# vklyukin/nf_distillation

Hardware: NVIDIA B200
Metric: kd_train_samples_per_sec (higher is better)
Workload: dtype bf16

## Files before the change

include/nfk.h:

```cpp
#ifndef NFK_H_
#define NFK_H_

#ifdef __cplusplus
extern "C" {
#endif

#define NFK_OK 0
#define NFK_ERR_SHAPE (-1)
#define NFK_ERR_ALIGN (-2)
#define NFK_ERR_ARG (-3)
#define NFK_ERR_LAUNCH (-4)
#define NFK_ERR_DRIVER (-5)

#define NFK_EPI_F32 0
#define NFK_EPI_BIAS_RELU_BF16 1
#define NFK_EPI_MASK_BF16 2

int nfk_version(void);

int nfk_gemm_nt_bf16(const void* A, long long lda, const void* B, long long ldb, int M, int N, int K, int epi,
                     void* out, long long ldo, const float* bias, const void* aux, long long ldaux, float* colsum,
                     void* stream);

int nfk_gemm_set_prof(void* buf);

int nfk_gemm_tn_bf16(const void* A, long long lda, const void* B, long long ldb, int Mo, int No, int Kpix,
                     float* out, long long ldo, int sm_count, void* stream);

typedef struct nfk_invconv_item {
  const float *an_bias, *an_logs, *lower, *upper, *log_s, *p, *sign_s, *weight;
  int C, reverse, transpose;
  float *outW, *outb, *out_sl;
} nfk_invconv_item;
typedef struct nfk_invconv_bwd_item {
  nfk_invconv_item fwd;
  const float* dWf;
  int dWf_ld;
  const float* dbf;
  const float* g_ld;
  int B;
  float pixels;
  float *d_bias, *d_logs, *d_lower, *d_upper, *d_log_s, *d_weight;
} nfk_invconv_bwd_item;
int nfk_invconv_prep_batch(int n, const nfk_invconv_item* items, void* stream);
int nfk_invconv_prep_bwd_batch(int n, const nfk_invconv_bwd_item* items, void* stream);

int nfk_invconv_prep(const float* an_bias, const float* an_logs, const float* lower, const float* upper,
                     const float* log_s, const float* p, const float* sign_s, const float* weight, int C, int reverse,
                     int transpose, float* outW, float* outb, float* out_sl, void* stream);

int nfk_invconv_prep_bwd(const float* an_bias, const float* an_logs, const float* lower, const float* upper,
                         const float* log_s, const float* p, const float* sign_s, const float* weight, int C,
                         int reverse, int transpose, const float* Wf, const float* dWf, const float* dbf,
                         const float* g_ld, int B,
                         float pixels, float* d_bias, float* d_logs, float* d_lower, float* d_upper, float* d_log_s,
                         float* d_weight, void* stream);

typedef struct nfk_coupling_item {
  const float *w1, *b1, *l1, *w2, *b2, *l2, *w3, *b3, *l3;
  int cin, hid, cout, K1p, K3p, with_transposed;
  void *B1, *B1T, *B2, *B2T, *B3, *B3T;
  float *bias1, *bias2, *bias3;
} nfk_coupling_item;
typedef struct nfk_coupling_bwd_item {
  nfk_coupling_item fwd;
  const float *dB1, *dbias1, *dB2, *dbias2, *dB3, *dbias3;
  float *dw1, *db1, *dl1, *dw2, *db2, *dl2, *dw3, *db3, *dl3;
} nfk_coupling_bwd_item;
int nfk_coupling_prep_batch(int n, const nfk_coupling_item* items, void* stream);
int nfk_coupling_prep_bwd_batch(int n, const nfk_coupling_bwd_item* items, void* stream);

int nfk_coupling_prep(const float* w1, const float* b1, const float* l1, const float* w2, const float* b2,
                      const float* l2, const float* w3, const float* b3, const float* l3, int cin, int hid, int cout,
                      int K1p, int K3p, void* B1, void* B1T, void* B2, void* B2T, void* B3, void* B3T, float* bias1,
                      float* bias2, float* bias3, int with_transposed, void* stream);

int nfk_coupling_prep_bwd(const float* w1, const float* b1, const float* l1, const float* w2, const float* b2,
                          const float* l2, const float* w3, const float* b3, const float* l3, int cin, int hid,
                          int cout, int K1p, int K3p, const float* dB1, const float* dbias1, const float* dB2,
                          const float* dbias2, const float* dB3, const float* dbias3, float* dw1, float* db1,
                          float* dl1, float* dw2, float* db2, float* dl2, float* dw3, float* db3, float* dl3,
                          void* stream);

int nfk_affine1x1_fwd(const float* x, const float* Wf, const float* bf, const float* sl, float* y, void* col,
                      int K1p, const float* ld_in, float* ld_out, int B, int C, int H, int W, void* stream);

int nfk_coupling_fwd(const float* P, int K3p, const float* bias3, float* y, float* hsave, float* ld, int B, int C,
                     int H, int W, int reverse, void* stream);

int nfk_coupling_bwd(const float* g_out, const float* g_ld, const float* z_out, const float* hsave, float* dy,
                     void* dhcol, int K3p, float* dbias3, int B, int C, int H, int W, void* stream);

int nfk_affine1x1_bwd(const float* dy, const float* dcol, int K1p, const float* x, const float* Wf, float* dx,
                      float* dWf, float* dbf, int B, int C, int H, int W, void* stream);

int nfk_coupling_inv_bwd(const float* g_zc, const float* g_ld, const float* zc, const float* hsave, float* dz,
                         void* dhcol, int K3p, float* dbias3, int B, int C, int H, int W, void* stream);

int nfk_col2im_add(const float* dcol, int K1p, float* dz, int B, int C, int H, int W, void* stream);

int nfk_split2d_fwd(const float* x, const float* w, const float* bias, const float* logs, float* z1_out, float* ld,
                    int B, int C, int H, int W, void* stream);
int nfk_split2d_rev(const float* z1, const float* w, const float* bias, const float* logs, const float* eps,
                    float temperature, float* out, int B, int C, int H, int W, void* stream);
int nfk_split2d_bwd(const float* x, const float* w, const float* bias, const float* logs, const float* g_z1,
                    const float* g_ld, float* dx, float* dw, float* dbias, float* dlogs, int B, int C, int H, int W,
                    void* stream);
int nfk_split2d_squeeze_fwd(const float* x, const float* w, const float* bias, const float* logs, float* z1_out,
                            float* z1_sq_out, float* ld, int B, int C, int H, int W, void* stream);
int nfk_split2d_squeeze_bwd(const float* x, const float* w, const float* bias, const float* logs, const float* g_z1,
                            const float* g_z1_sq, const float* g_ld, float* dx, float* dw, float* dbias, float* dlogs,
                            int B, int C, int H, int W, void* stream);
int nfk_dequant_squeeze(const void* src, int src_is_u8, int n_bits, const float* noise, float* x_out, float* sq_out,
                        int B, int C, int H, int W, void* stream);
int nfk_prior_bpd_fwd(const float* z, const float* mean, const float* logs, const float* logdet, int B, int n,
                      float scale, float* out, void* stream);
int nfk_prior_bpd_bwd(const float* z, const float* mean, const float* logs, const float* g_bpd, int B, int n,
                      float scale, float* dz, float* dlogdet, void* stream);
int nfk_kd_mse_fwd(const float* s, const float* t, int B, int n, float scale, float* acc, void* stream);
int nfk_kd_mse_bwd(const float* s, const float* t, const float* g, int B, int n, float scale, float* ds,
                   int accumulate, void* stream);

int nfk_pconv_coupling_supported(int C, int H, int W, int hid);
int nfk_pconv_coupling_fwd(const void* h2, const void* B3, int K3p, const float* bias3, float* y, float* hsave,
                           float* ld, int B, int C, int H, int W, int hid, int reverse, void* stream);

int nfk_conv1_dgrad_affine_bwd_supported(int C, int H, int W, int hid);
int nfk_conv1_dgrad_affine_bwd(const void* dpre1, const void* B1T, int K1p, const float* dy, const float* x,
                               const float* Wf, float* dx, float* dWf, float* dbf, int B, int C, int H, int W, int hid,
                               void* stream);

int nfk_flow1d_supported(int D, int Cc, int hid, int training);
int nfk_flow1d_sizes(int D, int Cc, int hid, int* total_fwd, int* total_bwd, int* total_grad, int* n_act,
                     int* offsets);
int nfk_flow1d_pack(const float* Wf, const float* bf, const float* const* w, const float* const* b, int D, int Cc,
                    int hid, float* PF, float* PB, void* stream);
int nfk_flow1d_fwd(const float* x, const float* cond, const float* PF, const float* sl, float* y, const float* ld_in,
                   float* ld_out, float* acts, int B, int D, int Cc, int hid, int reverse, void* stream);
int nfk_flow1d_bwd(const float* x_in, const float* cond, const float* acts, const float* PB, const float* y_out,
                   const float* g_out, const float* g_ld, float* dx, float* G, int B, int D, int Cc, int hid,
                   int reverse, void* stream);
int nfk_affine_rows(const float* x, const float* Wf, const float* bf, const float* sl, float* y, const float* ld_in,
                    float* ld_out, int B, int D, float pixels, void* stream);

int nfk_gemm_nt_bf16_ranged(const void* A, long long lda, const void* B, long long ldb, int M, int N, int K, int epi,
                            void* out, long long ldo, const float* bias, const void* aux, long long ldaux,
                            float* colsum, int bn, const int* kb_begin, const int* kb_end, void* stream);

int nfk_made_prep(const float* w1, const float* w2, const float* w3, const int* deg1, const int* deg2, int D, int H,
                  int Dp, int N3p, void* B1, void* B1T, void* B2, void* B2T, void* B3, void* B3T, int with_t,
                  void* stream);
int nfk_made_prep_bwd(const float* dB1, const float* dB2, const float* dB3, const int* deg1, const int* deg2, int D,
                      int H, int Dp, float* dw1, float* dw2, float* dw3, void* stream);
int nfk_rows_to_bf16(const float* x, int B, int D, int Dp, void* xb, void* stream);
int nfk_made_affine_fwd(const float* x, const float* out, int N3p, float* u, void* ub, int Dp, const float* ld_in,
                        float* ld_out, int B, int D, int flip, void* stream);
int nfk_made_affine_bwd(const float* x, const float* out, int N3p, const float* g_u, const float* g_ld, float* dx,
                        void* dout, float* db3, int B, int D, int flip, void* stream);
int nfk_made_inv_update(float* x, void* xb, int Dp, const float* u_in, const float* out, int N3p, const float* ld_in,
                        float* ld_out, int B, int D, int i, int flip, int last, void* stream);
int nfk_made_inverse_resident_supported(int D, int H, int Dp);
int nfk_made_inverse_push_supported(int D, int H, int Dp, int N3p);
int nfk_made_inverse_jobs(const int* cnt1, const int* cnt2, int D, int H, int Dp, int N3p, int push, int* jobs,
                          int cap);
int nfk_made_inverse_pack(const int* jobs, int njobs, const void* B1, const void* B2, const void* B3, int N3p, int D,
                          int H, int Dp, int push, void* wstream, void* stream);
int nfk_made_inverse_resident(const float* u_in, const void* wstream, const float* b1, const float* b2,
                              const float* b3, const int* jobs, int njobs, int push, int N3p, float* x,
                              const float* ld_in, float* ld_out, int B, int D, int H, int Dp, int flip, int mtiles,
                              void* stream);
int nfk_made_inv_bwd_update(const float* c, int ldc, const float* g_x, const float* g_ld, const float* out, int N3p,
                            const float* u_in, float* g_u, void* dout, float* db3, int B, int D, int d, int flip,
                            void* stream);
int nfk_made_inverse_bwd_supported(int D, int H, int N3p);
int nfk_made_inverse_bwd_jobs(const int* cnt1, const int* cnt2, int D, int H, int N3p, int* jobs, int cap);
int nfk_made_inverse_bwd_pack(const int* jobs, int njobs, const void* B1T, const void* B2T, const void* B3T, int D,
                              int H, int N3p, void* wstream, void* stream);
int nfk_made_inverse_bwd_resident(const float* g_x, const float* g_ld, const float* out, const void* m1,
                                  const void* m2, const float* u_in, const void* wstream, const int* jobs, int njobs,
                                  float* g_u, void* dout, float* db3, int B, int D, int H, int N3p, int flip,
                                  int mtiles, void* stream);

int nfk_cnet_set_prof(void* buf);
int nfk_cnet_fwd_fused(const void* col, int K1p, const void* B1, const void* B2, const float* bias1,
                       const float* bias2, void* h1, void* h2, void* mask1, void* mask2, long long ldmask, int M,
                       int hid, void* stream);
int nfk_cnet_bwd_fused(const void* dhcol, int K3p, const void* B3T, const void* B2T, const void* mask_h2,
                       const void* mask_h1, long long ldmask, void* dpre2, void* dpre1, float* dbias2, float* dbias1,
                       int M, int hid, void* stream);
int nfk_cnet_fwd_fused_ranged(const void* col, int K1p, const void* B1, const void* B2, const float* bias1,
                              const float* bias2, void* h1, void* h2, void* mask1, void* mask2, long long ldmask,
                              int M, int hid, int kb2_end_half0, void* stream);

#define NFK_LOSS_MAX_LEVELS 8
typedef struct {
  const float* s[NFK_LOSS_MAX_LEVELS];
  const float* t[NFK_LOSS_MAX_LEVELS];
  float* ds[NFK_LOSS_MAX_LEVELS];
  int n[NFK_LOSS_MAX_LEVELS];
  int L;
} nfk_loss_levels;
int nfk_kd_nll_loss_scratch_floats(int B);
int nfk_kd_nll_loss_fwd(const nfk_loss_levels* levels, const float* z_last, int nz, const float* prior_mean,
                        const float* prior_logs, const float* logdet, float nll_scale, const float* nll_in,
                        const float* perc, const float* sample_w, float w_nll, float w_kd, float w_perc, int B,
                        float* nll_out, float* kd_out, float* means, float* scratch, void* stream);
int nfk_kd_nll_loss_bwd(const nfk_loss_levels* levels, const float* z_last, int nz, const float* prior_mean,
                        const float* prior_logs, float nll_scale, const float* sample_w, float w_nll, float w_kd,
                        float w_perc, int B, const float* g_means, const float* g_nll, const float* g_kd,
                        float* dz_last, float* dlogdet, float* dnll_in, float* dperc, void* stream);

int nfk_optim_partials(void);
int nfk_grad_sqnorm(const float* g, long long n, float* partials, int* step, void* stream);
int nfk_adam_step(float* p, const float* g, float* m, float* v, long long n, const float* partials, const int* step,
                  float max_norm, float lr, float beta1, float beta2, float eps, float weight_decay, int adamax,
                  float* norm_out, void* stream);

int nfk_split3_rows(const float* src, long long lds, long long rows, int K, int Ksrc, int pattern, void* out,
                    void* stream);
int nfk_im2col3x3_split3(const float* src, int layout, int Ctot, int c0, int Cc, int B, int H, int W, int flip,
                         int Kp, int pattern, void* out, void* stream);
int nfk_act_split3(const float* pre, long long M, int N, int mode, const void* gate, long long ldg, int pattern,
                   void* out, float* colsum, void* stream);
int nfk_coupling_bwd_f32(const float* g_out, const float* g_ld, const float* z_out, const float* hsave, float* dy,
                         float* dh, float* dbias3, int B, int C, int H, int W, void* stream);

#ifdef __cplusplus
}
#endif
#endif
```

nf_distillation_b200/_lib.py:

```python
from __future__ import annotations

import ctypes
import os

from . import build as _build

_c = ctypes
_vp, _i, _ll, _f = _c.c_void_p, _c.c_int, _c.c_longlong, _c.c_float

ERRORS = {
    -1: "NFK_ERR_SHAPE (unsupported / inconsistent sizes)",
    -2: "NFK_ERR_ALIGN (pointer or leading dimension not 16-byte aligned)",
    -3: "NFK_ERR_ARG (missing / invalid argument)",
    -4: "NFK_ERR_LAUNCH (CUDA launch failure)",
    -5: "NFK_ERR_DRIVER (tensor-map encode failure)",
}



class InvconvItem(_c.Structure):
    _fields_ = [(n, _vp) for n in ("an_bias", "an_logs", "lower", "upper", "log_s", "p", "sign_s", "weight")] + \
               [("C", _i), ("reverse", _i), ("transpose", _i)] + \
               [(n, _vp) for n in ("outW", "outb", "out_sl")]


class InvconvBwdItem(_c.Structure):
    _fields_ = [("fwd", InvconvItem), ("dWf", _vp), ("dWf_ld", _i), ("dbf", _vp), ("g_ld", _vp), ("B", _i),
                ("pixels", _f)] + \
               [(n, _vp) for n in ("d_bias", "d_logs", "d_lower", "d_upper", "d_log_s", "d_weight")]


class CouplingItem(_c.Structure):
    _fields_ = [(n, _vp) for n in ("w1", "b1", "l1", "w2", "b2", "l2", "w3", "b3", "l3")] + \
               [(n, _i) for n in ("cin", "hid", "cout", "K1p", "K3p", "with_transposed")] + \
               [(n, _vp) for n in ("B1", "B1T", "B2", "B2T", "B3", "B3T", "bias1", "bias2", "bias3")]


class CouplingBwdItem(_c.Structure):
    _fields_ = [("fwd", CouplingItem)] + \
               [(n, _vp) for n in ("dB1", "dbias1", "dB2", "dbias2", "dB3", "dbias3")] + \
               [(n, _vp) for n in ("dw1", "db1", "dl1", "dw2", "db2", "dl2", "dw3", "db3", "dl3")]


NFK_LOSS_MAX_LEVELS = 8


class LossLevels(_c.Structure):
    _fields_ = [("s", _vp * NFK_LOSS_MAX_LEVELS), ("t", _vp * NFK_LOSS_MAX_LEVELS), ("ds", _vp * NFK_LOSS_MAX_LEVELS),
                ("n", _i * NFK_LOSS_MAX_LEVELS), ("L", _i)]


SIGNATURES: dict[str, list] = {
    "nfk_version": [],
    "nfk_gemm_nt_bf16": [_vp, _ll, _vp, _ll, _i, _i, _i, _i, _vp, _ll, _vp, _vp, _ll, _vp, _vp],
    "nfk_gemm_set_prof": [_vp],
    "nfk_gemm_tn_bf16": [_vp, _ll, _vp, _ll, _i, _i, _i, _vp, _ll, _i, _vp],
    "nfk_invconv_prep_batch": [_i, _vp, _vp],
    "nfk_invconv_prep_bwd_batch": [_i, _vp, _vp],
    "nfk_invconv_prep": [_vp] * 8 + [_i, _i, _i, _vp, _vp, _vp, _vp],
    "nfk_invconv_prep_bwd": [_vp] * 8 + [_i, _i, _i, _vp, _vp, _vp, _vp, _i, _f] + [_vp] * 6 + [_vp],
    "nfk_coupling_prep_batch": [_i, _vp, _vp],
    "nfk_coupling_prep_bwd_batch": [_i, _vp, _vp],
    "nfk_coupling_prep": [_vp] * 9 + [_i] * 5 + [_vp] * 9 + [_i, _vp],
    "nfk_coupling_prep_bwd": [_vp] * 9 + [_i] * 5 + [_vp] * 6 + [_vp] * 9 + [_vp],
    "nfk_affine1x1_fwd": [_vp, _vp, _vp, _vp, _vp, _vp, _i, _vp, _vp, _i, _i, _i, _i, _vp],
    "nfk_coupling_fwd": [_vp, _i, _vp, _vp, _vp, _vp, _i, _i, _i, _i, _i, _vp],
    "nfk_coupling_bwd": [_vp, _vp, _vp, _vp, _vp, _vp, _i, _vp, _i, _i, _i, _i, _vp],
    "nfk_affine1x1_bwd": [_vp, _vp, _i, _vp, _vp, _vp, _vp, _vp, _i, _i, _i, _i, _vp],
    "nfk_coupling_inv_bwd": [_vp, _vp, _vp, _vp, _vp, _vp, _i, _vp, _i, _i, _i, _i, _vp],
    "nfk_col2im_add": [_vp, _i, _vp, _i, _i, _i, _i, _vp],
    "nfk_split2d_fwd": [_vp] * 6 + [_i] * 4 + [_vp],
    "nfk_split2d_rev": [_vp] * 5 + [_f, _vp] + [_i] * 4 + [_vp],
    "nfk_split2d_bwd": [_vp] * 10 + [_i] * 4 + [_vp],
    "nfk_split2d_squeeze_fwd": [_vp] * 7 + [_i] * 4 + [_vp],
    "nfk_split2d_squeeze_bwd": [_vp] * 11 + [_i] * 4 + [_vp],
    "nfk_dequant_squeeze": [_vp, _i, _i, _vp, _vp, _vp, _i, _i, _i, _i, _vp],
    "nfk_prior_bpd_fwd": [_vp] * 4 + [_i, _i, _f, _vp, _vp],
    "nfk_prior_bpd_bwd": [_vp] * 4 + [_i, _i, _f, _vp, _vp, _vp],
    "nfk_kd_mse_fwd": [_vp, _vp, _i, _i, _f, _vp, _vp],
    "nfk_kd_mse_bwd": [_vp, _vp, _vp, _i, _i, _f, _vp, _i, _vp],
    "nfk_flow1d_supported": [_i, _i, _i, _i],
    "nfk_flow1d_sizes": [_i, _i, _i, _vp, _vp, _vp, _vp, _vp],
    "nfk_flow1d_pack": [_vp, _vp, _vp, _vp, _i, _i, _i, _vp, _vp, _vp],
    "nfk_flow1d_fwd": [_vp] * 8 + [_i] * 5 + [_vp],
    "nfk_flow1d_bwd": [_vp] * 9 + [_i] * 5 + [_vp],
    "nfk_affine_rows": [_vp] * 7 + [_i, _i, _f, _vp],
    "nfk_gemm_nt_bf16_ranged": [_vp, _ll, _vp, _ll, _i, _i, _i, _i, _vp, _ll, _vp, _vp, _ll, _vp, _i, _vp, _vp, _vp],
    "nfk_cnet_set_prof": [_vp],
    "nfk_cnet_fwd_fused": [_vp, _i, _vp, _vp, _vp, _vp, _vp, _vp, _vp, _vp, _ll, _i, _i, _vp],
    "nfk_cnet_bwd_fused": [_vp, _i, _vp, _vp, _vp, _vp, _ll, _vp, _vp, _vp, _vp, _i, _i, _vp],
    "nfk_cnet_fwd_fused_ranged": [_vp, _i, _vp, _vp, _vp, _vp, _vp, _vp, _vp, _vp, _ll, _i, _i, _i, _vp],
    "nfk_pconv_coupling_supported": [_i, _i, _i, _i],
    "nfk_pconv_coupling_fwd": [_vp, _vp, _i, _vp, _vp, _vp, _vp, _i, _i, _i, _i, _i, _i, _vp],
    "nfk_conv1_dgrad_affine_bwd_supported": [_i, _i, _i, _i],
    "nfk_conv1_dgrad_affine_bwd": [_vp] * 9 + [_i] * 5 + [_vp],
    "nfk_made_prep": [_vp] * 5 + [_i] * 4 + [_vp] * 6 + [_i, _vp],
    "nfk_made_prep_bwd": [_vp] * 5 + [_i] * 3 + [_vp] * 3 + [_vp],
    "nfk_rows_to_bf16": [_vp, _i, _i, _i, _vp, _vp],
    "nfk_made_affine_fwd": [_vp, _vp, _i, _vp, _vp, _i, _vp, _vp, _i, _i, _i, _vp],
    "nfk_made_affine_bwd": [_vp, _vp, _i, _vp, _vp, _vp, _vp, _vp, _i, _i, _i, _vp],
    "nfk_made_inv_update": [_vp, _vp, _i, _vp, _vp, _i, _vp, _vp, _i, _i, _i, _i, _i, _vp],
    "nfk_made_inverse_resident_supported": [_i, _i, _i],
    "nfk_made_inverse_push_supported": [_i, _i, _i, _i],
    "nfk_made_inverse_jobs": [_vp, _vp, _i, _i, _i, _i, _i, _vp, _i],
    "nfk_made_inverse_pack": [_vp, _i, _vp, _vp, _vp, _i, _i, _i, _i, _i, _vp, _vp],
    "nfk_made_inverse_resident": [_vp] * 6 + [_i] * 3 + [_vp] * 3 + [_i] * 6 + [_vp],
    "nfk_made_inv_bwd_update": [_vp, _i, _vp, _vp, _vp, _i, _vp, _vp, _vp, _vp, _i, _i, _i, _i, _vp],
    "nfk_made_inverse_bwd_supported": [_i, _i, _i],
    "nfk_made_inverse_bwd_jobs": [_vp, _vp, _i, _i, _i, _vp, _i],
    "nfk_made_inverse_bwd_pack": [_vp, _i, _vp, _vp, _vp, _i, _i, _i, _vp, _vp],
    "nfk_made_inverse_bwd_resident": [_vp] * 8 + [_i] + [_vp] * 3 + [_i] * 6 + [_vp],
    "nfk_kd_nll_loss_scratch_floats": [_i],
    "nfk_kd_nll_loss_fwd": [_vp, _vp, _i, _vp, _vp, _vp, _f, _vp, _vp, _vp, _f, _f, _f, _i, _vp, _vp, _vp, _vp, _vp],
    "nfk_kd_nll_loss_bwd": [_vp, _vp, _i, _vp, _vp, _f, _vp, _f, _f, _f, _i, _vp, _vp, _vp, _vp, _vp, _vp, _vp, _vp],
    "nfk_optim_partials": [],
    "nfk_grad_sqnorm": [_vp, _ll, _vp, _vp, _vp],
    "nfk_adam_step": [_vp, _vp, _vp, _vp, _ll, _vp, _vp, _f, _f, _f, _f, _f, _f, _i, _vp, _vp],
    "nfk_split3_rows": [_vp, _ll, _ll, _i, _i, _i, _vp, _vp],
    "nfk_im2col3x3_split3": [_vp, _i, _i, _i, _i, _i, _i, _i, _i, _i, _i, _vp, _vp],
    "nfk_act_split3": [_vp, _ll, _i, _i, _vp, _ll, _i, _vp, _vp, _vp],
    "nfk_coupling_bwd_f32": [_vp, _vp, _vp, _vp, _vp, _vp, _vp, _i, _i, _i, _i, _vp],
}


class NfkError(RuntimeError):
    pass


def _load() -> ctypes.CDLL:
    path = _build.LIB_PATH
    if _build.needs_build():
        try:
            _build.build()
        except Exception as e:
            if not os.path.exists(path):
                raise ImportError(
                    f"libnfk.so is not built and cannot be built here ({e}); there is no CPU fallback") from e
    lib = ctypes.CDLL(path)
    for name, argtypes in SIGNATURES.items():
        fn = getattr(lib, name)
        fn.argtypes = argtypes
        fn.restype = _c.c_int
    return lib


LIB = _load()


def check(rc: int, what: str) -> None:
    if rc != 0:
        raise NfkError(f"{what} failed: {ERRORS.get(rc, rc)}")


def ptr(t) -> int | None:
    return None if t is None else t.data_ptr()


def stream_ptr() -> int:
    import torch

    return torch.cuda.current_stream().cuda_stream
```

nf_distillation_b200/csrc/cnet_fused.cu:

```cuda
#include <cuda.h>
#include <cuda_bf16.h>
#include <cuda_runtime.h>
#include <cstdint>
#include <cstdlib>

#include "../../include/nfk.h"
#include "launch_util.h"
#include "ptx.cuh"

namespace nfk {

constexpr int CF_THREADS = 320;
constexpr int CF_HID = 512;
constexpr int CF_SLOT = 16384;
constexpr int CF_SLOTS = 4;
constexpr int CF_PANEL = 16384;

struct CnetArgs {
  int M;
  int kb1;
  const float* bias1;
  const float* bias2;
  uint32_t* mask1;
  uint32_t* mask2;
  long long ldmask;
  int store_h1;
  long long* prof;
  int kb2_end[2];
  float* colsum1;
  float* colsum2;
};

struct CnetSmem {
  static constexpr int h1 = 0;
  static constexpr int ring = h1 + 8 * CF_PANEL;
  static constexpr int stage = ring + CF_SLOTS * CF_SLOT;
  static constexpr int bars = stage + 8 * 4096;
  static constexpr int total = bars + 256;
};

__device__ __forceinline__ uint32_t pack2(float lo, float hi) {
  __nv_bfloat162 v = __floats2bfloat162_rn(lo, hi);
  return *reinterpret_cast<uint32_t*>(&v);
}

template <int MODE>
__device__ __forceinline__ void cnet_fused_body(const CUtensorMap& tmCol, const CUtensorMap& tmB1,
                                                const CUtensorMap& tmB2, const CUtensorMap& tmH1,
                                                const CUtensorMap& tmH2, const CnetArgs& g) {
  extern __shared__ __align__(1024) uint8_t smem[];
  pdl_launch_dependents();
  if (smem_u32(smem) & 1023u) __trap();
  const int warp = static_cast<int>(uniform_u32(threadIdx.x >> 5)), lane = threadIdx.x & 31;
  const uint32_t rank = blockIdx.x & 1;
  const int pair = blockIdx.x >> 1, num_pairs = gridDim.x >> 1;
  const int num_tiles = (g.M + 255) / 256;

  uint64_t* full = reinterpret_cast<uint64_t*>(smem + CnetSmem::bars);
  uint64_t* empty = full + CF_SLOTS;
  uint64_t* acc_full = empty + CF_SLOTS;
  uint64_t* acc_empty = acc_full + 2;
  uint64_t* h1_full = acc_empty + 2;
  uint64_t* h1_empty = h1_full + 8;
  uint32_t* tmem_slot = reinterpret_cast<uint32_t*>(h1_empty + 1);

  if (warp == 0 && lane == 0) {
    tma_prefetch_desc(&tmCol); tma_prefetch_desc(&tmB1); tma_prefetch_desc(&tmB2); tma_prefetch_desc(&tmH2);
    for (int s = 0; s < CF_SLOTS; ++s) { mbar_init(&full[s], 1); mbar_init(&empty[s], 1); }
    for (int a = 0; a < 2; ++a) { mbar_init(&acc_full[a], 1); mbar_init(&acc_empty[a], 16); }
    for (int p = 0; p < 8; ++p) mbar_init(&h1_full[p], 8);
    mbar_init(h1_empty, 1);
    fence_mbar_init();
  }
  if (warp == 1) { tmem_alloc_pair(tmem_slot, 512); tmem_relinquish_pair(); }
  tc_fence_before();
  cluster_sync_all();
  tc_fence_after();
  const uint32_t tmem_base = uniform_u32(*tmem_slot);
  pdl_wait();

  if (warp == 0) {
    {
      int s = 0; uint32_t ph = 0;
      auto load = [&](const CUtensorMap* tm, int c0, int c1) {
        mbar_wait_warp(&empty[s], ph ^ 1);
        if (rank == 0) mbar_expect_tx_elect(&full[s], 2 * CF_SLOT);
        tma_load_2d_pair_elect(smem + CnetSmem::ring + s * CF_SLOT, tm, &full[s], c0, c1);
        if (++s == CF_SLOTS) { s = 0; ph ^= 1; }
      };
      for (int t = pair; t < num_tiles; t += num_pairs) {
        const int row0 = t * 256 + static_cast<int>(rank) * 128;
        for (int h = 0; h < 2; ++h)
          for (int kb = 0; kb < g.kb1; ++kb) {
            load(&tmCol, kb * 64, row0);
            load(&tmB1, kb * 64, h * 256 + static_cast<int>(rank) * 128);
          }
        for (int h = 0; h < 2; ++h)
          for (int kb = 0; kb < g.kb2_end[h]; ++kb) load(&tmB2, kb * 64, h * 256 + static_cast<int>(rank) * 128);
      }
    }
  } else if (warp == 1) {
    if (rank == 0) {
      const uint32_t idesc = umma_idesc_bf16(256, 256, false, false);
      const uint32_t ring_addr = smem_u32(smem + CnetSmem::ring);
      const uint32_t h1_addr = smem_u32(smem + CnetSmem::h1);
      int s = 0; uint32_t ph = 0;
      uint32_t nacc = 0;
      uint32_t tile_ph = 0;
      long long w_op = 0, w_acc = 0, w_h1 = 0;
      const long long t_begin = g.prof ? clock64() : 0;
      auto take = [&]() {
        const long long c0 = g.prof ? clock64() : 0;
        mbar_wait_warp(&full[s], ph);
        if (g.prof) w_op += clock64() - c0;
        tc_fence_after();
        return ring_addr + s * CF_SLOT;
      };
      auto advance = [&]() { if (++s == CF_SLOTS) { s = 0; ph ^= 1; } };
      auto release = [&]() { umma_commit_pair_elect(&empty[s], 3); advance(); };
      auto acc_begin = [&]() {
        const uint32_t st = nacc & 1;
        const long long c0 = g.prof ? clock64() : 0;
        mbar_wait_warp(&acc_empty[st], ((nacc >> 1) & 1) ^ 1);
        if (g.prof) w_acc += clock64() - c0;
        tc_fence_after();
        return tmem_base + st * 256;
      };
      auto acc_end = [&]() { umma_commit_pair_elect(&acc_full[nacc & 1], 3); ++nacc; };
      for (int t = pair; t < num_tiles; t += num_pairs) {
        for (int h = 0; h < 2; ++h) {
          const uint32_t d = acc_begin();
          for (int kb = 0; kb < g.kb1; ++kb) {
            const uint32_t a = take();
            const int sa = s;
            advance();
            const uint32_t b = take();
#pragma unroll
            for (int k = 0; k < 4; ++k)
              umma_f16_pair_elect(d, umma_desc_sw128(a + k * 32, 16, 1024), umma_desc_sw128(b + k * 32, 16, 1024), idesc,
                            (kb > 0 || k > 0) ? 1u : 0u);
            umma_commit_pair_elect(&empty[sa], 3);
            release();
          }
          acc_end();
        }
        int panels_seen = 0;
        for (int h = 0; h < 2; ++h) {
          const uint32_t d = acc_begin();
          for (int kb = 0; kb < g.kb2_end[h]; ++kb) {
            if (kb >= panels_seen) {
              const long long c0 = g.prof ? clock64() : 0;
              mbar_wait_warp(&h1_full[kb], tile_ph);
              if (g.prof) w_h1 += clock64() - c0;
              tc_fence_after();
              panels_seen = kb + 1;
            }
            const uint32_t b = take();
#pragma unroll
            for (int k = 0; k < 4; ++k)
              umma_f16_pair_elect(d, umma_desc_sw128(h1_addr + kb * CF_PANEL + k * 32, 16, 1024),
                            umma_desc_sw128(b + k * 32, 16, 1024), idesc, (kb > 0 || k > 0) ? 1u : 0u);
            release();
          }
          acc_end();
        }
        umma_commit_pair_elect(h1_empty, 3);
        tile_ph ^= 1;
      }
      if (g.prof && lane == 0) {
        long long* o = g.prof + blockIdx.x * 8;
        o[0] = clock64() - t_begin; o[1] = w_op; o[2] = w_acc; o[3] = w_h1;
      }
    }
  } else {
    const int qd = warp & 3;
    const int hf = (warp - 2) >> 2;
    const uint32_t lane_off = static_cast<uint32_t>(qd * 32) << 16;
    const uint32_t sw = static_cast<uint32_t>(lane & 7);
    uint8_t* stage = smem + CnetSmem::stage + (warp - 2) * 4096;
    uint32_t nacc = 0, tile_ph = 0;
    auto epi16 = [&](const uint32_t (&r)[16], const float* bias16, uint8_t* dst, int cc0, bool want_bits) -> uint32_t {
      uint32_t p[8];
      const __nv_bfloat162 zero2 = __floats2bfloat162_rn(0.f, 0.f);
#pragma unroll
      for (int j = 0; j < 16; j += 4) {
        const float4 b = __ldg(reinterpret_cast<const float4*>(bias16 + j));
        const float2 s0 = __fadd2_rn(make_float2(__uint_as_float(r[j]), __uint_as_float(r[j + 1])),
                                     make_float2(b.x, b.y));
        const float2 s1 = __fadd2_rn(make_float2(__uint_as_float(r[j + 2]), __uint_as_float(r[j + 3])),
                                     make_float2(b.z, b.w));
        const __nv_bfloat162 h0 = __hmax2(__float22bfloat162_rn(s0), zero2);
        const __nv_bfloat162 h1 = __hmax2(__float22bfloat162_rn(s1), zero2);
        p[j / 2] = *reinterpret_cast<const uint32_t*>(&h0);
        p[j / 2 + 1] = *reinterpret_cast<const uint32_t*>(&h1);
      }
      uint32_t bits = 0;
      if (want_bits) {
#pragma unroll
        for (int k = 0; k < 8; ++k) {
          bits |= ((p[k] & 0xFFFFu) ? 1u : 0u) << (2 * k);
          bits |= ((p[k] >> 16) ? 1u : 0u) << (2 * k + 1);
        }
      }
      *reinterpret_cast<uint4*>(dst + ((static_cast<uint32_t>(cc0) ^ sw) << 4)) = make_uint4(p[0], p[1], p[2], p[3]);
      *reinterpret_cast<uint4*>(dst + ((static_cast<uint32_t>(cc0 + 1) ^ sw) << 4)) =
          make_uint4(p[4], p[5], p[6], p[7]);
      return bits;
    };
    auto panel64 = [&](const uint32_t (&r0)[16], const uint32_t (&r1)[16], const uint32_t (&r2)[16],
                       const uint32_t (&r3)[16], const float* bias, uint8_t* dst_rows, uint32_t* mask, long long row,
                       int col0) {
      uint8_t* dst = dst_rows + lane * 128;
      const bool wb = mask != nullptr;
      const uint32_t b0 = epi16(r0, bias, dst, 0, wb), b1 = epi16(r1, bias + 16, dst, 2, wb);
      const uint32_t b2 = epi16(r2, bias + 32, dst, 4, wb), b3 = epi16(r3, bias + 48, dst, 6, wb);
      if (wb && row < g.M) {
        mask[static_cast<long long>(col0 >> 5) * g.ldmask + row] = b0 | (b1 << 16);
        mask[static_cast<long long>((col0 + 32) >> 5) * g.ldmask + row] = b2 | (b3 << 16);
      }
    };
    auto epi16m = [&](const uint32_t (&r)[16], uint32_t bits16, uint8_t* dst, int cc0) {
      uint32_t p[8];
#pragma unroll
      for (int k = 0; k < 8; ++k) {
        const float lo = ((bits16 >> (2 * k)) & 1u) ? __uint_as_float(r[2 * k]) : 0.f;
        const float hi = ((bits16 >> (2 * k + 1)) & 1u) ? __uint_as_float(r[2 * k + 1]) : 0.f;
        p[k] = pack2(lo, hi);
      }
      *reinterpret_cast<uint4*>(dst + ((static_cast<uint32_t>(cc0) ^ sw) << 4)) = make_uint4(p[0], p[1], p[2], p[3]);
      *reinterpret_cast<uint4*>(dst + ((static_cast<uint32_t>(cc0 + 1) ^ sw) << 4)) =
          make_uint4(p[4], p[5], p[6], p[7]);
    };
    auto panel64m = [&](const uint32_t (&r0)[16], const uint32_t (&r1)[16], const uint32_t (&r2)[16],
                        const uint32_t (&r3)[16], uint32_t w0, uint32_t w1, uint8_t* dst_rows) {
      uint8_t* dst = dst_rows + lane * 128;
      epi16m(r0, w0 & 0xFFFFu, dst, 0); epi16m(r1, w0 >> 16, dst, 2);
      epi16m(r2, w1 & 0xFFFFu, dst, 4); epi16m(r3, w1 >> 16, dst, 6);
    };
    auto panel_colsum = [&](const uint8_t* rows, float& s0, float& s1) {
      const uint8_t* pb = rows + (lane & 3) * 4;
      const uint32_t chunk = static_cast<uint32_t>(lane >> 2);
      float a0 = 0.f, a1 = 0.f, b0 = 0.f, b1 = 0.f;
#pragma unroll 8
      for (int r = 0; r < 32; r += 2) {
        const uint32_t w0 = *reinterpret_cast<const uint32_t*>(pb + r * 128 + ((chunk ^ (r & 7)) << 4));
        const uint32_t w1 = *reinterpret_cast<const uint32_t*>(pb + (r + 1) * 128 + ((chunk ^ ((r + 1) & 7)) << 4));
        a0 += __uint_as_float(w0 << 16); a1 += __uint_as_float(w0 & 0xFFFF0000u);
        b0 += __uint_as_float(w1 << 16); b1 += __uint_as_float(w1 & 0xFFFF0000u);
      }
      s0 += a0 + b0; s1 += a1 + b1;
    };
    float cs1[4][2] = {}, cs2[4][2] = {};
    auto load128 = [&](uint32_t tm, uint32_t (&R)[8][16]) {
#pragma unroll
      for (int i = 0; i < 8; ++i) tmem_ld16(tm + 16 * i, R[i]);
      tmem_ld_wait();
    };
    for (int t = pair; t < num_tiles; t += num_pairs) {
      const int row0 = t * 256 + static_cast<int>(rank) * 128 + qd * 32;
      const long long row = row0 + lane;
      uint32_t mw1[8], mw2[8];
      if constexpr (MODE == 1) {
#pragma unroll
        for (int i = 0; i < 4; ++i) {
          const int c1 = (4 * (i >> 1) + 2 * (i & 1) + hf) * 64;
          const int c2 = (i >> 1) * 256 + hf * 128 + (i & 1) * 64;
          const bool ok = row < g.M;
          mw1[2 * i] = ok ? __ldg(g.mask1 + static_cast<long long>(c1 >> 5) * g.ldmask + row) : 0u;
          mw1[2 * i + 1] = ok ? __ldg(g.mask1 + static_cast<long long>((c1 + 32) >> 5) * g.ldmask + row) : 0u;
          mw2[2 * i] = ok ? __ldg(g.mask2 + static_cast<long long>(c2 >> 5) * g.ldmask + row) : 0u;
          mw2[2 * i + 1] = ok ? __ldg(g.mask2 + static_cast<long long>((c2 + 32) >> 5) * g.ldmask + row) : 0u;
        }
      }
      mbar_wait(h1_empty, tile_ph ^ 1);
      if (g.store_h1) {
        if (lane == 0) asm volatile("cp.async.bulk.wait_group.read 0;" ::: "memory");
        __syncwarp();
      }
      for (int h = 0; h < 2; ++h) {
        const uint32_t st = nacc & 1;
        mbar_wait(&acc_full[st], (nacc >> 1) & 1);
        tc_fence_after();
        const uint32_t tm = tmem_base + st * 256 + lane_off;
        uint32_t R[8][16];
#pragma unroll
        for (int i = 0; i < 4; ++i) tmem_ld16(tm + hf * 64 + 16 * i, R[i]);
#pragma unroll
        for (int i = 0; i < 4; ++i) tmem_ld16(tm + (hf + 2) * 64 + 16 * i, R[4 + i]);
        tmem_ld_wait();
        tc_fence_before();
        __syncwarp();
        if (lane == 0) mbar_arrive_cluster(&acc_empty[st], 0);
#pragma unroll
        for (int pz = 0; pz < 2; ++pz) {
          const int panel = 4 * h + 2 * pz + hf;
          uint8_t* dst = smem + CnetSmem::h1 + panel * CF_PANEL + qd * 32 * 128;
          if constexpr (MODE == 0) {
            if (pz == 0) panel64(R[0], R[1], R[2], R[3], g.bias1 + panel * 64, dst, g.mask1, row, panel * 64);
            else panel64(R[4], R[5], R[6], R[7], g.bias1 + panel * 64, dst, g.mask1, row, panel * 64);
          } else {
            if (pz == 0) panel64m(R[0], R[1], R[2], R[3], h ? mw1[4] : mw1[0], h ? mw1[5] : mw1[1], dst);
            else panel64m(R[4], R[5], R[6], R[7], h ? mw1[6] : mw1[2], h ? mw1[7] : mw1[3], dst);
          }
          fence_proxy_async();
          __syncwarp();
          if constexpr (MODE == 1) {
            float s0 = 0.f, s1 = 0.f;
            panel_colsum(dst, s0, s1);
            if (h == 0) { cs1[pz][0] += s0; cs1[pz][1] += s1; } else { cs1[2 + pz][0] += s0; cs1[2 + pz][1] += s1; }
          }
          if (lane == 0) {
            mbar_arrive_cluster(&h1_full[panel], 0);
            if (g.store_h1 && row0 < g.M) tma_store_2d(dst, &tmH1, panel * 64, row0);
          }
        }
        if (g.store_h1 && lane == 0) asm volatile("cp.async.bulk.commit_group;" ::: "memory");
        ++nacc;
      }
      for (int h = 0; h < 2; ++h) {
        const uint32_t st = nacc & 1;
        mbar_wait(&acc_full[st], (nacc >> 1) & 1);
        tc_fence_after();
        const uint32_t tm = tmem_base + st * 256 + hf * 128 + lane_off;
        uint32_t R[8][16];
        load128(tm, R);
        tc_fence_before();
        __syncwarp();
        if (lane == 0) mbar_arrive_cluster(&acc_empty[st], 0);
#pragma unroll
        for (int pz = 0; pz < 2; ++pz) {
          const int col0 = h * 256 + hf * 128 + pz * 64;
          if (lane == 0) asm volatile("cp.async.bulk.wait_group.read 0;" ::: "memory");
          __syncwarp();
          if constexpr (MODE == 0) {
            if (pz == 0) panel64(R[0], R[1], R[2], R[3], g.bias2 + col0, stage, g.mask2, row, col0);
            else panel64(R[4], R[5], R[6], R[7], g.bias2 + col0, stage, g.mask2, row, col0);
          } else {
            if (pz == 0) panel64m(R[0], R[1], R[2], R[3], h ? mw2[4] : mw2[0], h ? mw2[5] : mw2[1], stage);
            else panel64m(R[4], R[5], R[6], R[7], h ? mw2[6] : mw2[2], h ? mw2[7] : mw2[3], stage);
          }
          fence_proxy_async();
          __syncwarp();
          if constexpr (MODE == 1) {
            float s0 = 0.f, s1 = 0.f;
            panel_colsum(stage, s0, s1);
            if (h == 0) { cs2[pz][0] += s0; cs2[pz][1] += s1; } else { cs2[2 + pz][0] += s0; cs2[2 + pz][1] += s1; }
          }
          if (lane == 0 && row0 < g.M) {
            tma_store_2d(stage, &tmH2, col0, row0);
            asm volatile("cp.async.bulk.commit_group;" ::: "memory");
          }
        }
        ++nacc;
      }
      tile_ph ^= 1;
    }
    if constexpr (MODE == 1) {
      const int cpair = (lane >> 2) * 8 + (lane & 3) * 2;
#pragma unroll
      for (int i = 0; i < 4; ++i) {
        const int c1 = (4 * (i >> 1) + 2 * (i & 1) + hf) * 64 + cpair;
        const int c2 = (i >> 1) * 256 + hf * 128 + (i & 1) * 64 + cpair;
        if (g.colsum1) { atomicAdd(g.colsum1 + c1, cs1[i][0]); atomicAdd(g.colsum1 + c1 + 1, cs1[i][1]); }
        if (g.colsum2) { atomicAdd(g.colsum2 + c2, cs2[i][0]); atomicAdd(g.colsum2 + c2 + 1, cs2[i][1]); }
      }
    }
    if (lane == 0) asm volatile("cp.async.bulk.wait_group 0;" ::: "memory");
  }
  tc_fence_before();
  cluster_sync_all();
  if (warp == 1) tmem_dealloc_pair(tmem_base, 512);
}

__global__ void __cluster_dims__(2, 1, 1) __launch_bounds__(CF_THREADS, 1)
cnet_fwd_fused_kernel(const __grid_constant__ CUtensorMap tmCol, const __grid_constant__ CUtensorMap tmB1,
                      const __grid_constant__ CUtensorMap tmB2, const __grid_constant__ CUtensorMap tmH1,
                      const __grid_constant__ CUtensorMap tmH2, const CnetArgs g) {
  cnet_fused_body<0>(tmCol, tmB1, tmB2, tmH1, tmH2, g);
}

__global__ void __cluster_dims__(2, 1, 1) __launch_bounds__(CF_THREADS, 1)
cnet_bwd_fused_kernel(const __grid_constant__ CUtensorMap tmCol, const __grid_constant__ CUtensorMap tmB1,
                      const __grid_constant__ CUtensorMap tmB2, const __grid_constant__ CUtensorMap tmH1,
                      const __grid_constant__ CUtensorMap tmH2, const CnetArgs g) {
  cnet_fused_body<1>(tmCol, tmB1, tmB2, tmH1, tmH2, g);
}

typedef CUresult (*EncodeTiledFn2)(CUtensorMap*, CUtensorMapDataType, cuuint32_t, void*, const cuuint64_t*,
                                   const cuuint64_t*, const cuuint32_t*, const cuuint32_t*, CUtensorMapInterleave,
                                   CUtensorMapSwizzle, CUtensorMapL2promotion, CUtensorMapFloatOOBfill);

static int cf_tmap(CUtensorMap* m, const void* ptr, uint64_t cols, uint64_t rows, uint64_t ld, uint32_t box_rows,
                   bool f32) {
  static EncodeTiledFn2 enc = nullptr;
  if (!enc) {
    void* p = nullptr;
    cudaDriverEntryPointQueryResult q;
    if (cudaGetDriverEntryPoint("cuTensorMapEncodeTiled", &p, cudaEnableDefault, &q) != cudaSuccess ||
        q != cudaDriverEntryPointSuccess)
      return NFK_ERR_DRIVER;
    enc = reinterpret_cast<EncodeTiledFn2>(p);
  }
  const uint64_t es = f32 ? 4 : 2;
  if ((reinterpret_cast<uintptr_t>(ptr) & 15) || (ld * es) % 16) return NFK_ERR_ALIGN;
  cuuint64_t dims[2] = {cols, rows};
  cuuint64_t strides[1] = {ld * es};
  cuuint32_t box[2] = {static_cast<cuuint32_t>(128 / es), box_rows};
  cuuint32_t estr[2] = {1, 1};
  return enc(m, f32 ? CU_TENSOR_MAP_DATA_TYPE_FLOAT32 : CU_TENSOR_MAP_DATA_TYPE_BFLOAT16, 2, const_cast<void*>(ptr),
             dims, strides, box, estr, CU_TENSOR_MAP_INTERLEAVE_NONE, CU_TENSOR_MAP_SWIZZLE_128B,
             CU_TENSOR_MAP_L2_PROMOTION_L2_256B, CU_TENSOR_MAP_FLOAT_OOB_FILL_NONE) == CUDA_SUCCESS
             ? NFK_OK
             : NFK_ERR_DRIVER;
}

int cnet_ts_fwd(const void* col, int K1p, const void* B1, const void* B2, const float* bias1, const float* bias2,
                void* h1, void* h2, void* mask1, void* mask2, long long ldmask, int M, int kb2_end_half0,
                long long* prof, void* stream);
int cnet_ts_bwd(const void* dhcol, int K3p, const void* B3T, const void* B2T, const void* mask_h2,
                const void* mask_h1, long long ldmask, void* dpre2, void* dpre1, float* dbias2, float* dbias1, int M,
                void* stream);
static bool cnet_use_ts() {
  static const bool v = [] { const char* e = getenv("NFK_CNET_TS"); return !(e && e[0] == '0'); }();
  return v;
}

}

using namespace nfk;

static long long* g_cnet_prof = nullptr;
extern "C" int nfk_cnet_set_prof(void* buf) {
  g_cnet_prof = static_cast<long long*>(buf);
  return NFK_OK;
}

extern "C" int nfk_cnet_fwd_fused(const void* col, int K1p, const void* B1, const void* B2, const float* bias1,
                                  const float* bias2, void* h1, void* h2, void* mask1, void* mask2,
                                  long long ldmask, int M, int hid, void* stream) {
  return nfk_cnet_fwd_fused_ranged(col, K1p, B1, B2, bias1, bias2, h1, h2, mask1, mask2, ldmask, M, hid, 8, stream);
}

extern "C" int nfk_cnet_fwd_fused_ranged(const void* col, int K1p, const void* B1, const void* B2, const float* bias1,
                                         const float* bias2, void* h1, void* h2, void* mask1, void* mask2,
                                         long long ldmask, int M, int hid, int kb2_end_half0, void* stream) {
  if (M <= 0 || hid != CF_HID || K1p % 64 || K1p < 64 || K1p > 512) return NFK_ERR_SHAPE;
  if (kb2_end_half0 < 1 || kb2_end_half0 > 8) return NFK_ERR_ARG;
  if (!col || !B1 || !B2 || !bias1 || !bias2 || !h2) return NFK_ERR_ARG;
  if ((mask1 || mask2) && ldmask < M) return NFK_ERR_ARG;
  if (cnet_use_ts())
    return cnet_ts_fwd(col, K1p, B1, B2, bias1, bias2, h1, h2, mask1, mask2, ldmask, M, kb2_end_half0, g_cnet_prof,
                       stream);
  CnetArgs g{M, K1p / 64, bias1, bias2, static_cast<uint32_t*>(mask1), static_cast<uint32_t*>(mask2), ldmask,
             h1 ? 1 : 0, g_cnet_prof, {kb2_end_half0, 8}, nullptr, nullptr};
  CUtensorMap tmCol, tmB1, tmB2, tmH1, tmH2;
  int rc;
  if ((rc = cf_tmap(&tmCol, col, K1p, M, K1p, 128, false))) return rc;
  if ((rc = cf_tmap(&tmB1, B1, K1p, hid, K1p, 128, false))) return rc;
  if ((rc = cf_tmap(&tmB2, B2, hid, hid, hid, 128, false))) return rc;
  if ((rc = cf_tmap(&tmH2, h2, hid, M, hid, 32, false))) return rc;
  if (h1) { if ((rc = cf_tmap(&tmH1, h1, hid, M, hid, 32, false))) return rc; }
  else tmH1 = tmH2;
  if ((rc = ensure_dyn_smem(reinterpret_cast<const void*>(cnet_fwd_fused_kernel), CnetSmem::total))) return rc;
  int dev = 0, sms = 148;
  cudaGetDevice(&dev);
  cudaDeviceGetAttribute(&sms, cudaDevAttrMultiProcessorCount, dev);
  const int tiles = (M + 255) / 256;
  const int pairs = tiles < sms / 2 ? tiles : sms / 2;
  const cudaError_t le = launch_pdl(cnet_fwd_fused_kernel, dim3(2 * pairs), dim3(CF_THREADS), CnetSmem::total,
                                    static_cast<cudaStream_t>(stream), tmCol, tmB1, tmB2, tmH1, tmH2, g);
  return (le == cudaSuccess && cudaGetLastError() == cudaSuccess) ? NFK_OK : NFK_ERR_LAUNCH;
}

extern "C" int nfk_cnet_bwd_fused(const void* dhcol, int K3p, const void* B3T, const void* B2T, const void* mask_h2,
                                  const void* mask_h1, long long ldmask, void* dpre2, void* dpre1, float* dbias2,
                                  float* dbias1, int M, int hid, void* stream) {
  if (M <= 0 || hid != CF_HID || K3p % 64 || K3p < 64 || K3p > 512) return NFK_ERR_SHAPE;
  if (!dhcol || !B3T || !B2T || !mask_h2 || !mask_h1 || !dpre2 || !dpre1) return NFK_ERR_ARG;
  if (ldmask < M) return NFK_ERR_ARG;
  if (cnet_use_ts())
    return cnet_ts_bwd(dhcol, K3p, B3T, B2T, mask_h2, mask_h1, ldmask, dpre2, dpre1, dbias2, dbias1, M, stream);
  CnetArgs g{M, K3p / 64, nullptr, nullptr, static_cast<uint32_t*>(const_cast<void*>(mask_h2)),
             static_cast<uint32_t*>(const_cast<void*>(mask_h1)), ldmask, 1, nullptr, {8, 8}, dbias2, dbias1};
  CUtensorMap tmA, tmB1, tmB2, tmD2, tmD1;
  int rc;
  if ((rc = cf_tmap(&tmA, dhcol, K3p, M, K3p, 128, false))) return rc;
  if ((rc = cf_tmap(&tmB1, B3T, K3p, hid, K3p, 128, false))) return rc;
  if ((rc = cf_tmap(&tmB2, B2T, hid, hid, hid, 128, false))) return rc;
  if ((rc = cf_tmap(&tmD2, dpre2, hid, M, hid, 32, false))) return rc;
  if ((rc = cf_tmap(&tmD1, dpre1, hid, M, hid, 32, false))) return rc;
  if ((rc = ensure_dyn_smem(reinterpret_cast<const void*>(cnet_bwd_fused_kernel), CnetSmem::total))) return rc;
  int dev = 0, sms = 148;
  cudaGetDevice(&dev);
  cudaDeviceGetAttribute(&sms, cudaDevAttrMultiProcessorCount, dev);
  const int tiles = (M + 255) / 256;
  const int pairs = tiles < sms / 2 ? tiles : sms / 2;
  const cudaError_t le = launch_pdl(cnet_bwd_fused_kernel, dim3(2 * pairs), dim3(CF_THREADS), CnetSmem::total,
                                    static_cast<cudaStream_t>(stream), tmA, tmB1, tmB2, tmD2, tmD1, g);
  return (le == cudaSuccess && cudaGetLastError() == cudaSuccess) ? NFK_OK : NFK_ERR_LAUNCH;
}
```

nf_distillation_b200/csrc/cnet_ts.cu:

```cuda
#include <cuda.h>
#include <cuda_bf16.h>
#include <cuda_runtime.h>
#include <cstdint>
#include <cstdlib>

#include "../../include/nfk.h"
#include "launch_util.h"
#include "ptx.cuh"

namespace nfk {

constexpr int TS_THREADS = 576;
constexpr int TS_HID = 512;
constexpr int TS_BOX = 8192;
constexpr int TS_SLOT = 2 * TS_BOX;
constexpr int TS_MAX_SLOTS = 8;
constexpr int TS_COLBLK = 16384;
constexpr int TS_STAGE = 4096;
constexpr int TS_STAGE_BYTES = 16 * TS_STAGE;
constexpr int TS_BAR_BYTES = 512;
constexpr int TS_BIAS_BYTES = 2 * TS_HID * 4;
constexpr uint32_t TS_ACC0 = 256;

struct TsArgs {
  int M;
  int kb1;
  int nslots;
  const float* bias1;
  const float* bias2;
  uint32_t* mask1;
  uint32_t* mask2;
  long long ldmask;
  int store_h1;
  long long* prof;
  int kb2_end[2];
  float* colsum1;
  float* colsum2;
};

__device__ __forceinline__ void umma_f16_pair_ts(uint32_t tmem_d, uint32_t tmem_a, uint64_t bdesc, uint32_t idesc,
                                                 uint32_t accumulate) {
  asm volatile(
      "{\n\t.reg .pred p;\n\t"
      "setp.ne.b32 p, %4, 0;\n\t"
      "tcgen05.mma.cta_group::2.kind::f16 [%0], [%1], %2, %3, p;\n\t}\n"
      ::"r"(tmem_d), "r"(tmem_a), "l"(bdesc), "r"(idesc), "r"(accumulate)
      : "memory");
}
__device__ __forceinline__ void tmem_st16(uint32_t taddr, const uint32_t (&a)[8], const uint32_t (&b)[8]) {
  asm volatile(
      "tcgen05.st.sync.aligned.32x32b.x16.b32 [%0], "
      "{%1,%2,%3,%4,%5,%6,%7,%8,%9,%10,%11,%12,%13,%14,%15,%16};"
      ::"r"(taddr), "r"(a[0]), "r"(a[1]), "r"(a[2]), "r"(a[3]), "r"(a[4]), "r"(a[5]), "r"(a[6]), "r"(a[7]), "r"(b[0]),
        "r"(b[1]), "r"(b[2]), "r"(b[3]), "r"(b[4]), "r"(b[5]), "r"(b[6]), "r"(b[7])
      : "memory");
}
__device__ __forceinline__ uint32_t relu_bf16x2(float lo, float hi) {
  uint32_t d;
  asm("cvt.rn.relu.bf16x2.f32 %0, %1, %2;" : "=r"(d) : "f"(hi), "f"(lo));
  return d;
}
__device__ __forceinline__ void tmem_st_wait() { asm volatile("tcgen05.wait::st.sync.aligned;" ::: "memory"); }

template <int MODE>
__device__ __forceinline__ void cnet_ts_body(const CUtensorMap& tmCol, const CUtensorMap& tmB1, const CUtensorMap& tmB2,
                                             const CUtensorMap& tmH1, const CUtensorMap& tmH2, const TsArgs& g) {
  extern __shared__ __align__(1024) uint8_t smem[];
  pdl_launch_dependents();
  if (smem_u32(smem) & 1023u) __trap();
  const int warp = static_cast<int>(uniform_u32(threadIdx.x >> 5)), lane = threadIdx.x & 31;
  const uint32_t rank = blockIdx.x & 1;
  const int pair = blockIdx.x >> 1, num_pairs = gridDim.x >> 1;
  const int num_tiles = (g.M + 255) / 256;
  const int nslots = g.nslots;

  uint8_t* colbuf = smem;
  uint8_t* stage_base = colbuf + g.kb1 * TS_COLBLK;
  uint8_t* ring = stage_base + TS_STAGE_BYTES;
  uint64_t* full = reinterpret_cast<uint64_t*>(ring + nslots * TS_SLOT);
  uint64_t* empty = full + TS_MAX_SLOTS;
  uint64_t* acc_full = empty + TS_MAX_SLOTS;
  uint64_t* acc_empty = acc_full + 2;
  uint64_t* h1_full = acc_empty + 2;
  uint64_t* h1_empty = h1_full + 8;
  uint64_t* col_full = h1_empty + 1;
  uint64_t* col_empty = col_full + 1;
  uint32_t* tmem_slot = reinterpret_cast<uint32_t*>(col_empty + 1);
  float* bias_s = reinterpret_cast<float*>(reinterpret_cast<uint8_t*>(full) + TS_BAR_BYTES);

  if (warp == 0 && lane == 0) {
    tma_prefetch_desc(&tmCol); tma_prefetch_desc(&tmB1); tma_prefetch_desc(&tmB2); tma_prefetch_desc(&tmH2);
    for (int s = 0; s < nslots; ++s) { mbar_init(&full[s], 1); mbar_init(&empty[s], 1); }
    for (int a = 0; a < 2; ++a) { mbar_init(&acc_full[a], 1); mbar_init(&acc_empty[a], 16); }
    for (int p = 0; p < 8; ++p) mbar_init(&h1_full[p], 8);
    mbar_init(h1_empty, 1);
    mbar_init(col_full, 1);
    mbar_init(col_empty, 1);
    fence_mbar_init();
  }
  if (warp == 1) { tmem_alloc_pair(tmem_slot, 512); tmem_relinquish_pair(); }
  tc_fence_before();
  cluster_sync_all();
  tc_fence_after();
  const uint32_t tmem_base = uniform_u32(*tmem_slot);
  pdl_wait();

  if (warp == 0) {
    {
      int s = 0; uint32_t ph = 0, col_ph = 0;
      auto load = [&](const CUtensorMap* tm, int kb, int kend, int row) {
        const int nkb = kend - kb < 2 ? kend - kb : 2;
        mbar_wait_warp(&empty[s], ph ^ 1);
        if (rank == 0) mbar_expect_tx_elect(&full[s], static_cast<uint32_t>(2 * nkb * TS_BOX));
        for (int j = 0; j < nkb; ++j)
          tma_load_2d_pair_elect(ring + s * TS_SLOT + j * TS_BOX, tm, &full[s], (kb + j) * 64, row);
        if (++s == nslots) { s = 0; ph ^= 1; }
      };
      auto load_col = [&](int t) {
        mbar_wait_warp(col_empty, col_ph ^ 1);
        if (rank == 0) mbar_expect_tx_elect(col_full, static_cast<uint32_t>(2 * g.kb1 * TS_COLBLK));
        const int row0 = t * 256 + static_cast<int>(rank) * 128;
        for (int kb = 0; kb < g.kb1; ++kb)
          tma_load_2d_pair_elect(colbuf + kb * TS_COLBLK, &tmCol, col_full, kb * 64, row0);
        col_ph ^= 1;
      };
      if (pair < num_tiles) load_col(pair);
      for (int t = pair; t < num_tiles; t += num_pairs) {
        const int wrow = static_cast<int>(rank) * 64;
        for (int q = 0; q < 4; ++q)
          for (int kb = 0; kb < g.kb1; kb += 2) load(&tmB1, kb, g.kb1, q * 128 + wrow);
        for (int q = 0; q < 4; ++q) {
          const int qe = q;
          const int kend = qe < 2 ? g.kb2_end[0] : g.kb2_end[1];
          for (int kb = 0; kb < kend; kb += 2) load(&tmB2, kb, kend, qe * 128 + wrow);
          if (q == 0 && t + num_pairs < num_tiles) load_col(t + num_pairs);
        }
      }
    }
  } else if (warp == 1) {
    if (rank == 0) {
      const uint32_t idesc = umma_idesc_bf16(256, 128, false, false);
      const uint32_t ring_addr = smem_u32(ring);
      const uint32_t col_addr = smem_u32(colbuf);
      int s = 0; uint32_t ph = 0;
      uint32_t nacc = 0;
      uint32_t tile_ph = 0;
      long long w_op = 0, w_acc = 0, w_h1 = 0, w_col = 0, w_b1 = 0, w_q0 = 0;
      const long long t_begin = g.prof ? clock64() : 0;
      auto take = [&]() {
        const long long c0 = g.prof ? clock64() : 0;
        mbar_wait_warp(&full[s], ph);
        if (g.prof) w_op += clock64() - c0;
        tc_fence_after();
        return ring_addr + s * TS_SLOT;
      };
      auto release = [&]() { umma_commit_pair_elect(&empty[s], 3); if (++s == nslots) { s = 0; ph ^= 1; } };
      auto acc_begin = [&]() {
        const uint32_t st = nacc & 1;
        const long long c0 = g.prof ? clock64() : 0;
        mbar_wait_warp(&acc_empty[st], ((nacc >> 1) & 1) ^ 1);
        if (g.prof) w_acc += clock64() - c0;
        tc_fence_after();
        return tmem_base + TS_ACC0 + st * 128;
      };
      auto acc_end = [&]() { umma_commit_pair_elect(&acc_full[nacc & 1], 3); ++nacc; };
#ifdef NFK_CNET_TIMELINE
      auto mstamp = [&](int t, int idx) {
        if (g.prof && blockIdx.x == 0 && t == 6 * num_pairs && lane == 0) g.prof[150 * 8 + idx] = clock64();
      };
#else
      auto mstamp = [](int, int) {};
#endif
      for (int t = pair; t < num_tiles; t += num_pairs) {
        mstamp(t, 0);
        {
          const long long c0 = g.prof ? clock64() : 0;
          mbar_wait_warp(col_full, tile_ph);
          if (g.prof) { w_op += clock64() - c0; w_col += clock64() - c0; }
          tc_fence_after();
        }
        const long long w_op_g1 = w_op;
        for (int q = 0; q < 4; ++q) {
          const uint32_t d = acc_begin();
          if (q == 0) mstamp(t, 1);
          for (int kb = 0; kb < g.kb1; kb += 2) {
            const uint32_t b = take();
            const int nkb = g.kb1 - kb < 2 ? g.kb1 - kb : 2;
            for (int j = 0; j < nkb; ++j) {
#pragma unroll
              for (int k = 0; k < 4; ++k)
                umma_f16_pair_elect(d, umma_desc_sw128(col_addr + (kb + j) * TS_COLBLK + k * 32, 16, 1024),
                                    umma_desc_sw128(b + j * TS_BOX + k * 32, 16, 1024), idesc,
                                    (kb + j > 0 || k > 0) ? 1u : 0u);
            }
            release();
          }
          acc_end();
        }
        umma_commit_pair_elect(col_empty, 3);
        mstamp(t, 2);
        w_b1 += w_op - w_op_g1;
        int blocks_seen = 0;
        for (int q = 0; q < 4; ++q) {
          const uint32_t d = acc_begin();
          mstamp(t, 3 + q);
          const long long w_op_q = w_op;
          const int kend = q < 2 ? g.kb2_end[0] : g.kb2_end[1];
          for (int kb = 0; kb < kend; kb += 2) {
            const uint32_t b = take();
            const int nkb = kend - kb < 2 ? kend - kb : 2;
            for (int j = 0; j < nkb; ++j) {
              if (kb + j >= blocks_seen) {
                const long long c0 = g.prof ? clock64() : 0;
                mbar_wait_warp(&h1_full[kb + j], tile_ph);
                if (g.prof) w_h1 += clock64() - c0;
                tc_fence_after();
                blocks_seen = kb + j + 1;
              }
#pragma unroll
              for (int k = 0; k < 4; ++k)
                umma_f16_pair_ts_elect(d, tmem_base + static_cast<uint32_t>((kb + j) * 32 + k * 8),
                                       umma_desc_sw128(b + j * TS_BOX + k * 32, 16, 1024), idesc,
                                       (kb + j > 0 || k > 0) ? 1u : 0u);
            }
            release();
          }
          acc_end();
          if (q == 0) w_q0 += w_op - w_op_q;
          if (q == 3) mstamp(t, 7);
        }
        umma_commit_pair_elect(h1_empty, 3);
        tile_ph ^= 1;
      }
      if (g.prof && lane == 0) {
        long long* o = g.prof + blockIdx.x * 8;
        o[0] = clock64() - t_begin; o[1] = w_op; o[2] = w_acc; o[3] = w_h1; o[4] = w_col; o[5] = w_b1; o[6] = w_q0;
      }
    }
  } else {
    const int ew = warp - 2;
    const int qd = warp & 3;
    const int hf = (ew >> 2) & 1;
    const int ws = ew >> 3;
    const uint32_t lane_off = static_cast<uint32_t>(qd * 32) << 16;
    const uint32_t sw = static_cast<uint32_t>(lane & 7);
    uint8_t* panel = stage_base + ew * TS_STAGE;
    uint32_t nuse = 0, tile_ph = 0;
    auto epi16 = [&](const uint32_t (&r)[16], const float* bias16, uint32_t (&p)[8], bool want_bits) -> uint32_t {
#pragma unroll
      for (int j = 0; j < 16; j += 4) {
        const float4 b = *reinterpret_cast<const float4*>(bias16 + j);
        const float2 s0 = __fadd2_rn(make_float2(__uint_as_float(r[j]), __uint_as_float(r[j + 1])),
                                     make_float2(b.x, b.y));
        const float2 s1 = __fadd2_rn(make_float2(__uint_as_float(r[j + 2]), __uint_as_float(r[j + 3])),
                                     make_float2(b.z, b.w));
        p[j / 2] = relu_bf16x2(s0.x, s0.y);
        p[j / 2 + 1] = relu_bf16x2(s1.x, s1.y);
      }
      uint32_t bits = 0;
      if (want_bits) {
#pragma unroll
        for (int k = 0; k < 8; ++k) {
          bits |= ((p[k] & 0xFFFFu) ? 1u : 0u) << (2 * k);
          bits |= ((p[k] >> 16) ? 1u : 0u) << (2 * k + 1);
        }
      }
      return bits;
    };
    auto epi16m = [&](const uint32_t (&r)[16], uint32_t bits16, uint32_t (&p)[8]) {
#pragma unroll
      for (int k = 0; k < 8; ++k) {
        const float lo = ((bits16 >> (2 * k)) & 1u) ? __uint_as_float(r[2 * k]) : 0.f;
        const float hi = ((bits16 >> (2 * k + 1)) & 1u) ? __uint_as_float(r[2 * k + 1]) : 0.f;
        __nv_bfloat162 v = __floats2bfloat162_rn(lo, hi);
        p[k] = *reinterpret_cast<uint32_t*>(&v);
      }
    };
    auto to_panel = [&](const uint32_t (&P)[4][8]) {
      if (lane == 0) asm volatile("cp.async.bulk.wait_group.read 0;" ::: "memory");
      __syncwarp();
      uint8_t* dst = panel + lane * 128;
#pragma unroll
      for (int i = 0; i < 4; ++i) {
        *reinterpret_cast<uint4*>(dst + ((static_cast<uint32_t>(2 * i) ^ sw) << 4)) =
            make_uint4(P[i][0], P[i][1], P[i][2], P[i][3]);
        *reinterpret_cast<uint4*>(dst + ((static_cast<uint32_t>(2 * i + 1) ^ sw) << 4)) =
            make_uint4(P[i][4], P[i][5], P[i][6], P[i][7]);
      }
      fence_proxy_async();
      __syncwarp();
    };
    auto panel_colsum = [&](float& s0, float& s1) {
      const uint8_t* pb = panel + (lane & 3) * 4;
      const uint32_t chunk = static_cast<uint32_t>(lane >> 2);
      float a0 = 0.f, a1 = 0.f, b0 = 0.f, b1 = 0.f;
#pragma unroll 8
      for (int r = 0; r < 32; r += 2) {
        const uint32_t w0 = *reinterpret_cast<const uint32_t*>(pb + r * 128 + ((chunk ^ (r & 7)) << 4));
        const uint32_t w1 = *reinterpret_cast<const uint32_t*>(pb + (r + 1) * 128 + ((chunk ^ ((r + 1) & 7)) << 4));
        a0 += __uint_as_float(w0 << 16); a1 += __uint_as_float(w0 & 0xFFFF0000u);
        b0 += __uint_as_float(w1 << 16); b1 += __uint_as_float(w1 & 0xFFFF0000u);
      }
      s0 += a0 + b0; s1 += a1 + b1;
    };
    float cs1[2][2] = {}, cs2[2][2] = {};
    if constexpr (MODE == 0) {
      for (int i = threadIdx.x - 64; i < TS_HID; i += TS_THREADS - 64) {
        bias_s[i] = __ldg(g.bias1 + i);
        bias_s[TS_HID + i] = __ldg(g.bias2 + i);
      }
      asm volatile("bar.sync 1, %0;" ::"n"(TS_THREADS - 64) : "memory");
    }

#ifdef NFK_CNET_TIMELINE
    auto stamp = [&](int t, int idx) {
      if (g.prof && blockIdx.x == 0 && t == 6 * num_pairs && lane == 0) {
        if (qd == 0 && hf == 0) g.prof[(148 + ws) * 8 + idx] = clock64();
        g.prof[(152 + ew) * 8 + idx] = clock64();
      }
    };
#else
    auto stamp = [](int, int) {};
#endif
    for (int t = pair; t < num_tiles; t += num_pairs) {
      const int row0 = t * 256 + static_cast<int>(rank) * 128 + qd * 32;
      const long long row = row0 + lane;
      const bool row_ok = row < g.M;
      uint32_t mw1[4], mw2[4];
      if constexpr (MODE == 1) {
#pragma unroll
        for (int qq = 0; qq < 2; ++qq) {
          const int c = (2 * qq + ws) * 128 + hf * 64;
          mw1[2 * qq] = row_ok ? __ldg(g.mask1 + static_cast<long long>(c >> 5) * g.ldmask + row) : 0u;
          mw1[2 * qq + 1] = row_ok ? __ldg(g.mask1 + static_cast<long long>((c + 32) >> 5) * g.ldmask + row) : 0u;
          mw2[2 * qq] = row_ok ? __ldg(g.mask2 + static_cast<long long>(c >> 5) * g.ldmask + row) : 0u;
          mw2[2 * qq + 1] = row_ok ? __ldg(g.mask2 + static_cast<long long>((c + 32) >> 5) * g.ldmask + row) : 0u;
        }
      }
      const uint32_t tm = tmem_base + TS_ACC0 + ws * 128 + hf * 64 + lane_off;
#pragma unroll
      for (int qq = 0; qq < 2; ++qq) {
        mbar_wait(&acc_full[ws], nuse & 1);
        stamp(t, qq == 0 ? 0 : 6);
        tc_fence_after();
        uint32_t R[4][16];
#pragma unroll
        for (int i = 0; i < 4; ++i) tmem_ld16(tm + 16 * i, R[i]);
        tmem_ld_wait();
        if (qq == 0) stamp(t, 1);
        tc_fence_before();
        __syncwarp();
        if (lane == 0) mbar_arrive_cluster(&acc_empty[ws], 0);
        const int col0 = (2 * qq + ws) * 128 + hf * 64;
        uint32_t P[4][8];
        if constexpr (MODE == 0) {
          const bool wb = g.mask1 != nullptr;
          uint32_t b[4];
#pragma unroll
          for (int i = 0; i < 4; ++i) b[i] = epi16(R[i], bias_s + col0 + 16 * i, P[i], wb);
          if (wb && row_ok) {
            g.mask1[static_cast<long long>(col0 >> 5) * g.ldmask + row] = b[0] | (b[1] << 16);
            g.mask1[static_cast<long long>((col0 + 32) >> 5) * g.ldmask + row] = b[2] | (b[3] << 16);
          }
        } else {
          epi16m(R[0], mw1[2 * qq] & 0xFFFFu, P[0]); epi16m(R[1], mw1[2 * qq] >> 16, P[1]);
          epi16m(R[2], mw1[2 * qq + 1] & 0xFFFFu, P[2]); epi16m(R[3], mw1[2 * qq + 1] >> 16, P[3]);
        }
        if (qq == 0) stamp(t, 2);
        if (qq == 0) {
          mbar_wait(h1_empty, tile_ph ^ 1);
          tc_fence_after();
        }
        if (qq == 0) stamp(t, 3);
        const uint32_t th = tmem_base + lane_off + static_cast<uint32_t>(col0 >> 1);
        tmem_st16(th, P[0], P[1]);
        tmem_st16(th + 16, P[2], P[3]);
        tmem_st_wait();
        if (qq == 0) stamp(t, 4);
        tc_fence_before();
        __syncwarp();
        if (lane == 0) mbar_arrive_cluster(&h1_full[2 * (2 * qq + ws) + hf], 0);
        stamp(t, qq == 0 ? 5 : 7);
        if (g.store_h1) {
          to_panel(P);
          if constexpr (MODE == 1) {
            float s0 = 0.f, s1 = 0.f;
            panel_colsum(s0, s1);
            cs1[qq][0] += s0; cs1[qq][1] += s1;
          }
          if (lane == 0) {
            if (row0 < g.M) tma_store_2d(panel, &tmH1, col0, row0);
            asm volatile("cp.async.bulk.commit_group;" ::: "memory");
          }
        }
        ++nuse;
      }
#pragma unroll
      for (int qq = 0; qq < 2; ++qq) {
        mbar_wait(&acc_full[ws], nuse & 1);
        tc_fence_after();
        uint32_t R[4][16];
#pragma unroll
        for (int i = 0; i < 4; ++i) tmem_ld16(tm + 16 * i, R[i]);
        tmem_ld_wait();
        tc_fence_before();
        __syncwarp();
        if (lane == 0) mbar_arrive_cluster(&acc_empty[ws], 0);
        const int col0 = (2 * qq + ws) * 128 + hf * 64;
        uint32_t P[4][8];
        if constexpr (MODE == 0) {
          const bool wb = g.mask2 != nullptr;
          uint32_t b[4];
#pragma unroll
          for (int i = 0; i < 4; ++i) b[i] = epi16(R[i], bias_s + TS_HID + col0 + 16 * i, P[i], wb);
          if (wb && row_ok) {
            g.mask2[static_cast<long long>(col0 >> 5) * g.ldmask + row] = b[0] | (b[1] << 16);
            g.mask2[static_cast<long long>((col0 + 32) >> 5) * g.ldmask + row] = b[2] | (b[3] << 16);
          }
        } else {
          epi16m(R[0], mw2[2 * qq] & 0xFFFFu, P[0]); epi16m(R[1], mw2[2 * qq] >> 16, P[1]);
          epi16m(R[2], mw2[2 * qq + 1] & 0xFFFFu, P[2]); epi16m(R[3], mw2[2 * qq + 1] >> 16, P[3]);
        }
        to_panel(P);
        if constexpr (MODE == 1) {
          float s0 = 0.f, s1 = 0.f;
          panel_colsum(s0, s1);
          cs2[qq][0] += s0; cs2[qq][1] += s1;
        }
        if (lane == 0) {
          if (row0 < g.M) tma_store_2d(panel, &tmH2, col0, row0);
          asm volatile("cp.async.bulk.commit_group;" ::: "memory");
        }
        ++nuse;
      }
      tile_ph ^= 1;
    }
    if constexpr (MODE == 1) {
      const int cpair = (lane >> 2) * 8 + (lane & 3) * 2;
#pragma unroll
      for (int qq = 0; qq < 2; ++qq) {
        const int c = (2 * qq + ws) * 128 + hf * 64 + cpair;
        if (g.colsum1) { atomicAdd(g.colsum1 + c, cs1[qq][0]); atomicAdd(g.colsum1 + c + 1, cs1[qq][1]); }
        if (g.colsum2) { atomicAdd(g.colsum2 + c, cs2[qq][0]); atomicAdd(g.colsum2 + c + 1, cs2[qq][1]); }
      }
    }
    if (lane == 0) asm volatile("cp.async.bulk.wait_group 0;" ::: "memory");
  }
  tc_fence_before();
  cluster_sync_all();
  if (warp == 1) tmem_dealloc_pair(tmem_base, 512);
}

__global__ void __cluster_dims__(2, 1, 1) __launch_bounds__(TS_THREADS, 1)
cnet_fwd_ts_kernel(const __grid_constant__ CUtensorMap tmCol, const __grid_constant__ CUtensorMap tmB1,
                   const __grid_constant__ CUtensorMap tmB2, const __grid_constant__ CUtensorMap tmH1,
                   const __grid_constant__ CUtensorMap tmH2, const TsArgs g) {
  cnet_ts_body<0>(tmCol, tmB1, tmB2, tmH1, tmH2, g);
}

__global__ void __cluster_dims__(2, 1, 1) __launch_bounds__(TS_THREADS, 1)
cnet_bwd_ts_kernel(const __grid_constant__ CUtensorMap tmCol, const __grid_constant__ CUtensorMap tmB1,
                   const __grid_constant__ CUtensorMap tmB2, const __grid_constant__ CUtensorMap tmH1,
                   const __grid_constant__ CUtensorMap tmH2, const TsArgs g) {
  cnet_ts_body<1>(tmCol, tmB1, tmB2, tmH1, tmH2, g);
}

typedef CUresult (*EncodeTiledFn3)(CUtensorMap*, CUtensorMapDataType, cuuint32_t, void*, const cuuint64_t*,
                                   const cuuint64_t*, const cuuint32_t*, const cuuint32_t*, CUtensorMapInterleave,
                                   CUtensorMapSwizzle, CUtensorMapL2promotion, CUtensorMapFloatOOBfill);

static int ts_tmap(CUtensorMap* m, const void* ptr, uint64_t cols, uint64_t rows, uint64_t ld, uint32_t box_rows) {
  static EncodeTiledFn3 enc = nullptr;
  if (!enc) {
    void* p = nullptr;
    cudaDriverEntryPointQueryResult q;
    if (cudaGetDriverEntryPoint("cuTensorMapEncodeTiled", &p, cudaEnableDefault, &q) != cudaSuccess ||
        q != cudaDriverEntryPointSuccess)
      return NFK_ERR_DRIVER;
    enc = reinterpret_cast<EncodeTiledFn3>(p);
  }
  if ((reinterpret_cast<uintptr_t>(ptr) & 15) || (ld * 2) % 16) return NFK_ERR_ALIGN;
  cuuint64_t dims[2] = {cols, rows};
  cuuint64_t strides[1] = {ld * 2};
  cuuint32_t box[2] = {64, box_rows};
  cuuint32_t estr[2] = {1, 1};
  return enc(m, CU_TENSOR_MAP_DATA_TYPE_BFLOAT16, 2, const_cast<void*>(ptr), dims, strides, box, estr,
             CU_TENSOR_MAP_INTERLEAVE_NONE, CU_TENSOR_MAP_SWIZZLE_128B, CU_TENSOR_MAP_L2_PROMOTION_L2_256B,
             CU_TENSOR_MAP_FLOAT_OOB_FILL_NONE) == CUDA_SUCCESS
             ? NFK_OK
             : NFK_ERR_DRIVER;
}

static int ts_smem_plan(int kb1, int* nslots) {
  const int fixed = kb1 * TS_COLBLK + TS_STAGE_BYTES + TS_BAR_BYTES + TS_BIAS_BYTES;
  int n = (227 * 1024 - fixed) / TS_SLOT;
  if (n > TS_MAX_SLOTS) n = TS_MAX_SLOTS;
  static const int cap = [] { const char* e = getenv("NFK_CNET_SLOTS"); return e ? atoi(e) : 0; }();
  if (cap >= 2 && n > cap) n = cap;
  *nslots = n;
  return fixed + n * TS_SLOT;
}

template <int MODE>
static int ts_launch(const void* A, int Ka, const void* W1, const void* W2, void* out1, void* out2, TsArgs g,
                     cudaStream_t stream) {
  int nslots = 0;
  const int smem_bytes = ts_smem_plan(Ka / 64, &nslots);
  if (nslots < 2) return NFK_ERR_SHAPE;
  g.nslots = nslots;
  CUtensorMap tmA, tmW1, tmW2, tmO1, tmO2;
  int rc;
  if ((rc = ts_tmap(&tmA, A, Ka, g.M, Ka, 128))) return rc;
  if ((rc = ts_tmap(&tmW1, W1, Ka, TS_HID, Ka, 64))) return rc;
  if ((rc = ts_tmap(&tmW2, W2, TS_HID, TS_HID, TS_HID, 64))) return rc;
  if ((rc = ts_tmap(&tmO2, out2, TS_HID, g.M, TS_HID, 32))) return rc;
  if (out1) { if ((rc = ts_tmap(&tmO1, out1, TS_HID, g.M, TS_HID, 32))) return rc; }
  else tmO1 = tmO2;
  auto kernel = MODE == 0 ? cnet_fwd_ts_kernel : cnet_bwd_ts_kernel;
  if ((rc = ensure_dyn_smem(reinterpret_cast<const void*>(kernel), smem_bytes))) return rc;
  int dev = 0, sms = 148;
  cudaGetDevice(&dev);
  cudaDeviceGetAttribute(&sms, cudaDevAttrMultiProcessorCount, dev);
  const int tiles = (g.M + 255) / 256;
  const int pairs = tiles < sms / 2 ? tiles : sms / 2;
  const cudaError_t le = launch_pdl(kernel, dim3(2 * pairs), dim3(TS_THREADS), smem_bytes, stream, tmA, tmW1, tmW2,
                                    tmO1, tmO2, g);
  return (le == cudaSuccess && cudaGetLastError() == cudaSuccess) ? NFK_OK : NFK_ERR_LAUNCH;
}

int cnet_ts_fwd(const void* col, int K1p, const void* B1, const void* B2, const float* bias1, const float* bias2,
                void* h1, void* h2, void* mask1, void* mask2, long long ldmask, int M, int kb2_end_half0,
                long long* prof, void* stream) {
  TsArgs g{M, K1p / 64, 0, bias1, bias2, static_cast<uint32_t*>(mask1), static_cast<uint32_t*>(mask2), ldmask,
           h1 ? 1 : 0, prof, {kb2_end_half0, 8}, nullptr, nullptr};
  return ts_launch<0>(col, K1p, B1, B2, h1, h2, g, static_cast<cudaStream_t>(stream));
}

int cnet_ts_bwd(const void* dhcol, int K3p, const void* B3T, const void* B2T, const void* mask_h2,
                const void* mask_h1, long long ldmask, void* dpre2, void* dpre1, float* dbias2, float* dbias1, int M,
                void* stream) {
  TsArgs g{M, K3p / 64, 0, nullptr, nullptr, static_cast<uint32_t*>(const_cast<void*>(mask_h2)),
           static_cast<uint32_t*>(const_cast<void*>(mask_h1)), ldmask, 1, nullptr, {8, 8}, dbias2, dbias1};
  return ts_launch<1>(dhcol, K3p, B3T, B2T, dpre2, dpre1, g, static_cast<cudaStream_t>(stream));
}

}
```

nf_distillation_b200/csrc/zpath.cu:

```cuda
#include <cuda_bf16.h>
#include <cuda_runtime.h>
#include <cstdint>

#include "../../include/nfk.h"
#include "launch_util.h"
#include "ptx.cuh"

namespace nfk {

constexpr int ZT = 256;

__device__ __forceinline__ uint32_t bf2(float lo, float hi) {
  __nv_bfloat162 v = __floats2bfloat162_rn(lo, hi);
  return *reinterpret_cast<uint32_t*>(&v);
}

__device__ __forceinline__ void sigmoid_logsigmoid(float t, float& s, float& ls) {
  const float e = expf(-fabsf(t));
  const float l1p = log1pf(e);
  if (t >= 0.f) {
    s = 1.f / (1.f + e);
    ls = -l1p;
  } else {
    s = e / (1.f + e);
    ls = t - l1p;
  }
}

struct Geo {
  int B, HW, W, H;
  int ipc;
  int pixt;
  int og;
  int lgHW, lgW;
};

__device__ __forceinline__ void copy_out_rows(uint4* __restrict__ out4, const uint4* __restrict__ cst, int npix,
                                              int r16, int rs16, int tid) {
  if ((r16 & (r16 - 1)) == 0 && r16 <= ZT) {
    const int lg = __ffs(r16) - 1;
    const int c4 = tid & (r16 - 1), step = ZT >> lg;
    for (int pl = tid >> lg; pl < npix; pl += step) out4[(pl << lg) + c4] = cst[pl * rs16 + c4];
  } else {
    for (int i = tid; i < npix * r16; i += ZT) {
      const int pl = i / r16, c4 = i - pl * r16;
      out4[i] = cst[pl * rs16 + c4];
    }
  }
}

template <int C>
__global__ void __launch_bounds__(ZT)
affine1x1_fwd_kernel(const float* __restrict__ x, const float* __restrict__ Wf, const float* __restrict__ bf,
                     const float* __restrict__ sl, float* __restrict__ y, __nv_bfloat16* __restrict__ col,
                     const float* __restrict__ ld_in, float* __restrict__ ld_out, Geo g, int K1p) {
  pdl_launch_dependents();
  pdl_wait();
  extern __shared__ float sm[];
  constexpr int CH = C / 2;
  float* Ws = sm;
  float* bs = Ws + C * C;
  float* y1s = bs + C;
  float* cst_raw = y1s + ((CH * (g.pixt + 1) + 3) & ~3);
  const int tid = threadIdx.x;
  const int b0 = blockIdx.x * g.ipc;
  const int nimg = min(g.ipc, g.B - b0);
  const int npix = nimg << g.lgHW;
  const int ldp = g.pixt + 1;
  const int HWm = g.HW - 1, Wm = g.W - 1;

  const int pixb = ZT / g.og;
  const int og = tid / pixb;
  const int opg = C / g.og;
  constexpr bool PREFETCH_X = C <= 24;
  float xv[C];
  if (PREFETCH_X) {
    const int pl = tid % pixb;
    if (pl < npix && og < g.og) {
      const float* xp = x + (static_cast<long long>(b0 + (pl >> g.lgHW)) * C << g.lgHW) + (pl & HWm);
#pragma unroll
      for (int i = 0; i < C; ++i) xv[i] = __ldg(xp + (static_cast<long long>(i) << g.lgHW));
    }
  }
  if (Wf) {
    constexpr int W4 = C * C / 4, WPT = (W4 + ZT - 1) / ZT;
    float4 wreg[WPT];
#pragma unroll
    for (int k = 0; k < WPT; ++k) {
      const int i = tid + k * ZT;
      if (i < W4) wreg[k] = __ldg(reinterpret_cast<const float4*>(Wf) + i);
    }
#pragma unroll
    for (int k = 0; k < WPT; ++k) {
      const int i = tid + k * ZT;
      if (i < W4) reinterpret_cast<float4*>(Ws)[i] = wreg[k];
    }
    for (int i = tid; i < C; i += ZT) bs[i] = bf[i];
  }
  if (ld_out && tid < nimg) ld_out[b0 + tid] = ld_in[b0 + tid] + sl[0] * static_cast<float>(g.HW);
  __syncthreads();

  for (int pl = tid % pixb; pl < npix && og < g.og; pl += pixb) {
    const int img = pl >> g.lgHW, p = pl & HWm;
    const float* xp = x + (static_cast<long long>(b0 + img) * C << g.lgHW) + p;
    if (!PREFETCH_X || pl >= pixb) {
#pragma unroll
      for (int i = 0; i < C; ++i) xv[i] = __ldg(xp + (static_cast<long long>(i) << g.lgHW));
    }
    if (Wf) {
      float* yp = y + (static_cast<long long>(b0 + img) * C << g.lgHW) + p;
      for (int o = og * opg; o < (og + 1) * opg; ++o) {
        float acc = bs[o];
        const float4* wr = reinterpret_cast<const float4*>(Ws + o * C);
#pragma unroll
        for (int i = 0; i < C / 4; ++i) {
          const float4 w = wr[i];
          acc = fmaf(w.x, xv[4 * i], acc);
          acc = fmaf(w.y, xv[4 * i + 1], acc);
          acc = fmaf(w.z, xv[4 * i + 2], acc);
          acc = fmaf(w.w, xv[4 * i + 3], acc);
        }
        yp[static_cast<long long>(o) << g.lgHW] = acc;
        if (col && o < CH) y1s[o * ldp + pl] = acc;
      }
    } else if (col) {
#pragma unroll
      for (int o = 0; o < CH; ++o)
        if (o >= og * opg && o < (og + 1) * opg) y1s[o * ldp + pl] = xv[o];
    }
  }
  if (!col) return;
  __syncthreads();
  constexpr int K1 = 9 * CH;
  constexpr int NCH = (K1 + 7) / 8;
  const int r16 = K1p / 8;
  const int rs16 = r16 + 1;
  uint4* cst = reinterpret_cast<uint4*>(cst_raw);
  int noff[9];
#pragma unroll
  for (int tap = 0; tap < 9; ++tap) noff[tap] = (tap / 3 - 1) * g.W + (tap % 3 - 1);
  const int GR = g.pixt >= ZT ? 1 : ZT / g.pixt;
  const int gid = tid / g.pixt;
  for (int pl = GR > 1 ? (tid & (g.pixt - 1)) : tid; pl < npix; pl += (GR > 1 ? g.pixt : ZT)) {
    const int rem = pl & HWm;
    const int yy = rem >> g.lgW, xx = rem & Wm;
    uint32_t vmask = 0;
#pragma unroll
    for (int tap = 0; tap < 9; ++tap) {
      const int ny = yy + tap / 3 - 1, nx = xx + tap % 3 - 1;
      vmask |= (ny >= 0 && ny < g.H && nx >= 0 && nx < g.W) ? (1u << tap) : 0u;
    }
    const float* yb = y1s + pl;
    uint4* drow = cst + pl * rs16;
#pragma unroll
    for (int c4 = 0; c4 < NCH; ++c4) {
      if (GR > 1 && (c4 & (GR - 1)) != gid) continue;
      float v[8];
#pragma unroll
      for (int e = 0; e < 8; ++e) {
        constexpr int dummy = 0; (void)dummy;
        const int k = c4 * 8 + e;
        if (k < K1) {
          const int tap = k / CH, ci = k % CH;
          v[e] = ((vmask >> tap) & 1u) ? yb[ci * ldp + noff[tap]] : 0.f;
        } else {
          v[e] = 0.f;
        }
      }
      drow[c4] = make_uint4(bf2(v[0], v[1]), bf2(v[2], v[3]), bf2(v[4], v[5]), bf2(v[6], v[7]));
    }
    for (int c4 = NCH; c4 < r16; ++c4)
      if (GR == 1 || (c4 & (GR - 1)) == gid) drow[c4] = make_uint4(0u, 0u, 0u, 0u);
  }
  __syncthreads();
  uint4* out4 = reinterpret_cast<uint4*>(col + (static_cast<long long>(b0) << g.lgHW) * K1p);
  copy_out_rows(out4, cst, npix, r16, rs16, tid);
}

template <int CH, int UN>
__device__ __forceinline__ void col2im_gather(const float* __restrict__ dcol, int K1p, const Geo& g, long long m0,
                                              int i0, int nitems, float (&out)[UN]) {
  const int HWm = g.HW - 1, Wm = g.W - 1;
  float v[UN][9];
#pragma unroll
  for (int u = 0; u < UN; ++u) {
    const int i = i0 + u * ZT;
    const bool live = i < nitems;
    const int pl = live ? i / CH : 0, ci = live ? i - pl * CH : 0;
    const long long m = m0 + pl;
    const int rem = static_cast<int>(m & HWm);
    const int yy = rem >> g.lgW, xx = rem & Wm;
#pragma unroll
    for (int tap = 0; tap < 9; ++tap) {
      const int ddy = tap / 3 - 1, ddx = tap % 3 - 1;
      const int ny = yy - ddy, nx = xx - ddx;
      v[u][tap] = (live && ny >= 0 && ny < g.H && nx >= 0 && nx < g.W)
                      ? __ldg(dcol + (m - ddy * g.W - ddx) * K1p + tap * CH + ci) : 0.f;
    }
  }
#pragma unroll
  for (int u = 0; u < UN; ++u) {
    float a = 0.f;
#pragma unroll
    for (int tap = 0; tap < 9; ++tap) a += v[u][tap];
    out[u] = a;
  }
}

template <int C>
__global__ void __launch_bounds__(ZT)
coupling_fwd_kernel(const float* __restrict__ P, int K3p, const float* __restrict__ bias3, float* __restrict__ y,
                    float* __restrict__ hsave, float* __restrict__ ld, Geo g, int reverse) {
  constexpr int J = C / 2;
  const long long M = static_cast<long long>(g.B) << g.lgHW;
  const long long item = static_cast<long long>(blockIdx.x) * ZT + threadIdx.x;
  const long long m = item / J;
  const int j = static_cast<int>(item - m * J);
  const bool live = m < M;
  const int lane = threadIdx.x & 31;
  float lsum = 0.f;
  int b = -1;
  if (live) {
    b = static_cast<int>(m >> g.lgHW);
    const int rem = static_cast<int>(m) & (g.HW - 1);
    const int yy = rem >> g.lgW, xx = rem & (g.W - 1);
    float sh = __ldg(bias3 + 2 * j), lg = __ldg(bias3 + 2 * j + 1);
    const float* prow = P + m * K3p + 2 * j;
#pragma unroll
    for (int tap = 0; tap < 9; ++tap) {
      const int dy = tap / 3 - 1, dx = tap % 3 - 1;
      const int ny = yy + dy, nx = xx + dx;
      if (ny >= 0 && ny < g.H && nx >= 0 && nx < g.W) {
        const float2 v = __ldg(reinterpret_cast<const float2*>(prow + static_cast<long long>(dy * g.W + dx) * K3p +
                                                               tap * C));
        sh += v.x;
        lg += v.y;
      }
    }
    if (hsave) *reinterpret_cast<float2*>(hsave + m * C + 2 * j) = make_float2(sh, lg);
    float s, lsv;
    sigmoid_logsigmoid(lg + 2.f, s, lsv);
    float* yp = y + ((static_cast<long long>(b) * C + J + j) << g.lgHW) + rem;
    const float z2 = *yp;
    *yp = reverse ? (z2 / s - sh) : (z2 + sh) * s;
    lsum = reverse ? -lsv : lsv;
  }
  if (ld) {
#pragma unroll
    for (int o = 1; o < 32; o <<= 1) {
      const float v = __shfl_down_sync(0xffffffffu, lsum, o);
      const int bb = __shfl_down_sync(0xffffffffu, b, o);
      if (lane + o < 32 && bb == b) lsum += v;
    }
    const int bp = __shfl_up_sync(0xffffffffu, b, 1);
    if (live && (lane == 0 || bp != b)) atomicAdd(ld + b, lsum);
  }
}

template <int C, bool INV>
__global__ void __launch_bounds__(ZT)
coupling_bwd_kernel(const float* __restrict__ g_out, const float* __restrict__ g_ld, const float* __restrict__ z_out,
                    const float* __restrict__ hsave, float* __restrict__ dy, __nv_bfloat16* __restrict__ dhcol,
                    int K3p, float* __restrict__ dbias3, Geo g, int brows) {
  pdl_launch_dependents();
  pdl_wait();
  extern __shared__ float sm[];
  constexpr int J = C / 2;
  const int bands = g.H / brows;
  const bool banded = bands > 1;
  const int halo = banded ? g.W : 0;
  const int tile = banded ? brows * g.W : g.pixt;
  const int ldp = tile + 2 * halo + 1;
  float* dhs = sm;
  float* dbs = dhs + C * ldp;
  uint4* cst = reinterpret_cast<uint4*>(dbs + ((C + 3) & ~3));
  const int tid = threadIdx.x;
  const int HWm = g.HW - 1, Wm = g.W - 1;
  const int ngroups = banded ? g.B * bands : (g.B + g.ipc - 1) / g.ipc;
  constexpr int K3 = 9 * C;
  constexpr int NCH = (K3 + 7) / 8;
  const int r16 = K3p / 8, rs16 = r16 + 1;
  int noff[9];
#pragma unroll
  for (int tap = 0; tap < 9; ++tap) noff[tap] = -((tap / 3 - 1) * g.W + (tap % 3 - 1));
  for (int i = tid; i < C; i += ZT) dbs[i] = 0.f;

  for (int grp = blockIdx.x; grp < ngroups; grp += gridDim.x) {
    const int b0 = banded ? grp / bands : grp * g.ipc;
    const int p0 = banded ? (grp - b0 * bands) * tile : 0;
    const int nimg = banded ? 1 : min(g.ipc, g.B - b0);
    const int npix = banded ? tile : nimg << g.lgHW;
    const int np2 = npix + 2 * halo;
    __syncthreads();
    constexpr int UN = 4;
    for (int i0 = tid; i0 < J * np2; i0 += UN * ZT) {
      float g1[UN], g2[UN], o2[UN], glv[UN];
      float2 hh[UN];
      long long lo[UN];
      int pqv[UN], jjv[UN];
      bool inr[UN], ownv[UN];
#pragma unroll
      for (int u = 0; u < UN; ++u) {
        const int i = i0 + u * ZT;
        const int jj = i / np2, pq = i - jj * np2;
        const int pl = pq - halo;
        const int img = banded ? 0 : pl >> g.lgHW;
        const int rem = banded ? p0 + pl : pl & HWm;
        jjv[u] = jj; pqv[u] = pq;
        ownv[u] = i < J * np2 && pl >= 0 && pl < npix;
        inr[u] = i < J * np2 && rem >= 0 && rem < g.HW;
        g1[u] = g2[u] = o2[u] = glv[u] = 0.f;
        hh[u] = make_float2(0.f, 0.f);
        lo[u] = 0;
        if (inr[u]) {
          lo[u] = ((static_cast<long long>(b0 + img) * C + jj) << g.lgHW) + rem;
          const long long hi = lo[u] + (static_cast<long long>(J) << g.lgHW);
          const long long m = (static_cast<long long>(b0 + img) << g.lgHW) + rem;
          g2[u] = g_out[hi];
          o2[u] = z_out[hi];
          hh[u] = *reinterpret_cast<const float2*>(hsave + m * C + 2 * jj);
          glv[u] = g_ld[b0 + img];
          if (ownv[u]) g1[u] = g_out[lo[u]];
        }
      }
#pragma unroll
      for (int u = 0; u < UN; ++u) {
        if (i0 + u * ZT >= J * np2) continue;
        float dsh = 0.f, dlg = 0.f;
        if (inr[u]) {
          float sg, lsv;
          sigmoid_logsigmoid(hh[u].y + 2.f, sg, lsv);
          dsh = INV ? -g2[u] : g2[u] * sg;
          dlg = INV ? -(g2[u] * (o2[u] + hh[u].x) + glv[u]) * (1.f - sg) : (g2[u] * o2[u] + glv[u]) * (1.f - sg);
          if (ownv[u]) {
            dy[lo[u]] = g1[u];
            dy[lo[u] + (static_cast<long long>(J) << g.lgHW)] = INV ? g2[u] / sg : dsh;
          }
        }
        const int jj = jjv[u];
        dhs[(2 * jj) * ldp + pqv[u]] = dsh;
        dhs[(2 * jj + 1) * ldp + pqv[u]] = dlg;
        float a = ownv[u] ? dsh : 0.f, bsum = ownv[u] ? dlg : 0.f;
        if ((np2 & 31) == 0) {
          for (int o = 16; o > 0; o >>= 1) {
            a += __shfl_xor_sync(0xffffffffu, a, o);
            bsum += __shfl_xor_sync(0xffffffffu, bsum, o);
          }
          if ((tid & 31) == 0) { atomicAdd(&dbs[2 * jj], a); atomicAdd(&dbs[2 * jj + 1], bsum); }
        } else {
          atomicAdd(&dbs[2 * jj], a);
          atomicAdd(&dbs[2 * jj + 1], bsum);
        }
      }
    }
    __syncthreads();
    const int GR = tile >= ZT ? 1 : ZT / tile;
    const int gid = tid / tile;
    for (int pl = GR > 1 ? (tid & (tile - 1)) : tid; pl < npix; pl += (GR > 1 ? tile : ZT)) {
      const int rem = banded ? p0 + pl : pl & HWm;
      const int yy = rem >> g.lgW, xx = rem & Wm;
      uint32_t vmask = 0;
#pragma unroll
      for (int tap = 0; tap < 9; ++tap) {
        const int ny = yy - (tap / 3 - 1), nx = xx - (tap % 3 - 1);
        vmask |= (ny >= 0 && ny < g.H && nx >= 0 && nx < g.W) ? (1u << tap) : 0u;
      }
      const float* db = dhs + halo + pl;
      uint4* drow = cst + pl * rs16;
#pragma unroll
      for (int c4 = 0; c4 < NCH; ++c4) {
        if (GR > 1 && (c4 & (GR - 1)) != gid) continue;
        float v[8];
#pragma unroll
        for (int e = 0; e < 8; ++e) {
          const int k = c4 * 8 + e;
          if (k < K3) {
            const int tap = k / C, co = k % C;
            v[e] = ((vmask >> tap) & 1u) ? db[co * ldp + noff[tap]] : 0.f;
          } else {
            v[e] = 0.f;
          }
        }
        drow[c4] = make_uint4(bf2(v[0], v[1]), bf2(v[2], v[3]), bf2(v[4], v[5]), bf2(v[6], v[7]));
      }
      for (int c4 = NCH; c4 < r16; ++c4)
        if (GR == 1 || (c4 & (GR - 1)) == gid) drow[c4] = make_uint4(0u, 0u, 0u, 0u);
    }
    __syncthreads();
    uint4* out4 = reinterpret_cast<uint4*>(dhcol + ((static_cast<long long>(b0) << g.lgHW) + p0) * K3p);
    copy_out_rows(out4, cst, npix, r16, rs16, tid);
  }
  __syncthreads();
  for (int i = tid; i < C; i += ZT) atomicAdd(dbias3 + i, dbs[i]);
}

template <int C>
__global__ void __launch_bounds__(ZT)
affine1x1_bwd_kernel(const float* __restrict__ dy, const float* __restrict__ dcol, int K1p,
                     const float* __restrict__ x, const float* __restrict__ Wf, float* __restrict__ dx,
                     float* __restrict__ dWf, float* __restrict__ dbf, Geo g, int tile_floats) {
  pdl_launch_dependents();
  pdl_wait();
  extern __shared__ float sm[];
  constexpr int CH = C / 2;
  const int ldp = g.pixt + 1;
  float* WT = sm;
  float* dys = WT + C * C;
  float* xs = dys + C * ldp;
  float* acc = dys + tile_floats;
  const int tid = threadIdx.x;
  const int HWm = g.HW - 1;
  const int ngroups = (g.B + g.ipc - 1) / g.ipc;

  for (int i = tid; i < C * C; i += ZT) {
    const int o = i / C, c = i % C;
    WT[c * C + o] = Wf[i];
  }
  for (int i = tid; i < C * C + C; i += ZT) acc[i] = 0.f;
  constexpr int NBK = (C / 4) * (C / 4);
  constexpr int SL = NBK >= ZT ? 1 : ZT / NBK;
  constexpr int RB = (NBK + ZT - 1) / ZT;
  float wacc[RB][4][4] = {};

  for (int grp = blockIdx.x; grp < ngroups; grp += gridDim.x) {
    const int b0 = grp * g.ipc;
    const int nimg = min(g.ipc, g.B - b0);
    const int npix = nimg << g.lgHW;
    __syncthreads();
    {
      constexpr int UL = 4;
      const int total = C * npix;
      for (int i0 = tid; i0 < total; i0 += UL * ZT) {
        float xv[UL], dv[UL];
        int so[UL];
#pragma unroll
        for (int u = 0; u < UL; ++u) {
          const int i = i0 + u * ZT;
          xv[u] = dv[u] = 0.f;
          so[u] = -1;
          if (i < total) {
            const int c = i / npix, pl = i - c * npix;
            const int img = pl >> g.lgHW, rem = pl & HWm;
            const long long gi = ((static_cast<long long>(b0 + img) * C + c) << g.lgHW) + rem;
            xv[u] = x[gi];
            dv[u] = dy[gi];
            so[u] = c * ldp + pl;
          }
        }
#pragma unroll
        for (int u = 0; u < UL; ++u)
          if (so[u] >= 0) { xs[so[u]] = xv[u]; dys[so[u]] = dv[u]; }
      }
    }
    __syncthreads();
    if (dcol) {
      constexpr int UN = 3;
      for (int i0 = tid; i0 < CH * npix; i0 += UN * ZT) {
        float a[UN];
        col2im_gather<CH, UN>(dcol, K1p, g, static_cast<long long>(b0) << g.lgHW, i0, CH * npix, a);
#pragma unroll
        for (int u = 0; u < UN; ++u) {
          const int i = i0 + u * ZT;
          if (i < CH * npix) {
            const int pl = i / CH, ci = i - pl * CH;
            dys[ci * ldp + pl] += a[u];
          }
        }
      }
      __syncthreads();
    }
    for (int pl = tid; pl < npix; pl += ZT) {
      const int img = pl >> g.lgHW, rem = pl & HWm;
      float dv[C];
#pragma unroll
      for (int o = 0; o < C; ++o) dv[o] = dys[o * ldp + pl];
      float* dxp = dx + ((static_cast<long long>(b0 + img) * C) << g.lgHW) + rem;
#pragma unroll 4
      for (int i = 0; i < C; ++i) {
        float a = 0.f;
        const float4* wr = reinterpret_cast<const float4*>(WT + i * C);
#pragma unroll
        for (int o = 0; o < C / 4; ++o) {
          const float4 w = wr[o];
          a = fmaf(w.x, dv[4 * o], a);
          a = fmaf(w.y, dv[4 * o + 1], a);
          a = fmaf(w.z, dv[4 * o + 2], a);
          a = fmaf(w.w, dv[4 * o + 3], a);
        }
        dxp[static_cast<long long>(i) << g.lgHW] = a;
      }
    }
#pragma unroll
    for (int rb = 0; rb < RB; ++rb) {
      const int blk = (NBK < ZT ? tid % NBK : tid) + rb * ZT;
      const int slice = NBK < ZT ? tid / NBK : 0;
      if (blk >= NBK || slice >= SL) continue;
      const int to = blk / (C / 4), ti = blk % (C / 4);
      for (int p = slice; p < npix; p += SL) {
        float dv[4], xv[4];
#pragma unroll
        for (int q = 0; q < 4; ++q) {
          dv[q] = dys[(4 * to + q) * ldp + p];
          xv[q] = xs[(4 * ti + q) * ldp + p];
        }
#pragma unroll
        for (int q = 0; q < 4; ++q)
#pragma unroll
          for (int r = 0; r < 4; ++r) wacc[rb][q][r] = fmaf(dv[q], xv[r], wacc[rb][q][r]);
      }
    }
    {
      const int warp = tid >> 5, lane = tid & 31;
      for (int o = warp; o < C; o += ZT / 32) {
        float a = 0.f;
        for (int p = lane; p < npix; p += 32) a += dys[o * ldp + p];
        for (int sft = 16; sft > 0; sft >>= 1) a += __shfl_xor_sync(0xffffffffu, a, sft);
        if (lane == 0) acc[C * C + o] += a;
      }
    }
  }
  __syncthreads();
  float* scratch = dys;
#pragma unroll
  for (int rb = 0; rb < RB; ++rb) {
    const int blk = (NBK < ZT ? tid % NBK : tid) + rb * ZT;
    const int slice = NBK < ZT ? tid / NBK : 0;
    if (blk >= NBK || slice >= SL) continue;
    const int to = blk / (C / 4), ti = blk % (C / 4);
#pragma unroll
    for (int q = 0; q < 4; ++q)
#pragma unroll
      for (int r = 0; r < 4; ++r) scratch[slice * C * C + (4 * to + q) * C + 4 * ti + r] = wacc[rb][q][r];
  }
  __syncthreads();
  for (int i = tid; i < C * C; i += ZT) {
    float a = 0.f;
    for (int sl2 = 0; sl2 < SL; ++sl2) a += scratch[sl2 * C * C + i];
    acc[i] += a;
  }
  __syncthreads();
  for (int i = tid; i < C * C; i += ZT) atomicAdd(dWf + i, acc[i]);
  for (int i = tid; i < C; i += ZT) atomicAdd(dbf + i, acc[C * C + i]);
}

constexpr int C2I_UN = 3;
template <int C>
__global__ void __launch_bounds__(ZT)
col2im_add_kernel(const float* __restrict__ dcol, int K1p, float* __restrict__ dz, Geo g) {
  pdl_launch_dependents();
  pdl_wait();
  constexpr int CH = C / 2;
  constexpr int PPC = C2I_UN * ZT / CH;
  const long long M = static_cast<long long>(g.B) << g.lgHW;
  const long long m0 = static_cast<long long>(blockIdx.x) * PPC;
  const int nitems = static_cast<int>(min(static_cast<long long>(PPC), M - m0)) * CH;
  float a[C2I_UN];
  col2im_gather<CH, C2I_UN>(dcol, K1p, g, m0, threadIdx.x, nitems, a);
#pragma unroll
  for (int u = 0; u < C2I_UN; ++u) {
    const int i = threadIdx.x + u * ZT;
    if (i < nitems) {
      const int pl = i / CH, ci = i - pl * CH;
      const long long m = m0 + pl;
      dz[((((m >> g.lgHW) * C) + ci) << g.lgHW) + (m & (g.HW - 1))] += a[u];
    }
  }
}

static Geo make_geo(int B, int C, int H, int W, bool heavy) {
  Geo g;
  g.B = B; g.H = H; g.W = W; g.HW = H * W;
  int target = heavy ? (C <= 24 ? 256 : (C <= 48 ? 128 : 64)) : 256;
  g.ipc = g.HW >= target ? 1 : target / g.HW;
  if (g.ipc > B) g.ipc = B;
  while (g.ipc > 1 && (B + g.ipc - 1) / g.ipc < 2 * 148) g.ipc >>= 1;
  g.pixt = g.ipc * g.HW;
  g.og = 1;
  g.lgW = 0; while ((1 << g.lgW) < W) ++g.lgW;
  g.lgHW = 0; while ((1 << g.lgHW) < g.HW) ++g.lgHW;
  return g;
}

static bool pow2(int v) { return v > 0 && (v & (v - 1)) == 0; }

template <typename K>
static int ensure_smem(K kernel, int bytes) {
  return ensure_dyn_smem(reinterpret_cast<const void*>(kernel), bytes);
}

#define NFK_DISPATCH_C(C_, ...)                             \
  switch (C_) {                                             \
    case 12: { constexpr int CC = 12; __VA_ARGS__; } break; \
    case 24: { constexpr int CC = 24; __VA_ARGS__; } break; \
    case 48: { constexpr int CC = 48; __VA_ARGS__; } break; \
    case 96: { constexpr int CC = 96; __VA_ARGS__; } break; \
    default: return NFK_ERR_SHAPE;                          \
  }

}

using namespace nfk;

extern "C" int nfk_affine1x1_fwd(const float* x, const float* Wf, const float* bf, const float* sl, float* y,
                                 void* col, int K1p, const float* ld_in, float* ld_out, int B, int C, int H, int W,
                                 void* stream) {
  if (B <= 0 || H <= 0 || W <= 0 || H * W > 4096 || !pow2(H) || !pow2(W)) return NFK_ERR_SHAPE;
  if (!x || (!Wf && !col) || (Wf && (!bf || !y)) || (ld_out && (!ld_in || !sl))) return NFK_ERR_ARG;
  if (col && (K1p % 64 || K1p < 9 * (C / 2))) return NFK_ERR_SHAPE;
  Geo g = make_geo(B, C, H, W, false);
  if (col) {
    while (g.ipc > 1 && static_cast<long long>(g.pixt) * (K1p * 2 + 16) > 64 * 1024) { g.ipc >>= 1; g.pixt = g.ipc * g.HW; }
  }
  {
    const long long M = static_cast<long long>(B) * H * W;
    g.og = M >= 131072 ? 1 : (M >= 32768 ? 2 : (M >= 8192 && C < 48 ? 4 : 8));
    while (g.og > 1 && (C % g.og || (C / g.og) % 2)) g.og >>= 1;
  }
  if (col && g.HW <= 16)
    while (g.pixt < 128 && 2 * g.ipc <= B && (B + 2 * g.ipc - 1) / (2 * g.ipc) >= 148) { g.ipc <<= 1; g.pixt = g.ipc * g.HW; }
  const int smem = (C * C + C + (col ? (C / 2) * (g.pixt + 1) + 4 + g.pixt * (K1p / 8 + 1) * 4 : 0)) * 4;
  const int grid = (B + g.ipc - 1) / g.ipc;
  cudaStream_t st = static_cast<cudaStream_t>(stream);
  NFK_DISPATCH_C(C, {
    int rc = ensure_smem(affine1x1_fwd_kernel<CC>, smem);
    if (rc) return rc;
    if (launch_pdl(affine1x1_fwd_kernel<CC>, dim3(grid), dim3(ZT), smem, st, x, Wf, bf, sl, y,
                   static_cast<__nv_bfloat16*>(col), ld_in, ld_out, g, K1p) != cudaSuccess)
      return NFK_ERR_LAUNCH;
  });
  return cudaGetLastError() == cudaSuccess ? NFK_OK : NFK_ERR_LAUNCH;
}

extern "C" int nfk_coupling_fwd(const float* P, int K3p, const float* bias3, float* y, float* hsave, float* ld,
                                int B, int C, int H, int W, int reverse, void* stream) {
  if (B <= 0 || H <= 0 || W <= 0 || H * W > 4096 || K3p < 9 * C || K3p % 2 || !pow2(H) || !pow2(W))
    return NFK_ERR_SHAPE;
  if (!P || !bias3 || !y) return NFK_ERR_ARG;
  Geo g = make_geo(B, C, H, W, false);
  const long long items = static_cast<long long>(B) * H * W * (C / 2);
  const unsigned grid = static_cast<unsigned>((items + ZT - 1) / ZT);
  cudaStream_t st = static_cast<cudaStream_t>(stream);
  NFK_DISPATCH_C(C, { coupling_fwd_kernel<CC><<<grid, ZT, 0, st>>>(P, K3p, bias3, y, hsave, ld, g, reverse); });
  return cudaGetLastError() == cudaSuccess ? NFK_OK : NFK_ERR_LAUNCH;
}

namespace nfk {
template <bool INV>
static int coupling_bwd_launch(const float* g_out, const float* g_ld, const float* z_out, const float* hsave,
                               float* dy, void* dhcol, int K3p, float* dbias3, int B, int C, int H, int W,
                               void* stream) {
  if (B <= 0 || H <= 0 || W <= 0 || H * W > 4096 || K3p % 64 || K3p < 9 * C || !pow2(H) || !pow2(W))
    return NFK_ERR_SHAPE;
  if (!g_out || !g_ld || !z_out || !hsave || !dy || !dhcol || !dbias3) return NFK_ERR_ARG;
  Geo g = make_geo(B, C, H, W, true);
  auto bytes = [&](int tile, int halo) {
    return static_cast<long long>(C * (tile + 2 * halo + 1) + ((C + 3) & ~3)) * 4 +
           static_cast<long long>(tile) * (K3p / 8 + 1) * 16 + 16;
  };
  while (g.ipc > 1 && bytes(g.pixt, 0) > 100 * 1024) { g.ipc >>= 1; g.pixt = g.ipc * g.HW; }
  int brows = H;
  if (g.ipc == 1)
    while (brows > 1 && bytes(brows * W, brows < H ? W : 0) > 100 * 1024) brows >>= 1;
  const bool banded = brows < H;
  const int smem = static_cast<int>(bytes(banded ? brows * W : g.pixt, banded ? W : 0));
  const int groups = banded ? B * (H / brows) : (B + g.ipc - 1) / g.ipc;
  const int grid = groups < 4 * 148 ? groups : 4 * 148;
  cudaStream_t st = static_cast<cudaStream_t>(stream);
  NFK_DISPATCH_C(C, {
    int rc = ensure_smem(coupling_bwd_kernel<CC, INV>, smem);
    if (rc) return rc;
    if (launch_pdl(coupling_bwd_kernel<CC, INV>, dim3(grid), dim3(ZT), smem, st, g_out, g_ld, z_out, hsave, dy,
                   static_cast<__nv_bfloat16*>(dhcol), K3p, dbias3, g, brows) != cudaSuccess)
      return NFK_ERR_LAUNCH;
  });
  return cudaGetLastError() == cudaSuccess ? NFK_OK : NFK_ERR_LAUNCH;
}
}

extern "C" int nfk_coupling_bwd(const float* g_out, const float* g_ld, const float* z_out, const float* hsave,
                                float* dy, void* dhcol, int K3p, float* dbias3, int B, int C, int H, int W,
                                void* stream) {
  return coupling_bwd_launch<false>(g_out, g_ld, z_out, hsave, dy, dhcol, K3p, dbias3, B, C, H, W, stream);
}

extern "C" int nfk_coupling_inv_bwd(const float* g_zc, const float* g_ld, const float* zc, const float* hsave,
                                    float* dz, void* dhcol, int K3p, float* dbias3, int B, int C, int H, int W,
                                    void* stream) {
  return coupling_bwd_launch<true>(g_zc, g_ld, zc, hsave, dz, dhcol, K3p, dbias3, B, C, H, W, stream);
}

extern "C" int nfk_affine1x1_bwd(const float* dy, const float* dcol, int K1p, const float* x, const float* Wf,
                                 float* dx, float* dWf, float* dbf, int B, int C, int H, int W, void* stream) {
  if (B <= 0 || H <= 0 || W <= 0 || H * W > 4096 || !pow2(H) || !pow2(W)) return NFK_ERR_SHAPE;
  if (!dy || !x || !Wf || !dx || !dWf || !dbf) return NFK_ERR_ARG;
  Geo g = make_geo(B, C, H, W, true);
  const int nbk = (C / 4) * (C / 4);
  const int slices = nbk >= ZT ? 1 : ZT / nbk;
  int tile_floats = 2 * C * (g.pixt + 1);
  if (tile_floats < slices * C * C) tile_floats = slices * C * C;
  const int smem = (C * C + tile_floats + C * C + C) * 4;
  const int groups = (B + g.ipc - 1) / g.ipc;
  const int grid = groups < 4 * 148 ? groups : 4 * 148;
  cudaStream_t st = static_cast<cudaStream_t>(stream);
  NFK_DISPATCH_C(C, {
    int rc = ensure_smem(affine1x1_bwd_kernel<CC>, smem);
    if (rc) return rc;
    if (launch_pdl(affine1x1_bwd_kernel<CC>, dim3(grid), dim3(ZT), smem, st, dy, dcol, K1p, x, Wf, dx, dWf, dbf, g,
                   tile_floats) != cudaSuccess)
      return NFK_ERR_LAUNCH;
  });
  return cudaGetLastError() == cudaSuccess ? NFK_OK : NFK_ERR_LAUNCH;
}

extern "C" int nfk_col2im_add(const float* dcol, int K1p, float* dz, int B, int C, int H, int W, void* stream) {
  if (B <= 0 || H <= 0 || W <= 0 || H * W > 4096 || !pow2(H) || !pow2(W) || K1p < 9 * (C / 2)) return NFK_ERR_SHAPE;
  if (!dcol || !dz) return NFK_ERR_ARG;
  Geo g = make_geo(B, C, H, W, false);
  const long long M = static_cast<long long>(B) * H * W;
  const long long ppc = C2I_UN * ZT / (C / 2);
  const unsigned grid = static_cast<unsigned>((M + ppc - 1) / ppc);
  cudaStream_t st = static_cast<cudaStream_t>(stream);
  NFK_DISPATCH_C(C, {
    if (launch_pdl(col2im_add_kernel<CC>, dim3(grid), dim3(ZT), 0, st, dcol, K1p, dz, g) != cudaSuccess)
      return NFK_ERR_LAUNCH;
  });
  return cudaGetLastError() == cudaSuccess ? NFK_OK : NFK_ERR_LAUNCH;
}
```

nf_distillation_b200/functional.py:

```python
from __future__ import annotations

import os
from dataclasses import dataclass
from typing import Optional

import torch

from . import ops

BF16 = torch.bfloat16
F32 = torch.float32
USE_FUSED_CNET = os.environ.get("NFK_FUSED_CNET", "1") != "0"
USE_FUSED_PCONV = os.environ.get("NFK_FUSED_PCONV", "1") != "0"
USE_FUSED_CNET_BWD = os.environ.get("NFK_FUSED_CNET_BWD", "1") != "0"
USE_FUSED_DGRAD1 = os.environ.get("NFK_FUSED_DGRAD1", "1") != "0"

WGRAD_STREAM_MAX_M = int(os.environ.get("NFK_WGRAD_STREAM_MAX_M", "65536"))
_wgrad_streams: dict = {}
_wgrad_keepalive: list = []


def _wgrad_stream(dev):
    key = (dev.type, dev.index if dev.index is not None else torch.cuda.current_device())
    st = _wgrad_streams.get(key)
    if st is None:
        st = _wgrad_streams[key] = torch.cuda.Stream(device=dev)
    return st


def _join_wgrads(dev):
    if _wgrad_keepalive:
        torch.cuda.current_stream(dev).wait_stream(_wgrad_stream(dev))
        _wgrad_keepalive.clear()

_PARAM_EPOCH = [0]


def bump_param_epoch() -> None:
    _PARAM_EPOCH[0] += 1


def param_key(params) -> tuple:
    params = list(params)
    epoch = _PARAM_EPOCH[0] if any(p.requires_grad for p in params) else -1
    return (epoch, tuple((p.data_ptr(), p._version) for p in params))


@dataclass
class StepConsts:
    Wf: torch.Tensor
    bf: torch.Tensor
    sl: torch.Tensor
    B1: torch.Tensor = None
    B1T: torch.Tensor = None
    B2: torch.Tensor = None
    B2T: torch.Tensor = None
    B3: torch.Tensor = None
    B3T: torch.Tensor = None
    bias1: torch.Tensor = None
    bias2: torch.Tensor = None
    bias3: torch.Tensor = None


def build_affine(an_bias, an_logs, inv, C, reverse, transpose):
    dev = an_bias.device
    Wf = torch.empty(C, C, device=dev, dtype=F32)
    bf = torch.empty(C, device=dev, dtype=F32)
    sl = torch.empty(1, device=dev, dtype=F32)
    lower, upper, log_s, p, sign_s, weight = inv
    ops.invconv_prep(an_bias, an_logs, lower, upper, log_s, p, sign_s, weight, C, reverse, transpose, Wf, bf, sl)
    return Wf, bf, sl


class PrepCtx:

    def __init__(self, steps, reverse: bool):
        self.steps = list(steps)
        self.reverse = bool(reverse)
        self.index = {id(s): i for i, s in enumerate(self.steps)}
        n = len(self.steps)
        self.consts = [None] * n
        self.items = [None] * n
        self.grads = [None] * n
        self.cops = [None] * n
        self.citems = [None] * n
        self.cgrads = [None] * n
        self.token = None

    def build(self):
        flat = []
        for st in self.steps:
            iv = st.invconv
            if iv.LU_decomposed:
                flat += [st.actnorm.bias, st.actnorm.logs, iv.lower, iv.upper, iv.log_s]
            else:
                flat += [st.actnorm.bias, st.actnorm.logs, iv.weight, iv.weight, iv.weight]
        for st in self.steps:
            if not st.is_1d:
                flat += list(st._coupling_params_2d())
        self.token = PrepAllFn.apply(self, *flat)
        return self

    def lookup(self, step, reverse):
        i = self.index.get(id(step))
        return None if i is None or self.reverse != bool(reverse) else i


_PREP_STACK: list = []


class use_prep:

    def __init__(self, pctx):
        self.pctx = pctx

    def __enter__(self):
        if self.pctx is not None:
            _PREP_STACK.append(self.pctx)
        return self.pctx

    def __exit__(self, *exc):
        if self.pctx is not None:
            _PREP_STACK.pop()
            self.pctx.token = None
        return False


def prep_for(step, reverse):
    for pctx in reversed(_PREP_STACK):
        i = pctx.lookup(step, reverse)
        if i is not None:
            return pctx, i, pctx.token
    pctx = PrepCtx([step], reverse).build()
    token, pctx.token = pctx.token, None
    return pctx, 0, token


def prepare_steps(layers, reverse):
    if not torch.is_grad_enabled():
        return None
    steps = [l for l in layers if getattr(l, "_batched_prep_ok", None) is not None and l._batched_prep_ok()
             and l.actnorm.logs.requires_grad]
    if len(steps) < 2:
        return None
    return PrepCtx(steps, reverse).build()


class PrepAllFn(torch.autograd.Function):
    @staticmethod
    def forward(ctx, pctx, *flat):
        dev = flat[0].device
        sizes = [(st.in_channels * st.in_channels, st.in_channels, 1) for st in pctx.steps]
        total = sum(ops.round_up(a, 4) + ops.round_up(b, 4) + 4 for a, b, _ in sizes)
        buf = torch.empty(total, device=dev, dtype=F32)
        off = 0
        items = []
        for i, st in enumerate(pctx.steps):
            C = st.in_channels
            Wf = buf[off:off + C * C].view(C, C); off += ops.round_up(C * C, 4)
            bf = buf[off:off + C]; off += ops.round_up(C, 4)
            sl = buf[off:off + 1]; off += 4
            an_bias, an_logs, lower, upper, log_s = flat[5 * i:5 * i + 5]
            if st.invconv.LU_decomposed:
                it = ops.invconv_item(an_bias, an_logs, lower, upper, log_s, st.invconv.p, st.invconv.sign_s, None, C,
                                      pctx.reverse, st.is_1d, Wf, bf, sl)
            else:
                it = ops.invconv_item(an_bias, an_logs, None, None, None, None, None, lower, C, pctx.reverse,
                                      st.is_1d, Wf, bf, sl)
            items.append(it)
            pctx.consts[i] = (Wf, bf, sl)
            pctx.items[i] = it
        ops.invconv_prep_batch(items)
        off = 5 * len(pctx.steps)
        citems = []
        for i, st in enumerate(pctx.steps):
            if st.is_1d:
                continue
            cw = flat[off:off + 9]; off += 9
            C, hid = st.in_channels, st.hidden_channels
            cin, cout = C // 2, C
            K1p, K3p = ops.round_up(9 * cin, 64), ops.round_up(9 * cout, 64)
            e = lambda *s_: torch.empty(*s_, device=dev, dtype=BF16)
            B1, B2, B3 = e(hid, K1p), e(hid, hid), e(K3p, hid)
            B1T, B2T, B3T = e(K1p, hid), e(hid, hid), e(hid, K3p)
            bias = torch.empty(2 * hid + ops.round_up(cout, 4), device=dev, dtype=F32)
            bias1, bias2, bias3 = bias[:hid], bias[hid:2 * hid], bias[2 * hid:2 * hid + cout]
            it = ops.coupling_item(cw, cin, hid, cout, K1p, K3p, True, B1, B1T, B2, B2T, B3, B3T, bias1, bias2, bias3)
            citems.append(it)
            pctx.citems[i] = it
            pctx.cops[i] = (B1, B1T, B2, B2T, B3, B3T, bias1, bias2, bias3)
        ops.coupling_prep_batch(citems)
        ctx.pctx = pctx
        ctx.set_materialize_grads(False)
        ctx.save_for_backward(*flat)
        return torch.empty(1, device=dev, dtype=F32)

    @staticmethod
    def backward(ctx, _g_token):
        pctx = ctx.pctx
        flat = ctx.saved_tensors
        dev = flat[0].device
        _join_wgrads(dev)
        n = len(pctx.steps)
        live = [i for i in range(n) if pctx.grads[i] is not None]
        sizes = []
        for i in live:
            C = pctx.steps[i].in_channels
            sizes += [C, C, C * C, C * C, C]
        offs = [0]
        for sz in sizes:
            offs.append(offs[-1] + ops.round_up(sz, 4))
        arena = torch.empty(offs[-1], device=dev, dtype=F32)
        out = [None] * (5 * n)
        items = []
        for j, i in enumerate(live):
            C = pctx.steps[i].in_channels
            d = [arena[offs[5 * j + k]:offs[5 * j + k] + sizes[5 * j + k]] for k in range(5)]
            d_bias, d_logs = d[0].view_as(flat[5 * i]), d[1].view_as(flat[5 * i + 1])
            d_lower, d_upper, d_log_s = d[2].view(C, C), d[3].view(C, C), d[4]
            dWf, dWf_ld, dbf, g_ld, B, pixels = pctx.grads[i]
            if pctx.steps[i].invconv.LU_decomposed:
                items.append(ops.invconv_bwd_item(pctx.items[i], dWf.data_ptr(), dWf_ld, dbf, g_ld, B, pixels, d_bias,
                                                  d_logs, d_lower, d_upper, d_log_s))
                out[5 * i:5 * i + 5] = [d_bias, d_logs, d_lower, d_upper, d_log_s]
            else:
                items.append(ops.invconv_bwd_item(pctx.items[i], dWf.data_ptr(), dWf_ld, dbf, g_ld, B, pixels, d_bias,
                                                  d_logs, None, None, None, d_weight=d_lower))
                out[5 * i:5 * i + 5] = [d_bias, d_logs, d_lower, None, None]
        ops.invconv_prep_bwd_batch(items)
        pctx.grads = [None] * n
        off = 5 * n
        cout_grads, citems = [], []
        for i, st in enumerate(pctx.steps):
            if st.is_1d:
                continue
            cw = flat[off:off + 9]; off += 9
            if pctx.cgrads[i] is None:
                cout_grads += [None] * 9
                continue
            total = sum(ops.round_up(t.numel(), 4) for t in cw)
            arena_c = torch.empty(total, device=dev, dtype=F32)
            o2, gout = 0, []
            for t in cw:
                gout.append(arena_c[o2:o2 + t.numel()].view_as(t)); o2 += ops.round_up(t.numel(), 4)
            citems.append(ops.coupling_bwd_item(pctx.citems[i], pctx.cgrads[i], gout))
            cout_grads += gout
        ops.coupling_prep_bwd_batch(citems)
        pctx.cgrads = [None] * n
        return (None, *out, *cout_grads)


def build_coupling_ops(cw, cin, hid, cout, with_t):
    dev = cw[0].device
    K1p, K3p = ops.round_up(9 * cin, 64), ops.round_up(9 * cout, 64)
    e = lambda *s: torch.empty(*s, device=dev, dtype=BF16)
    B1, B2, B3 = e(hid, K1p), e(hid, hid), e(K3p, hid)
    B1T, B2T, B3T = (e(K1p, hid), e(hid, hid), e(hid, K3p)) if with_t else (None, None, None)
    bias1 = torch.empty(hid, device=dev, dtype=F32)
    bias2 = torch.empty(hid, device=dev, dtype=F32)
    bias3 = torch.empty(cout, device=dev, dtype=F32)
    ops.coupling_prep(*cw, cin, hid, cout, K1p, K3p, B1, B1T, B2, B2T, B3, B3T, bias1, bias2, bias3, with_t)
    return B1, B1T, B2, B2T, B3, B3T, bias1, bias2, bias3


def _coupling_net(col, k: StepConsts, M, hid, K1p, K3p, keep):
    dev = col.device
    m1 = ops.relu_mask_like(M, hid, dev) if keep else None
    m2 = ops.relu_mask_like(M, hid, dev) if keep else None
    h1 = torch.empty(M, hid, device=dev, dtype=BF16) if keep else None
    h2 = torch.empty(M, hid, device=dev, dtype=BF16)
    if USE_FUSED_CNET and ops.cnet_fused_supported(hid, K1p) and M >= 8192:
        ops.cnet_fwd_fused(col, K1p, k.B1, k.B2, k.bias1, k.bias2, h2, M, hid, h1=h1, mask1=m1, mask2=m2)
    else:
        if h1 is None:
            h1 = torch.empty(M, hid, device=dev, dtype=BF16)
        ops.gemm_nt(col, k.B1, M, hid, K1p, ops.EPI_BIAS_RELU_BF16, h1, bias=k.bias1, aux=m1)
        ops.gemm_nt(h1, k.B2, M, hid, hid, ops.EPI_BIAS_RELU_BF16, h2, bias=k.bias2, aux=m2)
    return (h1, h2, m1, m2) if keep else (None, h2, None, None)


def _conv3_coupling(h2, k: StepConsts, y, hsave, ld, B, C, H, W, hid, K3p, reverse):
    M = B * H * W
    if USE_FUSED_PCONV and ops.pconv_coupling_supported(C, H, W, hid):
        ops.pconv_coupling_fwd(h2, k.B3, K3p, k.bias3, y, hsave, ld, B, C, H, W, hid, reverse)
        return
    P = torch.empty(M, K3p, device=h2.device, dtype=F32)
    ops.gemm_nt(h2, k.B3, M, K3p, hid, ops.EPI_F32, P)
    ops.coupling_fwd(P, K3p, k.bias3, y, hsave, ld, B, C, H, W, reverse=reverse)


def flowstep2d_forward(x, ld_in, k: StepConsts, hid, keep):
    B, C, H, W = x.shape
    M, cin = B * H * W, C // 2
    K1p, K3p = ops.round_up(9 * cin, 64), ops.round_up(9 * C, 64)
    dev = x.device
    y = torch.empty_like(x)
    col = torch.empty(M, K1p, device=dev, dtype=BF16)
    ld_out = torch.empty(B, device=dev, dtype=F32)
    ops.affine1x1_fwd(x, k.Wf, k.bf, k.sl, y, col, K1p, ld_in, ld_out, B, C, H, W)
    h1, h2, m1, m2 = _coupling_net(col, k, M, hid, K1p, K3p, keep)
    hsave = torch.empty(M, C, device=dev, dtype=F32) if keep else None
    _conv3_coupling(h2, k, y, hsave, ld_out, B, C, H, W, hid, K3p, False)
    return y, ld_out, (col, h1, h2 if keep else None, hsave, m1, m2)


def flowstep2d_reverse(z, ld_in, k: StepConsts, hid, keep=False):
    B, C, H, W = z.shape
    M, cin = B * H * W, C // 2
    K1p, K3p = ops.round_up(9 * cin, 64), ops.round_up(9 * C, 64)
    dev = z.device
    col = torch.empty(M, K1p, device=dev, dtype=BF16)
    ops.affine1x1_fwd(z, None, None, None, None, col, K1p, None, None, B, C, H, W)
    h1, h2, m1, m2 = _coupling_net(col, k, M, hid, K1p, K3p, keep)
    hsave = torch.empty(M, C, device=dev, dtype=F32) if keep else None
    zc = z.clone()
    ld_mid = ld_in.clone()
    _conv3_coupling(h2, k, zc, hsave, ld_mid, B, C, H, W, hid, K3p, True)
    x = torch.empty_like(z)
    ld_out = torch.empty_like(ld_mid)
    ops.affine1x1_fwd(zc, k.Wf, k.bf, k.sl, x, None, 0, ld_mid, ld_out, B, C, H, W)
    if keep:
        return x, ld_out, (zc, col, h1, h2, hsave, m1, m2)
    return x, ld_out


def _grad_arena(C, hid, K1p, K3p, dev):
    sizes = [C, hid, hid, K3p * hid, hid * hid, hid * K1p, C * C, C]
    offs = [0]
    for s in sizes:
        offs.append(offs[-1] + ops.round_up(s, 4))
    arena = torch.zeros(offs[-1], device=dev, dtype=F32)
    dbias3, dbias2, dbias1, dB3, dB2, dB1, dWf, dbf = (arena[offs[i]:offs[i] + sizes[i]] for i in range(8))
    return (arena, dbias3, dbias2, dbias1, dB3.view(K3p, hid), dB2.view(hid, hid), dB1.view(hid, K1p),
            dWf.view(C, C), dbf)


def _coupling_net_backward(dhcol, col, h1, h2, m1, m2, B1T, B2T, B3T, dbias2, dbias1, dB3, dB2, dB1, arena, M, hid,
                           K1p, K3p):
    dev = dhcol.device
    dpre2 = torch.empty(M, hid, device=dev, dtype=BF16)
    dpre1 = torch.empty(M, hid, device=dev, dtype=BF16)
    if USE_FUSED_CNET_BWD and ops.cnet_fused_supported(hid, K3p) and M >= 8192:
        ops.cnet_bwd_fused(dhcol, K3p, B3T, B2T, m2, m1, dpre2, dpre1, dbias2, dbias1, M, hid)
    else:
        ops.gemm_nt(dhcol, B3T, M, hid, K3p, ops.EPI_MASK_BF16, dpre2, aux=m2, colsum=dbias2)
        ops.gemm_nt(dpre2, B2T, M, hid, hid, ops.EPI_MASK_BF16, dpre1, aux=m1, colsum=dbias1)
    if 0 < M <= WGRAD_STREAM_MAX_M:
        cur, side = torch.cuda.current_stream(dev), _wgrad_stream(dev)
        side.wait_stream(cur)
        with torch.cuda.stream(side):
            ops.gemm_tn(dhcol, h2, K3p, hid, M, dB3)
            ops.gemm_tn(dpre2, h1, hid, hid, M, dB2)
            ops.gemm_tn(dpre1, col, hid, K1p, M, dB1)
        _wgrad_keepalive.append((dhcol, dpre2, dpre1, h1, h2, col, arena))
    else:
        ops.gemm_tn(dhcol, h2, K3p, hid, M, dB3)
        ops.gemm_tn(dpre2, h1, hid, hid, M, dB2)
        ops.gemm_tn(dpre1, col, hid, K1p, M, dB1)
    return dpre1


def _conv1_dgrad(dpre1, B1T, M, K1p, hid):
    dcol = torch.empty(M, K1p, device=dpre1.device, dtype=F32)
    ops.gemm_nt(dpre1, B1T, M, K1p, hid, ops.EPI_F32, dcol)
    return dcol


class FlowStep2dFn(torch.autograd.Function):

    @staticmethod
    def forward(ctx, x, ld_in, hid, token, pctx, idx):
        B, C, H, W = x.shape
        x = x.contiguous()
        Wf, bf, sl = pctx.consts[idx]
        k = StepConsts(Wf, bf, sl, *pctx.cops[idx])
        y, ld_out, (col, h1, h2, hsave, m1, m2) = flowstep2d_forward(x, ld_in.contiguous(), k, hid, keep=True)
        ctx.hid = hid
        ctx.pctx, ctx.idx = pctx, idx
        ctx.save_for_backward(x, y, col, h1, h2, hsave, m1, m2, Wf, k.B1T, k.B2T, k.B3T)
        return y, ld_out

    @staticmethod
    def backward(ctx, g_out, g_ld):
        (x, z_out, col, h1, h2, hsave, m1, m2, Wf, B1T, B2T, B3T) = ctx.saved_tensors
        hid = ctx.hid
        B, C, H, W = x.shape
        M, cin = B * H * W, C // 2
        K1p, K3p = ops.round_up(9 * cin, 64), ops.round_up(9 * C, 64)
        dev = x.device
        _join_wgrads(dev)
        g_out = torch.zeros_like(x) if g_out is None else g_out.contiguous()
        g_ld = torch.zeros(B, device=dev, dtype=F32) if g_ld is None else g_ld.contiguous()
        arena, dbias3, dbias2, dbias1, dB3, dB2, dB1, dWf, dbf = _grad_arena(C, hid, K1p, K3p, dev)

        dy = torch.empty_like(x)
        dhcol = torch.empty(M, K3p, device=dev, dtype=BF16)
        ops.coupling_bwd(g_out, g_ld, z_out, hsave, dy, dhcol, K3p, dbias3, B, C, H, W)
        dpre1 = _coupling_net_backward(dhcol, col, h1, h2, m1, m2, B1T, B2T, B3T, dbias2, dbias1, dB3, dB2, dB1, arena,
                                       M, hid, K1p, K3p)
        dx = torch.empty_like(x)
        if USE_FUSED_DGRAD1 and ops.conv1_dgrad_affine_bwd_supported(C, H, W, hid):
            ops.conv1_dgrad_affine_bwd(dpre1, B1T, K1p, dy, x, Wf, dx, dWf, dbf, B, C, H, W, hid)
        else:
            dcol = _conv1_dgrad(dpre1, B1T, M, K1p, hid)
            ops.affine1x1_bwd(dy, dcol, K1p, x, Wf, dx, dWf, dbf, B, C, H, W)

        ctx.pctx.grads[ctx.idx] = (dWf, C, dbf, g_ld, B, float(H * W))
        ctx.pctx.cgrads[ctx.idx] = (dB1, dbias1, dB2, dbias2, dB3, dbias3)
        return (dx, g_ld, None, None, None, None)


class FlowStep2dReverseFn(torch.autograd.Function):

    @staticmethod
    def forward(ctx, z, ld_in, hid, token, pctx, idx):
        z = z.contiguous()
        Wf, bf, sl = pctx.consts[idx]
        k = StepConsts(Wf, bf, sl, *pctx.cops[idx])
        x, ld_out, (zc, col, h1, h2, hsave, m1, m2) = flowstep2d_reverse(z, ld_in.contiguous(), k, hid, keep=True)
        ctx.hid = hid
        ctx.pctx, ctx.idx = pctx, idx
        ctx.save_for_backward(zc, col, h1, h2, hsave, m1, m2, Wf, k.B1T, k.B2T, k.B3T)
        return x, ld_out

    @staticmethod
    def backward(ctx, g_x, g_ld):
        (zc, col, h1, h2, hsave, m1, m2, Wf, B1T, B2T, B3T) = ctx.saved_tensors
        hid = ctx.hid
        B, C, H, W = zc.shape
        M, cin = B * H * W, C // 2
        K1p, K3p = ops.round_up(9 * cin, 64), ops.round_up(9 * C, 64)
        dev = zc.device
        _join_wgrads(dev)
        g_x = torch.zeros_like(zc) if g_x is None else g_x.contiguous()
        g_ld = torch.zeros(B, device=dev, dtype=F32) if g_ld is None else g_ld.contiguous()
        arena, dbias3, dbias2, dbias1, dB3, dB2, dB1, dWf, dbf = _grad_arena(C, hid, K1p, K3p, dev)

        dzc = torch.empty_like(zc)
        ops.affine1x1_bwd(g_x, None, K1p, zc, Wf, dzc, dWf, dbf, B, C, H, W)
        dz = torch.empty_like(zc)
        dhcol = torch.empty(M, K3p, device=dev, dtype=BF16)
        ops.coupling_inv_bwd(dzc, g_ld, zc, hsave, dz, dhcol, K3p, dbias3, B, C, H, W)
        dpre1 = _coupling_net_backward(dhcol, col, h1, h2, m1, m2, B1T, B2T, B3T, dbias2, dbias1, dB3, dB2, dB1, arena,
                                       M, hid, K1p, K3p)
        ops.col2im_add(_conv1_dgrad(dpre1, B1T, M, K1p, hid), K1p, dz, B, C, H, W)

        ctx.pctx.grads[ctx.idx] = (dWf, C, dbf, g_ld, B, float(H * W))
        ctx.pctx.cgrads[ctx.idx] = (dB1, dbias1, dB2, dbias2, dB3, dbias3)
        return (dz, g_ld, None, None, None, None)


class Split2dFn(torch.autograd.Function):
    @staticmethod
    def forward(ctx, x, ld_in, w, bias, logs):
        B, C, H, W = x.shape
        x = x.contiguous()
        z1 = torch.empty(B, C // 2, H, W, device=x.device, dtype=F32)
        ld = ld_in.clone()
        ops.split2d_fwd(x, w, bias, logs, z1, ld, B, C, H, W)
        ctx.save_for_backward(x, w, bias, logs)
        return z1, ld

    @staticmethod
    def backward(ctx, g_z1, g_ld):
        x, w, bias, logs = ctx.saved_tensors
        B, C, H, W = x.shape
        dev = x.device
        g_ld = torch.zeros(B, device=dev, dtype=F32) if g_ld is None else g_ld.contiguous()
        g_z1 = None if g_z1 is None else g_z1.contiguous()
        dx = torch.empty_like(x)
        nw = w.numel()
        arena = torch.zeros(nw + 2 * C, device=dev, dtype=F32)
        dw, dbias, dlogs = arena[:nw].view_as(w), arena[nw:nw + C].view_as(bias), arena[nw + C:].view_as(logs)
        ops.split2d_bwd(x, w, bias, logs, g_z1, g_ld, dx, dw, dbias, dlogs, B, C, H, W)
        return dx, g_ld, dw, dbias, dlogs


class Split2dSqueezeFn(torch.autograd.Function):

    @staticmethod
    def forward(ctx, x, ld_in, w, bias, logs):
        B, C, H, W = x.shape
        x = x.contiguous()
        z1 = torch.empty(B, C // 2, H, W, device=x.device, dtype=F32)
        z1_sq = torch.empty(B, 2 * C, H // 2, W // 2, device=x.device, dtype=F32)
        ld = ld_in.clone()
        ops.split2d_fwd(x, w, bias, logs, z1, ld, B, C, H, W, z1_sq=z1_sq)
        ctx.save_for_backward(x, w, bias, logs)
        return z1, z1_sq, ld

    @staticmethod
    def backward(ctx, g_z1, g_sq, g_ld):
        x, w, bias, logs = ctx.saved_tensors
        B, C, H, W = x.shape
        dev = x.device
        g_ld = torch.zeros(B, device=dev, dtype=F32) if g_ld is None else g_ld.contiguous()
        g_z1 = None if g_z1 is None else g_z1.contiguous()
        g_sq = None if g_sq is None else g_sq.contiguous()
        dx = torch.empty_like(x)
        nw = w.numel()
        arena = torch.zeros(nw + 2 * C, device=dev, dtype=F32)
        dw, dbias, dlogs = arena[:nw].view_as(w), arena[nw:nw + C].view_as(bias), arena[nw + C:].view_as(logs)
        ops.split2d_bwd(x, w, bias, logs, g_z1, g_ld, dx, dw, dbias, dlogs, B, C, H, W, g_z1_sq=g_sq)
        return dx, g_ld, dw, dbias, dlogs


def split2d_reverse(z1, w, bias, logs, eps, temperature):
    B, CH, H, W = z1.shape
    out = torch.empty(B, 2 * CH, H, W, device=z1.device, dtype=F32)
    ops.split2d_rev(z1.contiguous(), w, bias, logs, eps, temperature, out, B, 2 * CH, H, W)
    return out


class Split2dReverseFn(torch.autograd.Function):

    @staticmethod
    def forward(ctx, z1, w, bias, logs, eps, temperature):
        ctx.ch = z1.shape[1]
        return split2d_reverse(z1, w.detach(), bias.detach(), logs.detach(), eps, temperature)

    @staticmethod
    def backward(ctx, g):
        return g[:, :ctx.ch], None, None, None, None, None


class PriorBpdFn(torch.autograd.Function):

    @staticmethod
    def forward(ctx, z, logdet, mean, logs, scale):
        B = z.shape[0]
        n = z[0].numel()
        z = z.contiguous()
        out = torch.empty(B, device=z.device, dtype=F32)
        ops.prior_bpd_fwd(z, mean, logs, logdet.contiguous(), B, n, scale, out)
        ctx.save_for_backward(z, mean, logs)
        ctx.scale = scale
        return out

    @staticmethod
    def backward(ctx, g):
        z, mean, logs = ctx.saved_tensors
        B = z.shape[0]
        n = z[0].numel()
        dz = torch.empty_like(z)
        dld = torch.empty(B, device=z.device, dtype=F32)
        ops.prior_bpd_bwd(z, mean, logs, g.contiguous(), B, n, ctx.scale, dz, dld)
        return dz, dld, None, None, None


class KdMseFn(torch.autograd.Function):

    @staticmethod
    def forward(ctx, *tensors):
        L = len(tensors) // 2
        s = [t.contiguous() for t in tensors[:L]]
        t = [t.contiguous() for t in tensors[L:]]
        B = s[0].shape[0]
        acc = torch.zeros(B, device=s[0].device, dtype=F32)
        for a, b in zip(s, t):
            n = a[0].numel()
            ops.kd_mse_fwd(a, b, B, n, 1.0 / (n * L), acc)
        ctx.save_for_backward(*s, *t)
        ctx.L = L
        return acc

    @staticmethod
    def backward(ctx, g):
        L = ctx.L
        saved = ctx.saved_tensors
        g = g.contiguous()
        grads = []
        for a, b in zip(saved[:L], saved[L:]):
            B, n = a.shape[0], a[0].numel()
            ds = torch.empty_like(a)
            ops.kd_mse_bwd(a, b, g, B, n, 1.0 / (n * L), ds)
            grads.append(ds)
        return (*grads, *([None] * L))


class KdNllLossFn(torch.autograd.Function):

    @staticmethod
    def forward(ctx, spec, ld_or_nll, z_last, perc, *s_levels):
        s = [t.contiguous() for t in s_levels]
        t = [x.detach().contiguous() for x in spec["teacher"]]
        assert len(s) == len(t)
        B = ld_or_nll.shape[0]
        dev = ld_or_nll.device
        ld_or_nll = ld_or_nll.contiguous()
        z_last = None if z_last is None else z_last.contiguous()
        perc = None if perc is None else perc.contiguous()
        mean, logs = spec["prior"] if spec.get("prior") is not None else (None, None)
        sw = spec.get("sample_w")
        sw = None if sw is None else sw.detach().to(F32).contiguous()
        w_nll, w_kd, w_perc = spec["w"]
        out = torch.empty(4 + 2 * B, device=dev, dtype=F32)
        means, nll, kd = out[:4], out[4:4 + B], out[4 + B:]
        ops.kd_nll_loss_fwd(s, t, z_last, mean, logs, ld_or_nll if z_last is not None else None,
                            spec.get("nll_scale", 1.0), None if z_last is not None else ld_or_nll, perc, sw,
                            w_nll, w_kd, w_perc, B, nll, kd, means)
        ctx.spec, ctx.sw, ctx.L, ctx.B = spec, sw, len(s), B
        ctx.has_z, ctx.has_perc = z_last is not None, perc is not None
        ctx.save_for_backward(z_last, mean, logs, *s, *t)
        ctx.mark_non_differentiable(nll, kd)
        return means, nll, kd

    @staticmethod
    def backward(ctx, g_means, _g_nll, _g_kd):
        z_last, mean, logs, *st = ctx.saved_tensors
        L, B = ctx.L, ctx.B
        s, t = st[:L], st[L:]
        spec = ctx.spec
        w_nll, w_kd, w_perc = spec["w"]
        dev = g_means.device
        needs = ctx.needs_input_grad
        ds = [torch.empty_like(a) if needs[4 + i] else None for i, a in enumerate(s)]
        dz = torch.empty_like(z_last) if ctx.has_z and needs[2] else None
        d_first = torch.empty(B, device=dev, dtype=F32) if needs[1] else None
        dperc = torch.empty(B, device=dev, dtype=F32) if ctx.has_perc and needs[3] else None
        ops.kd_nll_loss_bwd(s, t, ds, z_last if ctx.has_z else None, mean, logs, spec.get("nll_scale", 1.0), ctx.sw,
                            w_nll, w_kd, w_perc, B, g_means.contiguous(), None, None, dz,
                            d_first if ctx.has_z else None, None if ctx.has_z else d_first, dperc)
        return (None, d_first, dz, dperc, *ds)


def kd_mse(student_levels, teacher_levels) -> Optional[torch.Tensor]:
    if not student_levels:
        return None
    return KdMseFn.apply(*student_levels, *[t.detach() for t in teacher_levels])
```

nf_distillation_b200/ops.py:

```python
from __future__ import annotations

import ctypes

import torch

from ._lib import LIB, check

EPI_F32, EPI_BIAS_RELU_BF16, EPI_MASK_BF16 = 0, 1, 2

_LAUNCHES = 0


def launch_count() -> int:
    return _LAUNCHES


def _p(t):
    if t is None:
        return None
    assert t.is_cuda and t.is_contiguous(), "libnfk needs contiguous CUDA tensors"
    return t.data_ptr()


def _st():
    return torch.cuda.current_stream().cuda_stream


def _count(n=1):
    global _LAUNCHES
    _LAUNCHES += n


def round_up(x: int, m: int) -> int:
    return (x + m - 1) // m * m


def relu_mask_like(M, N, device):
    return torch.empty((N + 31) // 32, M, device=device, dtype=torch.int32)


def gemm_nt(A, B, M, N, K, epi, out, bias=None, aux=None, colsum=None):
    assert A.dtype == torch.bfloat16 and B.dtype == torch.bfloat16
    assert aux is None or aux.dtype == torch.int32
    _count()
    check(LIB.nfk_gemm_nt_bf16(_p(A), A.stride(0), _p(B), B.stride(0), M, N, K, epi, _p(out), out.stride(0),
                               _p(bias), _p(aux), 0 if aux is None else aux.stride(0), _p(colsum), _st()),
          "nfk_gemm_nt_bf16")


def gemm_tn(A, B, Mo, No, Kpix, out):
    assert A.dtype == torch.bfloat16 and B.dtype == torch.bfloat16 and out.dtype == torch.float32
    _count()
    check(LIB.nfk_gemm_tn_bf16(_p(A), A.stride(0), _p(B), B.stride(0), Mo, No, Kpix, _p(out), out.stride(0),
                               sm_count(), _st()), "nfk_gemm_tn_bf16")


_SM = {}


def sm_count() -> int:
    d = torch.cuda.current_device()
    if d not in _SM:
        _SM[d] = torch.cuda.get_device_properties(d).multi_processor_count
    return _SM[d]


def invconv_prep(an_bias, an_logs, lower, upper, log_s, p, sign_s, weight, C, reverse, transpose, outW, outb, out_sl):
    _count()
    check(LIB.nfk_invconv_prep(_p(an_bias), _p(an_logs), _p(lower), _p(upper), _p(log_s), _p(p), _p(sign_s),
                               _p(weight), C, int(reverse), int(transpose), _p(outW), _p(outb), _p(out_sl), _st()),
          "nfk_invconv_prep")


def invconv_prep_bwd(an_bias, an_logs, lower, upper, log_s, p, sign_s, weight, C, reverse, transpose, Wf, dWf, dbf,
                     g_ld, B, pixels, d_bias, d_logs, d_lower, d_upper, d_log_s, d_weight):
    _count()
    check(LIB.nfk_invconv_prep_bwd(_p(an_bias), _p(an_logs), _p(lower), _p(upper), _p(log_s), _p(p), _p(sign_s),
                                   _p(weight), C, int(reverse), int(transpose), _p(Wf), _p(dWf), _p(dbf), _p(g_ld),
                                   B,
                                   float(pixels), _p(d_bias), _p(d_logs), _p(d_lower), _p(d_upper), _p(d_log_s),
                                   _p(d_weight), _st()), "nfk_invconv_prep_bwd")


def invconv_item(an_bias, an_logs, lower, upper, log_s, p, sign_s, weight, C, reverse, transpose, outW, outb, out_sl):
    from ._lib import InvconvItem
    return InvconvItem(_p(an_bias), _p(an_logs), _p(lower), _p(upper), _p(log_s), _p(p), _p(sign_s), _p(weight), C,
                       int(reverse), int(transpose), _p(outW), _p(outb), _p(out_sl))


def invconv_prep_batch(items):
    from ._lib import InvconvItem
    n = len(items)
    if not n:
        return
    arr = (InvconvItem * n)(*items)
    _count((n + 23) // 24)
    check(LIB.nfk_invconv_prep_batch(n, ctypes.addressof(arr), _st()), "nfk_invconv_prep_batch")


def invconv_bwd_item(fwd_item, dWf_ptr, dWf_ld, dbf, g_ld, B, pixels, d_bias, d_logs, d_lower, d_upper, d_log_s,
                     d_weight=None):
    from ._lib import InvconvBwdItem
    return InvconvBwdItem(fwd_item, dWf_ptr, dWf_ld, _p(dbf), _p(g_ld), B, float(pixels), _p(d_bias), _p(d_logs),
                          _p(d_lower), _p(d_upper), _p(d_log_s), _p(d_weight))


def invconv_prep_bwd_batch(items):
    from ._lib import InvconvBwdItem
    n = len(items)
    if not n:
        return
    arr = (InvconvBwdItem * n)(*items)
    _count((n + 23) // 24)
    check(LIB.nfk_invconv_prep_bwd_batch(n, ctypes.addressof(arr), _st()), "nfk_invconv_prep_bwd_batch")


def coupling_item(cw, cin, hid, cout, K1p, K3p, with_t, B1, B1T, B2, B2T, B3, B3T, bias1, bias2, bias3):
    from ._lib import CouplingItem
    return CouplingItem(*[_p(t) for t in cw], cin, hid, cout, K1p, K3p, int(with_t), _p(B1), _p(B1T), _p(B2), _p(B2T),
                        _p(B3), _p(B3T), _p(bias1), _p(bias2), _p(bias3))


def coupling_prep_batch(items):
    from ._lib import CouplingItem
    n = len(items)
    if not n:
        return
    arr = (CouplingItem * n)(*items)
    _count((n + 15) // 16)
    check(LIB.nfk_coupling_prep_batch(n, ctypes.addressof(arr), _st()), "nfk_coupling_prep_batch")


def coupling_bwd_item(fwd_item, gin, gout):
    from ._lib import CouplingBwdItem
    return CouplingBwdItem(fwd_item, *[_p(t) for t in gin], *[_p(t) for t in gout])


def coupling_prep_bwd_batch(items):
    from ._lib import CouplingBwdItem
    n = len(items)
    if not n:
        return
    arr = (CouplingBwdItem * n)(*items)
    _count((n + 11) // 12)
    check(LIB.nfk_coupling_prep_bwd_batch(n, ctypes.addressof(arr), _st()), "nfk_coupling_prep_bwd_batch")


def coupling_prep(w1, b1, l1, w2, b2, l2, w3, b3, l3, cin, hid, cout, K1p, K3p, B1, B1T, B2, B2T, B3, B3T, bias1,
                  bias2, bias3, with_t):
    _count()
    check(LIB.nfk_coupling_prep(_p(w1), _p(b1), _p(l1), _p(w2), _p(b2), _p(l2), _p(w3), _p(b3), _p(l3), cin, hid,
                                cout, K1p, K3p, _p(B1), _p(B1T), _p(B2), _p(B2T), _p(B3), _p(B3T), _p(bias1),
                                _p(bias2), _p(bias3), int(with_t), _st()), "nfk_coupling_prep")


def coupling_prep_bwd(w1, b1, l1, w2, b2, l2, w3, b3, l3, cin, hid, cout, K1p, K3p, dB1, dbias1, dB2, dbias2, dB3,
                      dbias3, dw1, db1, dl1, dw2, db2, dl2, dw3, db3, dl3):
    _count()
    check(LIB.nfk_coupling_prep_bwd(_p(w1), _p(b1), _p(l1), _p(w2), _p(b2), _p(l2), _p(w3), _p(b3), _p(l3), cin, hid,
                                    cout, K1p, K3p, _p(dB1), _p(dbias1), _p(dB2), _p(dbias2), _p(dB3), _p(dbias3),
                                    _p(dw1), _p(db1), _p(dl1), _p(dw2), _p(db2), _p(dl2), _p(dw3), _p(db3), _p(dl3),
                                    _st()), "nfk_coupling_prep_bwd")


def affine1x1_fwd(x, Wf, bf, sl, y, col, K1p, ld_in, ld_out, B, C, H, W):
    _count()
    check(LIB.nfk_affine1x1_fwd(_p(x), _p(Wf), _p(bf), _p(sl), _p(y), _p(col), K1p, _p(ld_in), _p(ld_out), B, C, H,
                                W, _st()), "nfk_affine1x1_fwd")


def coupling_fwd(P, K3p, bias3, y, hsave, ld, B, C, H, W, reverse):
    _count()
    check(LIB.nfk_coupling_fwd(_p(P), K3p, _p(bias3), _p(y), _p(hsave), _p(ld), B, C, H, W, int(reverse), _st()),
          "nfk_coupling_fwd")


def coupling_bwd(g_out, g_ld, z_out, hsave, dy, dhcol, K3p, dbias3, B, C, H, W):
    _count()
    check(LIB.nfk_coupling_bwd(_p(g_out), _p(g_ld), _p(z_out), _p(hsave), _p(dy), _p(dhcol), K3p, _p(dbias3), B, C,
                               H, W, _st()), "nfk_coupling_bwd")


def affine1x1_bwd(dy, dcol, K1p, x, Wf, dx, dWf, dbf, B, C, H, W):
    _count()
    check(LIB.nfk_affine1x1_bwd(_p(dy), _p(dcol), K1p, _p(x), _p(Wf), _p(dx), _p(dWf), _p(dbf), B, C, H, W, _st()),
          "nfk_affine1x1_bwd")


def coupling_inv_bwd(g_zc, g_ld, zc, hsave, dz, dhcol, K3p, dbias3, B, C, H, W):
    _count()
    check(LIB.nfk_coupling_inv_bwd(_p(g_zc), _p(g_ld), _p(zc), _p(hsave), _p(dz), _p(dhcol), K3p, _p(dbias3), B, C,
                                   H, W, _st()), "nfk_coupling_inv_bwd")


def col2im_add(dcol, K1p, dz, B, C, H, W):
    _count()
    check(LIB.nfk_col2im_add(_p(dcol), K1p, _p(dz), B, C, H, W, _st()), "nfk_col2im_add")


def split2d_fwd(x, w, bias, logs, z1_out, ld, B, C, H, W, z1_sq=None):
    _count()
    check(LIB.nfk_split2d_squeeze_fwd(_p(x), _p(w), _p(bias), _p(logs), _p(z1_out), _p(z1_sq), _p(ld), B, C, H, W,
                                      _st()), "nfk_split2d_squeeze_fwd")


def dequant_squeeze(src, noise, x_out, sq_out, n_bits=8):
    _count()
    B, C, H, W = src.shape
    check(LIB.nfk_dequant_squeeze(_p(src), int(src.dtype == torch.uint8), n_bits, _p(noise), _p(x_out), _p(sq_out),
                                  B, C, H, W, _st()), "nfk_dequant_squeeze")


def split2d_rev(z1, w, bias, logs, eps, temperature, out, B, C, H, W):
    _count()
    check(LIB.nfk_split2d_rev(_p(z1), _p(w), _p(bias), _p(logs), _p(eps), float(temperature), _p(out), B, C, H, W,
                              _st()), "nfk_split2d_rev")


def split2d_bwd(x, w, bias, logs, g_z1, g_ld, dx, dw, dbias, dlogs, B, C, H, W, g_z1_sq=None):
    _count()
    check(LIB.nfk_split2d_squeeze_bwd(_p(x), _p(w), _p(bias), _p(logs), _p(g_z1), _p(g_z1_sq), _p(g_ld), _p(dx),
                                      _p(dw), _p(dbias), _p(dlogs), B, C, H, W, _st()), "nfk_split2d_squeeze_bwd")


def prior_bpd_fwd(z, mean, logs, logdet, B, n, scale, out):
    _count()
    check(LIB.nfk_prior_bpd_fwd(_p(z), _p(mean), _p(logs), _p(logdet), B, n, float(scale), _p(out), _st()),
          "nfk_prior_bpd_fwd")


def prior_bpd_bwd(z, mean, logs, g_bpd, B, n, scale, dz, dlogdet):
    _count()
    check(LIB.nfk_prior_bpd_bwd(_p(z), _p(mean), _p(logs), _p(g_bpd), B, n, float(scale), _p(dz), _p(dlogdet),
                                _st()), "nfk_prior_bpd_bwd")


def kd_mse_fwd(s, t, B, n, scale, acc):
    _count()
    check(LIB.nfk_kd_mse_fwd(_p(s), _p(t), B, n, float(scale), _p(acc), _st()), "nfk_kd_mse_fwd")


def kd_mse_bwd(s, t, g, B, n, scale, ds, accumulate=False):
    _count()
    check(LIB.nfk_kd_mse_bwd(_p(s), _p(t), _p(g), B, n, float(scale), _p(ds), int(accumulate), _st()),
          "nfk_kd_mse_bwd")


def pconv_coupling_supported(C, H, W, hid):
    return bool(LIB.nfk_pconv_coupling_supported(C, H, W, hid))


def pconv_coupling_fwd(h2, B3, K3p, bias3, y, hsave, ld, B, C, H, W, hid, reverse):
    _count()
    check(LIB.nfk_pconv_coupling_fwd(_p(h2), _p(B3), K3p, _p(bias3), _p(y), _p(hsave), _p(ld), B, C, H, W, hid,
                                     int(reverse), _st()), "nfk_pconv_coupling_fwd")


def conv1_dgrad_affine_bwd_supported(C, H, W, hid):
    return bool(LIB.nfk_conv1_dgrad_affine_bwd_supported(C, H, W, hid))


def conv1_dgrad_affine_bwd(dpre1, B1T, K1p, dy, x, Wf, dx, dWf, dbf, B, C, H, W, hid):
    assert dpre1.dtype == torch.bfloat16 and B1T.dtype == torch.bfloat16
    _count()
    check(LIB.nfk_conv1_dgrad_affine_bwd(_p(dpre1), _p(B1T), K1p, _p(dy), _p(x), _p(Wf), _p(dx), _p(dWf), _p(dbf), B,
                                         C, H, W, hid, _st()), "nfk_conv1_dgrad_affine_bwd")


def flow1d_supported(D, Cc, hid, training=False):
    return bool(LIB.nfk_flow1d_supported(D, Cc, hid, int(training)))


def flow1d_sizes(D, Cc, hid):
    import ctypes
    vals = [ctypes.c_int() for _ in range(4)]
    offs = (ctypes.c_int * 28)()
    check(LIB.nfk_flow1d_sizes(D, Cc, hid, *[ctypes.addressof(v) for v in vals], ctypes.addressof(offs)),
          "nfk_flow1d_sizes")
    return (*[v.value for v in vals], [tuple(offs[4 * l:4 * l + 4]) for l in range(7)])


def flow1d_pack(Wf, bf, ws, bs, D, Cc, hid, PF, PB):
    import ctypes
    _count()
    wa = (ctypes.c_void_p * 6)(*[_p(t) for t in ws])
    ba = (ctypes.c_void_p * 6)(*[_p(t) for t in bs])
    check(LIB.nfk_flow1d_pack(_p(Wf), _p(bf), ctypes.addressof(wa), ctypes.addressof(ba), D, Cc, hid, _p(PF), _p(PB),
                              _st()), "nfk_flow1d_pack")


def flow1d_fwd(x, cond, PF, sl, y, ld_in, ld_out, acts, B, D, Cc, hid, reverse):
    _count()
    check(LIB.nfk_flow1d_fwd(_p(x), _p(cond), _p(PF), _p(sl), _p(y), _p(ld_in), _p(ld_out), _p(acts), B, D, Cc, hid,
                             int(reverse), _st()), "nfk_flow1d_fwd")


def flow1d_bwd(x_in, cond, acts, PB, y_out, g_out, g_ld, dx, G, B, D, Cc, hid, reverse):
    _count()
    check(LIB.nfk_flow1d_bwd(_p(x_in), _p(cond), _p(acts), _p(PB), _p(y_out), _p(g_out), _p(g_ld), _p(dx), _p(G), B, D,
                             Cc, hid, int(reverse), _st()), "nfk_flow1d_bwd")


def affine_rows(x, Wf, bf, sl, y, ld_in, ld_out, B, D, pixels):
    _count()
    check(LIB.nfk_affine_rows(_p(x), _p(Wf), _p(bf), _p(sl), _p(y), _p(ld_in), _p(ld_out), B, D, float(pixels),
                              _st()), "nfk_affine_rows")


def gemm_nt_ranged(A, B, M, N, K, epi, out, bn, kb_begin, kb_end, bias=None, aux=None, colsum=None):
    import ctypes
    _count()
    n = len(kb_begin)
    kb0 = (ctypes.c_int * n)(*kb_begin)
    kb1 = (ctypes.c_int * n)(*kb_end)
    check(LIB.nfk_gemm_nt_bf16_ranged(_p(A), A.stride(0), _p(B), B.stride(0), M, N, K, epi, _p(out), out.stride(0),
                                      _p(bias), _p(aux), 0 if aux is None else aux.stride(0), _p(colsum), bn,
                                      ctypes.addressof(kb0), ctypes.addressof(kb1), _st()), "nfk_gemm_nt_bf16_ranged")


def made_prep(w1, w2, w3, deg1, deg2, D, H, Dp, N3p, B1, B1T, B2, B2T, B3, B3T, with_t):
    _count()
    check(LIB.nfk_made_prep(_p(w1), _p(w2), _p(w3), _p(deg1), _p(deg2), D, H, Dp, N3p, _p(B1), _p(B1T), _p(B2),
                            _p(B2T), _p(B3), _p(B3T), int(with_t), _st()), "nfk_made_prep")


def made_prep_bwd(dB1, dB2, dB3, deg1, deg2, D, H, Dp, dw1, dw2, dw3):
    _count()
    check(LIB.nfk_made_prep_bwd(_p(dB1), _p(dB2), _p(dB3), _p(deg1), _p(deg2), D, H, Dp, _p(dw1), _p(dw2), _p(dw3),
                                _st()), "nfk_made_prep_bwd")


def rows_to_bf16(x, B, D, Dp, xb):
    _count()
    check(LIB.nfk_rows_to_bf16(_p(x), B, D, Dp, _p(xb), _st()), "nfk_rows_to_bf16")


def made_affine_fwd(x, out, N3p, u, ub, Dp, ld_in, ld_out, B, D, flip):
    _count()
    check(LIB.nfk_made_affine_fwd(_p(x), _p(out), N3p, _p(u), _p(ub), Dp, _p(ld_in), _p(ld_out), B, D, int(flip),
                                  _st()), "nfk_made_affine_fwd")


def made_affine_bwd(x, out, N3p, g_u, g_ld, dx, dout, db3, B, D, flip):
    _count()
    check(LIB.nfk_made_affine_bwd(_p(x), _p(out), N3p, _p(g_u), _p(g_ld), _p(dx), _p(dout), _p(db3), B, D, int(flip),
                                  _st()), "nfk_made_affine_bwd")


def made_inv_update(x, xb, Dp, u_in, out, N3p, ld_in, ld_out, B, D, i, flip, last):
    _count()
    check(LIB.nfk_made_inv_update(_p(x), _p(xb), Dp, _p(u_in), _p(out), N3p, _p(ld_in), _p(ld_out), B, D, i,
                                  int(flip), int(last), _st()), "nfk_made_inv_update")


def made_inverse_resident_supported(D, H, Dp) -> bool:
    return bool(LIB.nfk_made_inverse_resident_supported(D, H, Dp))


def made_inverse_push_supported(D, H, Dp, N3p) -> bool:
    return bool(LIB.nfk_made_inverse_push_supported(D, H, Dp, N3p))


def made_inverse_jobs(cnt1, cnt2, D, H, Dp, N3p=0, push=False):
    import torch
    cnt1 = cnt1.to(torch.int32).contiguous().cpu()
    cnt2 = cnt2.to(torch.int32).contiguous().cpu()
    n = LIB.nfk_made_inverse_jobs(cnt1.data_ptr(), cnt2.data_ptr(), D, H, Dp, N3p, int(push), None, 0)
    if push and n == -1:
        return None
    if n <= 0:
        check(n if n < 0 else -1, "nfk_made_inverse_jobs")
    jobs = torch.empty(n, 8, dtype=torch.int32)
    check(0 if LIB.nfk_made_inverse_jobs(cnt1.data_ptr(), cnt2.data_ptr(), D, H, Dp, N3p, int(push), jobs.data_ptr(),
                                         n) == n else -1, "nfk_made_inverse_jobs")
    return jobs


def made_inverse_pack(jobs_dev, B1, B2, B3, N3p, D, H, Dp, push, wstream):
    _count()
    check(LIB.nfk_made_inverse_pack(_p(jobs_dev), jobs_dev.shape[0], _p(B1), _p(B2), _p(B3), N3p, D, H, Dp, int(push),
                                    _p(wstream), _st()), "nfk_made_inverse_pack")


def made_inverse_resident(u_in, wstream, b1, b2, b3, jobs, push, N3p, x, ld_in, ld_out, B, D, H, Dp, flip, mtiles=0):
    _count()
    check(LIB.nfk_made_inverse_resident(_p(u_in), _p(wstream), _p(b1), _p(b2), _p(b3), _p(jobs), jobs.shape[0],
                                        int(push), N3p, _p(x), _p(ld_in), _p(ld_out), B, D, H, Dp, int(flip),
                                        int(mtiles), _st()), "nfk_made_inverse_resident")


def made_inv_bwd_update(c, ldc, g_x, g_ld, out, N3p, u_in, g_u, dout, db3, B, D, d, flip):
    _count()
    check(LIB.nfk_made_inv_bwd_update(_p(c), ldc, _p(g_x), _p(g_ld), _p(out), N3p, _p(u_in), _p(g_u), _p(dout),
                                      _p(db3), B, D, d, int(flip), _st()), "nfk_made_inv_bwd_update")


def made_inverse_bwd_supported(D, H, N3p) -> bool:
    return bool(LIB.nfk_made_inverse_bwd_supported(D, H, N3p))


def made_inverse_bwd_jobs(cnt1, cnt2, D, H, N3p):
    import torch
    cnt1 = cnt1.to(torch.int32).contiguous().cpu()
    cnt2 = cnt2.to(torch.int32).contiguous().cpu()
    n = LIB.nfk_made_inverse_bwd_jobs(cnt1.data_ptr(), cnt2.data_ptr(), D, H, N3p, None, 0)
    if n <= 0:
        check(n if n < 0 else -1, "nfk_made_inverse_bwd_jobs")
    jobs = torch.empty(n, 8, dtype=torch.int32)
    check(0 if LIB.nfk_made_inverse_bwd_jobs(cnt1.data_ptr(), cnt2.data_ptr(), D, H, N3p, jobs.data_ptr(), n) == n
          else -1, "nfk_made_inverse_bwd_jobs")
    return jobs


def made_inverse_bwd_pack(jobs_dev, B1T, B2T, B3T, D, H, N3p, wstream):
    _count()
    check(LIB.nfk_made_inverse_bwd_pack(_p(jobs_dev), jobs_dev.shape[0], _p(B1T), _p(B2T), _p(B3T), D, H, N3p,
                                        _p(wstream), _st()), "nfk_made_inverse_bwd_pack")


def made_inverse_bwd_resident(g_x, g_ld, out, m1, m2, u_in, wstream, jobs, g_u, dout, db3, B, D, H, N3p, flip,
                              mtiles=0):
    _count()
    check(LIB.nfk_made_inverse_bwd_resident(_p(g_x), _p(g_ld), _p(out), _p(m1), _p(m2), _p(u_in), _p(wstream),
                                            _p(jobs), jobs.shape[0], _p(g_u), _p(dout), _p(db3), B, D, H, N3p,
                                            int(flip), int(mtiles), _st()), "nfk_made_inverse_bwd_resident")


def cnet_fused_supported(hid, K1p) -> bool:
    return hid == 512 and K1p % 64 == 0 and 64 <= K1p <= 512


def cnet_fwd_fused(col, K1p, B1, B2, bias1, bias2, h2, M, hid, h1=None, mask1=None, mask2=None, kb2_end_half0=8):
    _count()
    ldm = 0 if mask1 is None else mask1.stride(0)
    check(LIB.nfk_cnet_fwd_fused_ranged(_p(col), K1p, _p(B1), _p(B2), _p(bias1), _p(bias2), _p(h1), _p(h2), _p(mask1),
                                        _p(mask2), ldm, M, hid, int(kb2_end_half0), _st()), "nfk_cnet_fwd_fused_ranged")


def _loss_levels(s_list, t_list, ds_list=None):
    from ._lib import NFK_LOSS_MAX_LEVELS, LossLevels
    L = len(s_list)
    if L > NFK_LOSS_MAX_LEVELS:
        raise ValueError(f"at most {NFK_LOSS_MAX_LEVELS} KD levels per launch")
    lv = LossLevels()
    lv.L = L
    for k in range(L):
        lv.s[k], lv.t[k] = _p(s_list[k]), _p(t_list[k])
        lv.ds[k] = None if ds_list is None or ds_list[k] is None else _p(ds_list[k])
        lv.n[k] = s_list[k][0].numel()
    return lv


def kd_nll_loss_fwd(s_list, t_list, z_last, prior_mean, prior_logs, logdet, nll_scale, nll_in, perc, sample_w, w_nll,
                    w_kd, w_perc, B, nll_out, kd_out, means):
    _count()
    lv = _loss_levels(s_list, t_list)
    scratch = torch.empty(LIB.nfk_kd_nll_loss_scratch_floats(B), device=means.device, dtype=torch.float32)
    nz = 0 if z_last is None else z_last[0].numel()
    check(LIB.nfk_kd_nll_loss_fwd(ctypes.addressof(lv), _p(z_last), nz, _p(prior_mean), _p(prior_logs), _p(logdet),
                                  float(nll_scale), _p(nll_in), _p(perc), _p(sample_w), float(w_nll), float(w_kd),
                                  float(w_perc), B, _p(nll_out), _p(kd_out), _p(means), _p(scratch), _st()),
          "nfk_kd_nll_loss_fwd")


def kd_nll_loss_bwd(s_list, t_list, ds_list, z_last, prior_mean, prior_logs, nll_scale, sample_w, w_nll, w_kd, w_perc,
                    B, g_means, g_nll, g_kd, dz_last, dlogdet, dnll_in, dperc):
    _count()
    lv = _loss_levels(s_list, t_list, ds_list)
    nz = 0 if z_last is None else z_last[0].numel()
    check(LIB.nfk_kd_nll_loss_bwd(ctypes.addressof(lv), _p(z_last), nz, _p(prior_mean), _p(prior_logs),
                                  float(nll_scale), _p(sample_w), float(w_nll), float(w_kd), float(w_perc), B,
                                  _p(g_means), _p(g_nll), _p(g_kd), _p(dz_last), _p(dlogdet), _p(dnll_in), _p(dperc),
                                  _st()), "nfk_kd_nll_loss_bwd")


def optim_partials() -> int:
    return int(LIB.nfk_optim_partials())


def grad_sqnorm(g, partials, step=None):
    _count()
    check(LIB.nfk_grad_sqnorm(_p(g), g.numel(), _p(partials), _p(step), _st()), "nfk_grad_sqnorm")


def adam_step(p, g, m, v, partials, step, max_norm, lr, beta1, beta2, eps, weight_decay, adamax, norm_out=None):
    _count()
    check(LIB.nfk_adam_step(_p(p), _p(g), _p(m), _p(v), p.numel(), _p(partials), _p(step), float(max_norm), float(lr),
                            float(beta1), float(beta2), float(eps), float(weight_decay), int(adamax), _p(norm_out),
                            _st()), "nfk_adam_step")


def cnet_bwd_fused(dhcol, K3p, B3T, B2T, mask_h2, mask_h1, dpre2, dpre1, dbias2, dbias1, M, hid):
    _count()
    check(LIB.nfk_cnet_bwd_fused(_p(dhcol), K3p, _p(B3T), _p(B2T), _p(mask_h2), _p(mask_h1), mask_h2.stride(0),
                                 _p(dpre2), _p(dpre1), _p(dbias2), _p(dbias1), M, hid, _st()), "nfk_cnet_bwd_fused")
```

Measured before the change: 55200.

## Fuse affine 1x1 and im2col building into the tensor-core coupling-net kernel

Adds a MODE 2 variant of the TS cnet forward kernel whose two extra builder warps compute the affine 1x1 transform, the logdet and the swizzled im2col tile in shared memory. The tensor-core pipeline then consumes that tile directly instead of loading col through TMA. This removes the separate affine1x1 launch and the col round trip through global memory, and col is written back only when it is kept for backward. It is enabled for C==12 steps with M>=8192. In exchange it adds halo recomputation, extra shared-memory scratch that can reduce pipeline slots, and the risk that the builder warps stall the MMA.

```diff
diff --git a/include/nfk.h b/include/nfk.h
--- a/include/nfk.h
+++ b/include/nfk.h
@@ -191,6 +191,11 @@
 int nfk_cnet_fwd_fused_ranged(const void* col, int K1p, const void* B1, const void* B2, const float* bias1,
                               const float* bias2, void* h1, void* h2, void* mask1, void* mask2, long long ldmask,
                               int M, int hid, int kb2_end_half0, void* stream);
+int nfk_cnet_fwd_affine_supported(int B, int C, int H, int W, int hid, int K1p);
+int nfk_cnet_fwd_affine(const float* x, const float* Wf, const float* bf, const float* sl, float* y,
+                        const float* ld_in, float* ld_out, void* col, int K1p, const void* B1, const void* B2,
+                        const float* bias1, const float* bias2, void* h1, void* h2, void* mask1, void* mask2,
+                        long long ldmask, int B, int C, int H, int W, int hid, void* stream);
 
 #define NFK_LOSS_MAX_LEVELS 8
 typedef struct {
diff --git a/nf_distillation_b200/_lib.py b/nf_distillation_b200/_lib.py
--- a/nf_distillation_b200/_lib.py
+++ b/nf_distillation_b200/_lib.py
@@ -90,6 +90,8 @@
     "nfk_cnet_fwd_fused": [_vp, _i, _vp, _vp, _vp, _vp, _vp, _vp, _vp, _vp, _ll, _i, _i, _vp],
     "nfk_cnet_bwd_fused": [_vp, _i, _vp, _vp, _vp, _vp, _ll, _vp, _vp, _vp, _vp, _i, _i, _vp],
     "nfk_cnet_fwd_fused_ranged": [_vp, _i, _vp, _vp, _vp, _vp, _vp, _vp, _vp, _vp, _ll, _i, _i, _i, _vp],
+    "nfk_cnet_fwd_affine_supported": [_i] * 6,
+    "nfk_cnet_fwd_affine": [_vp] * 8 + [_i] + [_vp] * 8 + [_ll] + [_i] * 5 + [_vp],
     "nfk_pconv_coupling_supported": [_i, _i, _i, _i],
     "nfk_pconv_coupling_fwd": [_vp, _vp, _i, _vp, _vp, _vp, _vp, _i, _i, _i, _i, _i, _i, _vp],
     "nfk_conv1_dgrad_affine_bwd_supported": [_i, _i, _i, _i],
diff --git a/nf_distillation_b200/csrc/affine_row.cuh b/nf_distillation_b200/csrc/affine_row.cuh
--- /dev/null
+++ b/nf_distillation_b200/csrc/affine_row.cuh
@@ -0,0 +1,24 @@
+#pragma once
+
+namespace nfk {
+
+template <int C>
+__device__ __forceinline__ float affine_row(const float* w, float b, const float (&xv)[C]) {
+  float acc = b;
+  const float4* wr = reinterpret_cast<const float4*>(w);
+#pragma unroll
+  for (int i = 0; i < C / 4; ++i) {
+    const float4 q = wr[i];
+    acc = fmaf(q.x, xv[4 * i], acc);
+    acc = fmaf(q.y, xv[4 * i + 1], acc);
+    acc = fmaf(q.z, xv[4 * i + 2], acc);
+    acc = fmaf(q.w, xv[4 * i + 3], acc);
+  }
+  return acc;
+}
+
+__device__ __forceinline__ float affine_logdet(float ld_in, float sl, int pixels) {
+  return fmaf(sl, static_cast<float>(pixels), ld_in);
+}
+
+}
diff --git a/nf_distillation_b200/csrc/cnet_fused.cu b/nf_distillation_b200/csrc/cnet_fused.cu
--- a/nf_distillation_b200/csrc/cnet_fused.cu
+++ b/nf_distillation_b200/csrc/cnet_fused.cu
@@ -420,7 +420,8 @@
 int cnet_ts_bwd(const void* dhcol, int K3p, const void* B3T, const void* B2T, const void* mask_h2,
                 const void* mask_h1, long long ldmask, void* dpre2, void* dpre1, float* dbias2, float* dbias1, int M,
                 void* stream);
-static bool cnet_use_ts() {
+long long* cnet_prof();
+bool cnet_use_ts() {
   static const bool v = [] { const char* e = getenv("NFK_CNET_TS"); return !(e && e[0] == '0'); }();
   return v;
 }
@@ -430,6 +431,7 @@
 using namespace nfk;
 
 static long long* g_cnet_prof = nullptr;
+long long* nfk::cnet_prof() { return g_cnet_prof; }
 extern "C" int nfk_cnet_set_prof(void* buf) {
   g_cnet_prof = static_cast<long long*>(buf);
   return NFK_OK;
diff --git a/nf_distillation_b200/csrc/cnet_ts.cu b/nf_distillation_b200/csrc/cnet_ts.cu
--- a/nf_distillation_b200/csrc/cnet_ts.cu
+++ b/nf_distillation_b200/csrc/cnet_ts.cu
@@ -5,12 +5,15 @@
 #include <cstdlib>
 
 #include "../../include/nfk.h"
+#include "affine_row.cuh"
 #include "launch_util.h"
 #include "ptx.cuh"
 
 namespace nfk {
 
 constexpr int TS_THREADS = 576;
+constexpr int TS_THREADS_AFF = 640;
+constexpr int TS_EPI_THREADS = 512;
 constexpr int TS_HID = 512;
 constexpr int TS_BOX = 8192;
 constexpr int TS_SLOT = 2 * TS_BOX;
@@ -38,6 +41,43 @@
   float* colsum2;
 };
 
+struct TsAffArgs {
+  const float* x;
+  const float* Wf;
+  const float* bf;
+  const float* sl;
+  float* y;
+  const float* ld_in;
+  float* ld_out;
+  int lgHW, lgW;
+  int halo;
+  int store_col;
+};
+
+__device__ __forceinline__ void mbar_arrive_leader_release(uint64_t* bar) {
+  asm volatile(
+      "{\n\t.reg .b32 remAddr32;\n\t"
+      "mapa.shared::cluster.u32 remAddr32, %0, 0;\n\t"
+      "mbarrier.arrive.release.cluster.shared::cluster.b64 _, [remAddr32];\n\t}\n"
+      ::"r"(smem_u32(bar))
+      : "memory");
+}
+__device__ __forceinline__ void mbar_wait_warp_cluster(uint64_t* bar, uint32_t parity) {
+  auto try_wait = [&]() {
+    uint32_t ok;
+    asm volatile(
+        "{\n\t.reg .pred P;\n\t"
+        "mbarrier.try_wait.parity.acquire.cluster.shared::cta.b64 P, [%1], %2;\n\t"
+        "selp.b32 %0, 1, 0, P;\n\t}\n"
+        : "=r"(ok)
+        : "r"(smem_u32(bar)), "r"(parity)
+        : "memory");
+    return ok != 0;
+  };
+  while (!__all_sync(0xffffffffu, try_wait())) {
+  }
+}
+
 __device__ __forceinline__ void umma_f16_pair_ts(uint32_t tmem_d, uint32_t tmem_a, uint64_t bdesc, uint32_t idesc,
                                                  uint32_t accumulate) {
   asm volatile(
@@ -62,9 +102,10 @@
 }
 __device__ __forceinline__ void tmem_st_wait() { asm volatile("tcgen05.wait::st.sync.aligned;" ::: "memory"); }
 
-template <int MODE>
+template <int MODE, int C = 0>
 __device__ __forceinline__ void cnet_ts_body(const CUtensorMap& tmCol, const CUtensorMap& tmB1, const CUtensorMap& tmB2,
-                                             const CUtensorMap& tmH1, const CUtensorMap& tmH2, const TsArgs& g) {
+                                             const CUtensorMap& tmH1, const CUtensorMap& tmH2, const TsArgs& g,
+                                             const TsAffArgs& a) {
   extern __shared__ __align__(1024) uint8_t smem[];
   pdl_launch_dependents();
   if (smem_u32(smem) & 1023u) __trap();
@@ -94,7 +135,7 @@
     for (int a = 0; a < 2; ++a) { mbar_init(&acc_full[a], 1); mbar_init(&acc_empty[a], 16); }
     for (int p = 0; p < 8; ++p) mbar_init(&h1_full[p], 8);
     mbar_init(h1_empty, 1);
-    mbar_init(col_full, 1);
+    mbar_init(col_full, MODE == 2 ? 2 : 1);
     mbar_init(col_empty, 1);
     fence_mbar_init();
   }
@@ -124,7 +165,7 @@
           tma_load_2d_pair_elect(colbuf + kb * TS_COLBLK, &tmCol, col_full, kb * 64, row0);
         col_ph ^= 1;
       };
-      if (pair < num_tiles) load_col(pair);
+      if (MODE != 2 && pair < num_tiles) load_col(pair);
       for (int t = pair; t < num_tiles; t += num_pairs) {
         const int wrow = static_cast<int>(rank) * 64;
         for (int q = 0; q < 4; ++q)
@@ -133,7 +174,7 @@
           const int qe = q;
           const int kend = qe < 2 ? g.kb2_end[0] : g.kb2_end[1];
           for (int kb = 0; kb < kend; kb += 2) load(&tmB2, kb, kend, qe * 128 + wrow);
-          if (q == 0 && t + num_pairs < num_tiles) load_col(t + num_pairs);
+          if (MODE != 2 && q == 0 && t + num_pairs < num_tiles) load_col(t + num_pairs);
         }
       }
     }
@@ -175,7 +216,8 @@
         mstamp(t, 0);
         {
           const long long c0 = g.prof ? clock64() : 0;
-          mbar_wait_warp(col_full, tile_ph);
+          if constexpr (MODE == 2) mbar_wait_warp_cluster(col_full, tile_ph);
+          else mbar_wait_warp(col_full, tile_ph);
           if (g.prof) { w_op += clock64() - c0; w_col += clock64() - c0; }
           tc_fence_after();
         }
@@ -237,6 +279,100 @@
         o[0] = clock64() - t_begin; o[1] = w_op; o[2] = w_acc; o[3] = w_h1; o[4] = w_col; o[5] = w_b1; o[6] = w_q0;
       }
     }
+  } else if (MODE == 2 && warp >= 18) {
+    if constexpr (MODE == 2) {
+      constexpr int CH = C / 2, K1 = 9 * CH;
+      constexpr int NCH = (K1 + 7) / 8;
+      constexpr int RCH = (K1 + 63) / 64 * 8;
+      constexpr int OU = C == 12 ? 6 : (C == 24 ? 4 : 3);
+      static_assert(C % 4 == 0 && CH % OU == 0 && RCH / 8 <= 8, "unsupported channel count");
+      const int bt = threadIdx.x - 18 * 32;
+      const int lgHW = a.lgHW, lgW = a.lgW, HWm = (1 << lgHW) - 1, Wd = 1 << lgW, Wm = Wd - 1;
+      const int halo = a.halo, npx = 128 + 2 * halo;
+      uint16_t* y1s = reinterpret_cast<uint16_t*>(bias_s + 2 * TS_HID);
+      int noff[9];
+#pragma unroll
+      for (int tap = 0; tap < 9; ++tap) noff[tap] = (tap / 3 - 1) * Wd + (tap % 3 - 1);
+      auto bar_builders = [] { asm volatile("bar.sync 2, 64;" ::: "memory"); };
+      uint32_t col_ph = 0;
+      for (int t = pair; t < num_tiles; t += num_pairs) {
+        const long long m0 = static_cast<long long>(t) * 256 + static_cast<long long>(rank) * 128;
+#pragma unroll 1
+        for (int lp = bt; lp < npx; lp += 64) {
+          const long long m = m0 - halo + lp;
+          if (m < 0 || m >= g.M) continue;
+          const bool own = lp >= halo && lp < halo + 128;
+          const long long img = m >> lgHW;
+          const int p = static_cast<int>(m & HWm);
+          const long long base = (img * C << lgHW) + p;
+          float xv[C];
+#pragma unroll
+          for (int i = 0; i < C; ++i) xv[i] = __ldg(a.x + base + (static_cast<long long>(i) << lgHW));
+          const int nout = own ? C : CH;
+#pragma unroll 1
+          for (int o0 = 0; o0 < nout; o0 += OU) {
+            float acc[OU];
+#pragma unroll
+            for (int u = 0; u < OU; ++u) acc[u] = affine_row<C>(a.Wf + (o0 + u) * C, __ldg(a.bf + o0 + u), xv);
+#pragma unroll
+            for (int u = 0; u < OU; ++u) {
+              if (own) a.y[base + (static_cast<long long>(o0 + u) << lgHW)] = acc[u];
+              if (o0 < CH) y1s[(o0 + u) * npx + lp] = __bfloat16_as_ushort(__float2bfloat16_rn(acc[u]));
+            }
+          }
+          if (own && p == 0) a.ld_out[img] = affine_logdet(__ldg(a.ld_in + img), __ldg(a.sl), HWm + 1);
+        }
+        bar_builders();
+        mbar_wait(col_empty, col_ph ^ 1);
+        if (bt == 0 && a.store_col) asm volatile("cp.async.bulk.wait_group.read 0;" ::: "memory");
+        bar_builders();
+#pragma unroll 1
+        for (int r = bt; r < 128; r += 64) {
+          const long long m = m0 + r;
+          uint8_t* rowp = colbuf + r * 128;
+          const uint32_t sw = static_cast<uint32_t>(r & 7);
+          uint32_t vmask = 0;
+          if (m < g.M) {
+            const int rem = static_cast<int>(m & HWm), yy = rem >> lgW, xx = rem & Wm;
+#pragma unroll
+            for (int tap = 0; tap < 9; ++tap) {
+              const int ny = yy + tap / 3 - 1, nx = xx + tap % 3 - 1;
+              vmask |= (ny >= 0 && ny < (HWm + 1) >> lgW && nx >= 0 && nx < Wd) ? (1u << tap) : 0u;
+            }
+          }
+          const uint16_t* yb = y1s + halo + r;
+#pragma unroll
+          for (int c = 0; c < RCH; ++c) {
+            uint32_t wv[4] = {0u, 0u, 0u, 0u};
+            if (c < NCH) {
+#pragma unroll
+              for (int e = 0; e < 8; ++e) {
+                const int k = c * 8 + e;
+                if (k < K1) {
+                  const int tap = k / CH, ci = k % CH;
+                  const uint32_t v = ((vmask >> tap) & 1u) ? yb[ci * npx + noff[tap]] : 0u;
+                  wv[e / 2] |= v << (16 * (e & 1));
+                }
+              }
+            }
+            *reinterpret_cast<uint4*>(rowp + (c / 8) * TS_COLBLK + ((static_cast<uint32_t>(c % 8) ^ sw) << 4)) =
+                make_uint4(wv[0], wv[1], wv[2], wv[3]);
+          }
+        }
+        fence_proxy_async();
+        bar_builders();
+        if (bt == 0) {
+          mbar_arrive_leader_release(col_full);
+          if (a.store_col) {
+            if (m0 < g.M)
+              for (int kb = 0; kb < RCH / 8; ++kb) tma_store_2d(colbuf + kb * TS_COLBLK, &tmCol, kb * 64, static_cast<int>(m0));
+            asm volatile("cp.async.bulk.commit_group;" ::: "memory");
+          }
+        }
+        col_ph ^= 1;
+      }
+      if (bt == 0) asm volatile("cp.async.bulk.wait_group 0;" ::: "memory");
+    }
   } else {
     const int ew = warp - 2;
     const int qd = warp & 3;
@@ -304,12 +440,12 @@
       s0 += a0 + b0; s1 += a1 + b1;
     };
     float cs1[2][2] = {}, cs2[2][2] = {};
-    if constexpr (MODE == 0) {
-      for (int i = threadIdx.x - 64; i < TS_HID; i += TS_THREADS - 64) {
+    if constexpr (MODE != 1) {
+      for (int i = threadIdx.x - 64; i < TS_HID; i += TS_EPI_THREADS) {
         bias_s[i] = __ldg(g.bias1 + i);
         bias_s[TS_HID + i] = __ldg(g.bias2 + i);
       }
-      asm volatile("bar.sync 1, %0;" ::"n"(TS_THREADS - 64) : "memory");
+      asm volatile("bar.sync 1, %0;" ::"n"(TS_EPI_THREADS) : "memory");
     }
 
 #ifdef NFK_CNET_TIMELINE
@@ -353,7 +489,7 @@
         if (lane == 0) mbar_arrive_cluster(&acc_empty[ws], 0);
         const int col0 = (2 * qq + ws) * 128 + hf * 64;
         uint32_t P[4][8];
-        if constexpr (MODE == 0) {
+        if constexpr (MODE != 1) {
           const bool wb = g.mask1 != nullptr;
           uint32_t b[4];
 #pragma unroll
@@ -408,7 +544,7 @@
         if (lane == 0) mbar_arrive_cluster(&acc_empty[ws], 0);
         const int col0 = (2 * qq + ws) * 128 + hf * 64;
         uint32_t P[4][8];
-        if constexpr (MODE == 0) {
+        if constexpr (MODE != 1) {
           const bool wb = g.mask2 != nullptr;
           uint32_t b[4];
 #pragma unroll
@@ -455,14 +591,22 @@
 cnet_fwd_ts_kernel(const __grid_constant__ CUtensorMap tmCol, const __grid_constant__ CUtensorMap tmB1,
                    const __grid_constant__ CUtensorMap tmB2, const __grid_constant__ CUtensorMap tmH1,
                    const __grid_constant__ CUtensorMap tmH2, const TsArgs g) {
-  cnet_ts_body<0>(tmCol, tmB1, tmB2, tmH1, tmH2, g);
+  cnet_ts_body<0>(tmCol, tmB1, tmB2, tmH1, tmH2, g, TsAffArgs{});
 }
 
 __global__ void __cluster_dims__(2, 1, 1) __launch_bounds__(TS_THREADS, 1)
 cnet_bwd_ts_kernel(const __grid_constant__ CUtensorMap tmCol, const __grid_constant__ CUtensorMap tmB1,
                    const __grid_constant__ CUtensorMap tmB2, const __grid_constant__ CUtensorMap tmH1,
                    const __grid_constant__ CUtensorMap tmH2, const TsArgs g) {
-  cnet_ts_body<1>(tmCol, tmB1, tmB2, tmH1, tmH2, g);
+  cnet_ts_body<1>(tmCol, tmB1, tmB2, tmH1, tmH2, g, TsAffArgs{});
+}
+
+template <int C>
+__global__ void __cluster_dims__(2, 1, 1) __launch_bounds__(TS_THREADS_AFF, 1)
+cnet_fwd_affine_ts_kernel(const __grid_constant__ CUtensorMap tmCol, const __grid_constant__ CUtensorMap tmB1,
+                          const __grid_constant__ CUtensorMap tmB2, const __grid_constant__ CUtensorMap tmH1,
+                          const __grid_constant__ CUtensorMap tmH2, const TsArgs g, const TsAffArgs a) {
+  cnet_ts_body<2, C>(tmCol, tmB1, tmB2, tmH1, tmH2, g, a);
 }
 
 typedef CUresult (*EncodeTiledFn3)(CUtensorMap*, CUtensorMapDataType, cuuint32_t, void*, const cuuint64_t*,
@@ -491,8 +635,8 @@
              : NFK_ERR_DRIVER;
 }
 
-static int ts_smem_plan(int kb1, int* nslots) {
-  const int fixed = kb1 * TS_COLBLK + TS_STAGE_BYTES + TS_BAR_BYTES + TS_BIAS_BYTES;
+static int ts_smem_plan(int kb1, int extra, int* nslots) {
+  const int fixed = kb1 * TS_COLBLK + TS_STAGE_BYTES + TS_BAR_BYTES + TS_BIAS_BYTES + extra;
   int n = (227 * 1024 - fixed) / TS_SLOT;
   if (n > TS_MAX_SLOTS) n = TS_MAX_SLOTS;
   static const int cap = [] { const char* e = getenv("NFK_CNET_SLOTS"); return e ? atoi(e) : 0; }();
@@ -501,30 +645,39 @@
   return fixed + n * TS_SLOT;
 }
 
-template <int MODE>
+static int ts_aff_scratch_bytes(int C, int halo) { return ((C / 2) * (128 + 2 * halo) * 2 + 15) & ~15; }
+
+template <int MODE, int C = 0>
 static int ts_launch(const void* A, int Ka, const void* W1, const void* W2, void* out1, void* out2, TsArgs g,
-                     cudaStream_t stream) {
+                     cudaStream_t stream, const TsAffArgs& a = TsAffArgs{}) {
   int nslots = 0;
-  const int smem_bytes = ts_smem_plan(Ka / 64, &nslots);
+  const int smem_bytes = ts_smem_plan(Ka / 64, MODE == 2 ? ts_aff_scratch_bytes(C, a.halo) : 0, &nslots);
   if (nslots < 2) return NFK_ERR_SHAPE;
   g.nslots = nslots;
   CUtensorMap tmA, tmW1, tmW2, tmO1, tmO2;
   int rc;
-  if ((rc = ts_tmap(&tmA, A, Ka, g.M, Ka, 128))) return rc;
   if ((rc = ts_tmap(&tmW1, W1, Ka, TS_HID, Ka, 64))) return rc;
+  if (A) { if ((rc = ts_tmap(&tmA, A, Ka, g.M, Ka, 128))) return rc; }
+  else tmA = tmW1;
   if ((rc = ts_tmap(&tmW2, W2, TS_HID, TS_HID, TS_HID, 64))) return rc;
   if ((rc = ts_tmap(&tmO2, out2, TS_HID, g.M, TS_HID, 32))) return rc;
   if (out1) { if ((rc = ts_tmap(&tmO1, out1, TS_HID, g.M, TS_HID, 32))) return rc; }
   else tmO1 = tmO2;
   auto kernel = MODE == 0 ? cnet_fwd_ts_kernel : cnet_bwd_ts_kernel;
-  if ((rc = ensure_dyn_smem(reinterpret_cast<const void*>(kernel), smem_bytes))) return rc;
+  const void* kfn = reinterpret_cast<const void*>(kernel);
+  if constexpr (MODE == 2) kfn = reinterpret_cast<const void*>(cnet_fwd_affine_ts_kernel<C>);
+  if ((rc = ensure_dyn_smem(kfn, smem_bytes))) return rc;
   int dev = 0, sms = 148;
   cudaGetDevice(&dev);
   cudaDeviceGetAttribute(&sms, cudaDevAttrMultiProcessorCount, dev);
   const int tiles = (g.M + 255) / 256;
   const int pairs = tiles < sms / 2 ? tiles : sms / 2;
-  const cudaError_t le = launch_pdl(kernel, dim3(2 * pairs), dim3(TS_THREADS), smem_bytes, stream, tmA, tmW1, tmW2,
-                                    tmO1, tmO2, g);
+  cudaError_t le;
+  if constexpr (MODE == 2)
+    le = launch_pdl(cnet_fwd_affine_ts_kernel<C>, dim3(2 * pairs), dim3(TS_THREADS_AFF), smem_bytes, stream, tmA, tmW1,
+                    tmW2, tmO1, tmO2, g, a);
+  else
+    le = launch_pdl(kernel, dim3(2 * pairs), dim3(TS_THREADS), smem_bytes, stream, tmA, tmW1, tmW2, tmO1, tmO2, g);
   return (le == cudaSuccess && cudaGetLastError() == cudaSuccess) ? NFK_OK : NFK_ERR_LAUNCH;
 }
 
@@ -544,4 +697,46 @@
   return ts_launch<1>(dhcol, K3p, B3T, B2T, dpre2, dpre1, g, static_cast<cudaStream_t>(stream));
 }
 
-}
+bool cnet_use_ts();
+long long* cnet_prof();
+
+static bool ts_aff_supported(int B, int C, int H, int W, int hid, int K1p) {
+  if (B <= 0 || H <= 0 || W <= 0 || (H & (H - 1)) || (W & (W - 1)) || hid != TS_HID) return false;
+  if (C != 12 && C != 24 && C != 48) return false;
+  if (K1p != (9 * (C / 2) + 63) / 64 * 64) return false;
+  const long long HW = static_cast<long long>(H) * W;
+  if (!(128 % HW == 0 || (HW % 128 == 0 && 128 % W == 0))) return false;
+  if (static_cast<long long>(B) * HW > (1LL << 31) - 256) return false;
+  int nslots = 0;
+  ts_smem_plan(K1p / 64, ts_aff_scratch_bytes(C, HW > 128 ? W : 0), &nslots);
+  return nslots >= 2 && cnet_use_ts();
+}
+
+}
+
+using namespace nfk;
+
+extern "C" int nfk_cnet_fwd_affine_supported(int B, int C, int H, int W, int hid, int K1p) {
+  return ts_aff_supported(B, C, H, W, hid, K1p) ? 1 : 0;
+}
+
+extern "C" int nfk_cnet_fwd_affine(const float* x, const float* Wf, const float* bf, const float* sl, float* y,
+                                   const float* ld_in, float* ld_out, void* col, int K1p, const void* B1,
+                                   const void* B2, const float* bias1, const float* bias2, void* h1, void* h2,
+                                   void* mask1, void* mask2, long long ldmask, int B, int C, int H, int W, int hid,
+                                   void* stream) {
+  if (!ts_aff_supported(B, C, H, W, hid, K1p)) return NFK_ERR_SHAPE;
+  if (!x || !Wf || !bf || !sl || !y || !ld_in || !ld_out || !B1 || !B2 || !bias1 || !bias2 || !h2) return NFK_ERR_ARG;
+  const int M = B * H * W;
+  if ((mask1 || mask2) && ldmask < M) return NFK_ERR_ARG;
+  TsArgs g{M, K1p / 64, 0, bias1, bias2, static_cast<uint32_t*>(mask1), static_cast<uint32_t*>(mask2), ldmask,
+           h1 ? 1 : 0, cnet_prof(), {8, 8}, nullptr, nullptr};
+  const int lgW = __builtin_ctz(static_cast<unsigned>(W)), lgHW = lgW + __builtin_ctz(static_cast<unsigned>(H));
+  TsAffArgs a{x, Wf, bf, sl, y, ld_in, ld_out, lgHW, lgW, H * W > 128 ? W : 0, col ? 1 : 0};
+  cudaStream_t st = static_cast<cudaStream_t>(stream);
+  switch (C) {
+    case 12: return ts_launch<2, 12>(col, K1p, B1, B2, h1, h2, g, st, a);
+    case 24: return ts_launch<2, 24>(col, K1p, B1, B2, h1, h2, g, st, a);
+    default: return ts_launch<2, 48>(col, K1p, B1, B2, h1, h2, g, st, a);
+  }
+}
diff --git a/nf_distillation_b200/csrc/zpath.cu b/nf_distillation_b200/csrc/zpath.cu
--- a/nf_distillation_b200/csrc/zpath.cu
+++ b/nf_distillation_b200/csrc/zpath.cu
@@ -3,6 +3,7 @@
 #include <cstdint>
 
 #include "../../include/nfk.h"
+#include "affine_row.cuh"
 #include "launch_util.h"
 #include "ptx.cuh"
 
@@ -97,7 +98,7 @@
     }
     for (int i = tid; i < C; i += ZT) bs[i] = bf[i];
   }
-  if (ld_out && tid < nimg) ld_out[b0 + tid] = ld_in[b0 + tid] + sl[0] * static_cast<float>(g.HW);
+  if (ld_out && tid < nimg) ld_out[b0 + tid] = affine_logdet(ld_in[b0 + tid], sl[0], g.HW);
   __syncthreads();
 
   for (int pl = tid % pixb; pl < npix && og < g.og; pl += pixb) {
@@ -110,16 +111,7 @@
     if (Wf) {
       float* yp = y + (static_cast<long long>(b0 + img) * C << g.lgHW) + p;
       for (int o = og * opg; o < (og + 1) * opg; ++o) {
-        float acc = bs[o];
-        const float4* wr = reinterpret_cast<const float4*>(Ws + o * C);
-#pragma unroll
-        for (int i = 0; i < C / 4; ++i) {
-          const float4 w = wr[i];
-          acc = fmaf(w.x, xv[4 * i], acc);
-          acc = fmaf(w.y, xv[4 * i + 1], acc);
-          acc = fmaf(w.z, xv[4 * i + 2], acc);
-          acc = fmaf(w.w, xv[4 * i + 3], acc);
-        }
+        const float acc = affine_row<C>(Ws + o * C, bs[o], xv);
         yp[static_cast<long long>(o) << g.lgHW] = acc;
         if (col && o < CH) y1s[o * ldp + pl] = acc;
       }
diff --git a/nf_distillation_b200/functional.py b/nf_distillation_b200/functional.py
--- a/nf_distillation_b200/functional.py
+++ b/nf_distillation_b200/functional.py
@@ -14,6 +14,7 @@
 USE_FUSED_PCONV = os.environ.get("NFK_FUSED_PCONV", "1") != "0"
 USE_FUSED_CNET_BWD = os.environ.get("NFK_FUSED_CNET_BWD", "1") != "0"
 USE_FUSED_DGRAD1 = os.environ.get("NFK_FUSED_DGRAD1", "1") != "0"
+USE_FUSED_AFFINE = os.environ.get("NFK_FUSED_AFFINE", "1") != "0"
 
 WGRAD_STREAM_MAX_M = int(os.environ.get("NFK_WGRAD_STREAM_MAX_M", "65536"))
 _wgrad_streams: dict = {}
@@ -263,12 +264,17 @@
     return B1, B1T, B2, B2T, B3, B3T, bias1, bias2, bias3
 
 
-def _coupling_net(col, k: StepConsts, M, hid, K1p, K3p, keep):
-    dev = col.device
+def _coupling_net_outputs(M, hid, dev, keep):
     m1 = ops.relu_mask_like(M, hid, dev) if keep else None
     m2 = ops.relu_mask_like(M, hid, dev) if keep else None
     h1 = torch.empty(M, hid, device=dev, dtype=BF16) if keep else None
     h2 = torch.empty(M, hid, device=dev, dtype=BF16)
+    return h1, h2, m1, m2
+
+
+def _coupling_net(col, k: StepConsts, M, hid, K1p, K3p, keep):
+    dev = col.device
+    h1, h2, m1, m2 = _coupling_net_outputs(M, hid, dev, keep)
     if USE_FUSED_CNET and ops.cnet_fused_supported(hid, K1p) and M >= 8192:
         ops.cnet_fwd_fused(col, K1p, k.B1, k.B2, k.bias1, k.bias2, h2, M, hid, h1=h1, mask1=m1, mask2=m2)
     else:
@@ -295,10 +301,17 @@
     K1p, K3p = ops.round_up(9 * cin, 64), ops.round_up(9 * C, 64)
     dev = x.device
     y = torch.empty_like(x)
-    col = torch.empty(M, K1p, device=dev, dtype=BF16)
     ld_out = torch.empty(B, device=dev, dtype=F32)
-    ops.affine1x1_fwd(x, k.Wf, k.bf, k.sl, y, col, K1p, ld_in, ld_out, B, C, H, W)
-    h1, h2, m1, m2 = _coupling_net(col, k, M, hid, K1p, K3p, keep)
+    if (USE_FUSED_AFFINE and USE_FUSED_CNET and M >= 8192 and C == 12
+            and ops.cnet_fwd_affine_supported(B, C, H, W, hid, K1p)):
+        col = torch.empty(M, K1p, device=dev, dtype=BF16) if keep else None
+        h1, h2, m1, m2 = _coupling_net_outputs(M, hid, dev, keep)
+        ops.cnet_fwd_affine(x, k.Wf, k.bf, k.sl, y, ld_in, ld_out, col, K1p, k.B1, k.B2, k.bias1, k.bias2, h2, hid,
+                            h1=h1, mask1=m1, mask2=m2)
+    else:
+        col = torch.empty(M, K1p, device=dev, dtype=BF16)
+        ops.affine1x1_fwd(x, k.Wf, k.bf, k.sl, y, col, K1p, ld_in, ld_out, B, C, H, W)
+        h1, h2, m1, m2 = _coupling_net(col, k, M, hid, K1p, K3p, keep)
     hsave = torch.empty(M, C, device=dev, dtype=F32) if keep else None
     _conv3_coupling(h2, k, y, hsave, ld_out, B, C, H, W, hid, K3p, False)
     return y, ld_out, (col, h1, h2 if keep else None, hsave, m1, m2)
diff --git a/nf_distillation_b200/ops.py b/nf_distillation_b200/ops.py
--- a/nf_distillation_b200/ops.py
+++ b/nf_distillation_b200/ops.py
@@ -437,6 +437,20 @@
                                         _p(mask2), ldm, M, hid, int(kb2_end_half0), _st()), "nfk_cnet_fwd_fused_ranged")
 
 
+def cnet_fwd_affine_supported(B, C, H, W, hid, K1p) -> bool:
+    return bool(LIB.nfk_cnet_fwd_affine_supported(B, C, H, W, hid, K1p))
+
+
+def cnet_fwd_affine(x, Wf, bf, sl, y, ld_in, ld_out, col, K1p, B1, B2, bias1, bias2, h2, hid, h1=None, mask1=None,
+                    mask2=None):
+    B, C, H, W = x.shape
+    _count()
+    ldm = 0 if mask1 is None else mask1.stride(0)
+    check(LIB.nfk_cnet_fwd_affine(_p(x), _p(Wf), _p(bf), _p(sl), _p(y), _p(ld_in), _p(ld_out), _p(col), K1p, _p(B1),
+                                  _p(B2), _p(bias1), _p(bias2), _p(h1), _p(h2), _p(mask1), _p(mask2), ldm, B, C, H, W,
+                                  hid, _st()), "nfk_cnet_fwd_affine")
+
+
 def _loss_levels(s_list, t_list, ds_list=None):
     from ._lib import NFK_LOSS_MAX_LEVELS, LossLevels
     L = len(s_list)
```

Result: no change. 55670 (median of 6 runs) (+0.9%).
